# suryanshkumar/online-joint-depthfusion-and-semantic

Measured on AMD Instinct MI355X. Metric: frames/sec fused (320x240, 256^3 grid), higher is better.
Workload: dtype f16x3; 1 GPU; BASELINE configs[1]: 320x240 depth into a 256^3 fp16 TSDF grid, FusionNet_v3, geometry-only, fast integrate, f16x3 arithmetic, one scene per GPU; grid=256, n_points=9, n_tail_points=7, volume_dtype=f16, parallelism=scene-sharded x1, cpu_affinity=not pinned

## Files before the change

### online_joint_depthfusion_and_semantic_amd/csrc/ojf_net.hip

```cpp
#ifndef OJF_CHAIN_DMA_HALF
#define OJF_CHAIN_DMA_HALF 1536
#endif
#ifndef OJF_CHAIN_BLOCKS
#define OJF_CHAIN_BLOCKS 3
#endif
#ifndef OJF_CHAIN_WAVES
#define OJF_CHAIN_WAVES 4
#endif
#ifndef OJF_CHAIN_AHEAD
#define OJF_CHAIN_AHEAD 2
#endif
#include <chrono>
#include <cmath>
#include <cstdio>
#include <cstdlib>
#include <cstring>
#include <vector>

#include "ojf_common.h"

namespace ojf {

typedef float f32x4 __attribute__((ext_vector_type(4)));
typedef float f32x8 __attribute__((ext_vector_type(8)));
typedef _Float16 f16x8 __attribute__((ext_vector_type(8)));

typedef unsigned u32x4 __attribute__((ext_vector_type(4)));
__device__ __forceinline__ void split_f16(const f32x4 &a, const f32x4 &b, f16x8 &hi, f16x8 &lo)
{
    const f32x8 x = __builtin_shufflevector(a, b, 0, 1, 2, 3, 4, 5, 6, 7);
    hi = __builtin_convertvector(x, f16x8);
    const u32x4 h = __builtin_bit_cast(u32x4, hi);
    u32x4 l;
#pragma unroll
    for (int i = 0; i < 4; ++i) l[i] = split_lo_pair(h[i], x[2 * i], x[2 * i + 1]);
    lo = __builtin_bit_cast(f16x8, l);
}

typedef _Float16 f16x4 __attribute__((ext_vector_type(4)));
typedef unsigned u32x2 __attribute__((ext_vector_type(2)));
__device__ __forceinline__ f32x4 split_pack4(const f32x4 &x)
{
    const f16x4 hi = __builtin_convertvector(x, f16x4);
    const u32x2 h = __builtin_bit_cast(u32x2, hi);
    const u32x4 r{h[0], h[1], split_lo_pair(h[0], x[0], x[1]), split_lo_pair(h[1], x[2], x[3])};
    return __builtin_bit_cast(f32x4, r);
}
__device__ __forceinline__ f32x4 unsplit4(const f32x4 &s)
{
    typedef _Float16 f16x8_ __attribute__((ext_vector_type(8)));
    const f16x8_ h = __builtin_bit_cast(f16x8_, s);
    return f32x4{(float)h[0] + (float)h[4], (float)h[1] + (float)h[5], (float)h[2] + (float)h[6], (float)h[3] + (float)h[7]};
}
#ifndef OJF_UNSAFE_SWAP
#define OJF_UNSAFE_SWAP 0
#endif
__device__ __forceinline__ void unpack_split(const f32x4 &a, const f32x4 &b, f16x8 &hi, f16x8 &lo)
{
#if OJF_UNSAFE_SWAP
    u32x4 A = __builtin_bit_cast(u32x4, a), B = __builtin_bit_cast(u32x4, b);
    unsigned a2 = A[2], a3 = A[3], b0 = B[0], b1 = B[1];
    asm("v_swap_b32 %0, %1" : "+v"(a2), "+v"(b0));
    asm("v_swap_b32 %0, %1" : "+v"(a3), "+v"(b1));
    A[2] = a2; A[3] = a3; B[0] = b0; B[1] = b1;
    hi = __builtin_bit_cast(f16x8, A);
    lo = __builtin_bit_cast(f16x8, B);
#else
    hi = __builtin_bit_cast(f16x8, __builtin_shufflevector(a, b, 0, 1, 4, 5));
    lo = __builtin_bit_cast(f16x8, __builtin_shufflevector(a, b, 2, 3, 6, 7));
#endif
}

__device__ __forceinline__ f32x4 mfma_f16x3(const f32x4 &wh, const f32x4 &wl, const f16x8 &xh, const f16x8 &xl, f32x4 acc)
{
    const f16x8 h = __builtin_bit_cast(f16x8, wh), l = __builtin_bit_cast(f16x8, wl);
    acc = __builtin_amdgcn_mfma_f32_16x16x32_f16(l, xh, acc, 0, 0, 0);
    acc = __builtin_amdgcn_mfma_f32_16x16x32_f16(h, xl, acc, 0, 0, 0);
    return __builtin_amdgcn_mfma_f32_16x16x32_f16(h, xh, acc, 0, 0, 0);
}

static inline int round_up(int x, int m) { return (x + m - 1) / m * m; }

struct ConvArgs {
    const f32x4 *in;
    f32x4 *out;
    float *out_rows;
    const f32x4 *wp;
    const float *bias;
    const float *rinv;
    int in_g0, out_g0, rows_stride, rows_n;
    int h, w, npix;
    int taps, dil;
    int c4;
    int nsteps;
    int og_store;
    int act, act_n;
    float scale;
    int *ovf;
    int accum;
    const float *dscale;
    unsigned w_magic, c4_magic;
    int in_split = 0, out_split = 0;
    int row_perm = 0, perm_q = 0, perm_rem = 0;
};

__device__ __forceinline__ int perm_row(int pr, int r, int q, int rem)
{
    const int big = rem * (q + 1);
    if (pr < big) {
        const int c = pr / (q + 1);
        return c + (pr - c * (q + 1)) * r;
    }
    const int p2 = pr - big, c = p2 / q;
    return rem + c + (p2 - c * q) * r;
}

__device__ __forceinline__ int fast_div(int x, int d, unsigned magic) { return magic ? (int)__umulhi((unsigned)x, magic) : x / d; }

__device__ __forceinline__ float guard_max(float mx, const f32x4 &v)
{
    return fmaxf(fmaxf(fmaxf(mx, fabsf(v[0])), fmaxf(fabsf(v[1]), fabsf(v[2]))), fabsf(v[3]));
}
__device__ __forceinline__ bool beyond_f16(const f32x4 &v)
{
    return guard_max(0.0f, v) > 65504.0f;
}
__device__ __forceinline__ f32x4 fma4(const f32x4 &a, const f32x4 &b, const f32x4 &c)
{
    return f32x4{__builtin_fmaf(a[0], b[0], c[0]), __builtin_fmaf(a[1], b[1], c[1]), __builtin_fmaf(a[2], b[2], c[2]),
                 __builtin_fmaf(a[3], b[3], c[3])};
}

__device__ __forceinline__ float act_slope(int act)
{
    return act == OJF_ACT_RELU ? 0.0f : (act == OJF_ACT_LEAKY ? 0.01f : 1.0f);
}
__device__ __forceinline__ float leaky_max(float x, float slope)
{
    const float sx = slope * x;
    float r;
    asm("v_max_f32 %0, %1, %2" : "=v"(r) : "v"(x), "v"(sx));
    return r;
}
__device__ __forceinline__ f32x4 leaky_max4(const f32x4 &x, float slope)
{
    const f32x4 sx = x * slope;
    f32x4 r;
#pragma unroll
    for (int j = 0; j < 4; ++j) asm("v_max_f32 %0, %1, %2" : "=v"(r[j]) : "v"(x[j]), "v"(sx[j]));
    return r;
}

constexpr int kMaxSteps = 128;
constexpr int kPadSteps = 4;

template <int MT, int NT, bool GUARD = false>
__device__ __forceinline__ void conv_epilogue(const ConvArgs &a, const f32x4 (&acc)[MT][NT], int strip, int i16, int g,
                                              const f32x4 (&bvec)[NT], const f32x4 (&rvec)[NT])
{
    const float slope = act_slope(a.act);
    const bool use_tanh = a.act == OJF_ACT_TANH;
    const float oscale = a.dscale ? a.scale / *a.dscale : a.scale;
    float gmax = 0.0f;
#pragma unroll
    for (int n = 0; n < NT; ++n) {
        const int og = n * 4 + g;
        const f32x4 b = bvec[n];
        const f32x4 ri = rvec[n];
#pragma unroll
        for (int m = 0; m < MT; ++m) {
            const int p = strip + m * 16 + i16;
            const f32x4 lin4 = GUARD ? fma4(acc[m][n], ri, b) : acc[m][n] + b;
            f32x4 v = lin4;
#pragma unroll
            for (int j = 0; j < 4; ++j) {
                const float lin = v[j];
                float r = lin > 0.0f ? lin : lin * slope;
                if (use_tanh) r = tanhf(lin);
                v[j] = (og * 4 + j < a.act_n ? r : lin) * oscale;
            }
            if (p >= a.npix) continue;
            if (a.out_rows) {
#pragma unroll
                for (int j = 0; j < 4; ++j)
                    if (og * 4 + j < a.rows_n) a.out_rows[(size_t)p * a.rows_stride + og * 4 + j] = v[j];
            } else if (og < a.og_store) {
                f32x4 *dst = a.out + (size_t)(a.out_g0 + og) * a.npix + p;
                if (a.accum) v += *dst;
                *dst = a.out_split ? split_pack4(v) : v;
                if constexpr (GUARD) gmax = guard_max(gmax, lin4);
            }
        }
    }
    if constexpr (GUARD)
        if (gmax > 65504.0f && a.ovf) guard_raise(a.ovf, 1);
}

template <int MT, int NT>
__device__ __forceinline__ void conv_epilogue_lean(const ConvArgs &a, const f32x4 (&acc)[MT][NT], int strip, int i16, int g,
                                                   const f32x4 (&bvec)[NT], const f32x4 (&rvec)[NT])
{
    const float slope = act_slope(a.act);
    float gmax = 0.0f;
#pragma unroll
    for (int n = 0; n < NT; ++n) {
        const int og = n * 4 + g;
        if (og >= a.og_store) continue;
#pragma unroll
        for (int m = 0; m < MT; ++m) {
            const int p = strip + m * 16 + i16;
            const f32x4 lin4 = fma4(acc[m][n], rvec[n], bvec[n]);
            const f32x4 v = leaky_max4(lin4, slope);
            if (p < a.npix) {
                a.out[(size_t)(a.out_g0 + og) * a.npix + p] = a.out_split ? split_pack4(v) : v;
                gmax = guard_max(gmax, lin4);
            }
        }
    }
    if (gmax > 65504.0f && a.ovf) guard_raise(a.ovf, 1);
}

static inline bool conv_lean_ok(const ConvArgs &a)
{
    return !a.out_rows && a.act != OJF_ACT_TANH && (a.act == OJF_ACT_NONE || a.act_n >= 4 * a.og_store) && a.scale == 1.0f && !a.dscale && !a.accum;
}

__device__ __forceinline__ void build_tap_table(int2 *tab, const ConvArgs &a, int entries)
{
    for (int G = threadIdx.x; G < entries; G += 256) {
        const int t = G / a.c4, cg = G - t * a.c4;
        int off = -1, dy = -30000, dx = 0;
        if (t < a.taps) {
            dy = dx = 0;
            if (a.taps == 9) {
                const int ky = t / 3;
                dy = (ky - 1) * a.dil;
                dx = (t - 3 * ky - 1) * a.dil;
            }
            off = (a.in_g0 + cg) * a.npix + dy * a.w + dx;
        }
        tab[G] = int2{off, (int)(((unsigned)dy << 16) | ((unsigned)dx & 0xffffu))};
    }
}

__device__ __forceinline__ void build_tap_table16(int2 *tab, const ConvArgs &a, int entries)
{
    for (int G = threadIdx.x; G < entries; G += 256) {
        const int t = fast_div(G, a.c4, a.c4_magic), cg = G - t * a.c4;
        int off = 0, bit = 0;
        if (t < a.taps) {
            int dy = 0, dx = 0;
            if (a.taps == 9) {
                const int ky = t / 3;
                dy = (ky - 1) * a.dil;
                dx = (t - 3 * ky - 1) * a.dil;
            }
            off = ((a.in_g0 + cg) * a.npix + dy * a.w + dx) * 16;
            bit = 1 << t;
        }
        tab[G] = int2{off, bit};
    }
}

struct ConvGroup {
    ConvArgs g[4];
    int nblocks;
    int band = 0;
};


template <int MT, int NT, int ABL = 0, bool SKIP = true>
__global__ __launch_bounds__(256) void conv_mfma_kernel(const ConvGroup grp)
{
    const ConvArgs &a = grp.g[blockIdx.y];
    __shared__ int2 tab[(kMaxSteps + kPadSteps) * 4];
    build_tap_table(tab, a, (a.nsteps + kPadSteps) * 4);
    __syncthreads();

    const int lane = threadIdx.x & 63;
    const int wave = threadIdx.x >> 6;
    const int i16 = lane & 15, g = lane >> 4;
    const int strip = (blockIdx.x * 4 + wave) * (MT * 16);
    if (strip >= a.npix) return;
    constexpr int ot0 = 0;

    int py[MT], px[MT], plin[MT];
#pragma unroll
    for (int m = 0; m < MT; ++m) {
        const int p = strip + m * 16 + i16;
        plin[m] = p;
        py[m] = p < a.npix ? p / a.w : -0x40000000;
        px[m] = p - (p / a.w) * a.w;
    }
    f32x4 acc[MT][NT];
#pragma unroll
    for (int m = 0; m < MT; ++m)
#pragma unroll
        for (int n = 0; n < NT; ++n) acc[m][n] = f32x4{0.f, 0.f, 0.f, 0.f};

    const f32x4 *wb[NT];
#pragma unroll
    for (int n = 0; n < NT; ++n) wb[n] = a.wp + (size_t)(ot0 + n) * (a.nsteps + kPadSteps) * 64 + lane;
    const __amdgpu_buffer_rsrc_t rs = __builtin_amdgcn_make_buffer_rsrc(
        const_cast<f32x4 *>(a.in), 0, (a.in_g0 + a.c4) * a.npix * 16, 0x00020000);

    auto fetch = [&](f32x4(&xv)[MT], f32x4(&wv)[NT], int S, bool &live) {
        if constexpr (ABL & 8) {
            live = true;
#pragma unroll
            for (int m = 0; m < MT; ++m) {
                if constexpr (ABL & 1) xv[m] = f32x4{1.f, 2.f, 3.f, 4.f};
                else xv[m] = __builtin_bit_cast(f32x4, __builtin_amdgcn_raw_buffer_load_b128(rs, (unsigned)plin[m] * 16u, 0, 0));
            }
        } else {
            const int2 e = tab[S * 4 + g];
            const int dy = e.y >> 16, dx = (int)(short)(e.y & 0xffff);
            bool any_ok = false;
#pragma unroll
            for (int m = 0; m < MT; ++m) {
                const bool ok = (unsigned)(py[m] + dy) < (unsigned)a.h && (unsigned)(px[m] + dx) < (unsigned)a.w;
                const unsigned boff = ok ? (unsigned)(e.x + plin[m]) * 16u : 0xffffffffu;
                if constexpr (ABL & 1) {
                    xv[m] = f32x4{1.f, 2.f, 3.f, 4.f};
                    asm volatile("" ::"v"(boff));
                } else {
                    xv[m] = __builtin_bit_cast(f32x4, __builtin_amdgcn_raw_buffer_load_b128(rs, boff, 0, 0));
                }
                any_ok |= ok;
            }
            live = SKIP ? __any(any_ok) : true;
        }
#pragma unroll
        for (int n = 0; n < NT; ++n) {
            if constexpr (ABL & 2) wv[n] = f32x4{1.f, 1.f, 1.f, 1.f};
            else wv[n] = wb[n][(size_t)S * 64];
        }
    };
    auto mac = [&](const f32x4(&xv)[MT], const f32x4(&wv)[NT]) {
        if constexpr (ABL & 4) {
#pragma unroll
            for (int m = 0; m < MT; ++m) asm volatile("" ::"v"(xv[m][0]), "v"(xv[m][1]), "v"(xv[m][2]), "v"(xv[m][3]));
#pragma unroll
            for (int n = 0; n < NT; ++n) asm volatile("" ::"v"(wv[n][0]), "v"(wv[n][1]), "v"(wv[n][2]), "v"(wv[n][3]));
            return;
        }
#pragma unroll
        for (int j = 0; j < 4; ++j)
#pragma unroll
            for (int m = 0; m < MT; ++m)
#pragma unroll
                for (int n = 0; n < NT; ++n)
                    acc[m][n] = __builtin_amdgcn_mfma_f32_16x16x4f32(wv[n][j], xv[m][j], acc[m][n], 0, 0, 0);
    };

    f32x4 x0[MT], w0[NT], x1[MT], w1[NT], x2[MT], w2[NT];
    bool l0, l1, l2;
    fetch(x0, w0, 0, l0);
    fetch(x1, w1, 1, l1);
    for (int S = 0; S < a.nsteps; S += 3) {
        fetch(x2, w2, S + 2, l2);
        if (!SKIP || l0) mac(x0, w0);
        fetch(x0, w0, S + 3, l0);
        if (!SKIP || l1) mac(x1, w1);
        fetch(x1, w1, S + 4, l1);
        if (!SKIP || l2) mac(x2, w2);
    }

    f32x4 bvec[NT], rvec[NT];
#pragma unroll
    for (int n = 0; n < NT; ++n) {
        bvec[n] = *reinterpret_cast<const f32x4 *>(a.bias + (size_t)n * 16 + 4 * g);
        rvec[n] = f32x4{1.f, 1.f, 1.f, 1.f};
    }
    conv_epilogue<MT, NT>(a, acc, strip, i16, g, bvec, rvec);
}

template <int NT>
__global__ __launch_bounds__(256) void conv_mfma_lds_kernel(const ConvGroup grp)
{
    constexpr int CS = 3;
    const ConvArgs &a = grp.g[blockIdx.y];
    __shared__ int2 tab[(kMaxSteps + kPadSteps) * 4];
    __shared__ f32x4 wl[CS * NT * 64];
    build_tap_table(tab, a, (a.nsteps + kPadSteps) * 4);
    __syncthreads();
    const int lane = threadIdx.x & 63, wave = threadIdx.x >> 6;
    const int i16 = lane & 15, g = lane >> 4;
    const int strip = (blockIdx.x * 4 + wave) * 16;
    const int p = strip + i16;
    const int py = p < a.npix ? p / a.w : -0x40000000;
    const int px = p - (p / a.w) * a.w;
    f32x4 acc[1][NT];
#pragma unroll
    for (int n = 0; n < NT; ++n) acc[0][n] = f32x4{0.f, 0.f, 0.f, 0.f};
    const __amdgpu_buffer_rsrc_t rs = __builtin_amdgcn_make_buffer_rsrc(
        const_cast<f32x4 *>(a.in), 0, (a.in_g0 + a.c4) * a.npix * 16, 0x00020000);
    auto fetch = [&](f32x4 &xv, int S) {
        const int2 e = tab[S * 4 + g];
        const int dy = e.y >> 16, dx = (int)(short)(e.y & 0xffff);
        const bool ok = (unsigned)(py + dy) < (unsigned)a.h && (unsigned)(px + dx) < (unsigned)a.w;
        xv = __builtin_bit_cast(f32x4, __builtin_amdgcn_raw_buffer_load_b128(rs, ok ? (unsigned)(e.x + p) * 16u : 0xffffffffu, 0, 0));
    };
    auto mac = [&](const f32x4 &xv, int sl) {
        f32x4 wv[NT];
#pragma unroll
        for (int n = 0; n < NT; ++n) wv[n] = wl[(sl * NT + n) * 64 + lane];
#pragma unroll
        for (int j = 0; j < 4; ++j)
#pragma unroll
            for (int n = 0; n < NT; ++n) acc[0][n] = __builtin_amdgcn_mfma_f32_16x16x4f32(wv[n][j], xv[j], acc[0][n], 0, 0, 0);
    };
    f32x4 x0, x1, x2;
    fetch(x0, 0);
    fetch(x1, 1);
    const int nsp = a.nsteps + kPadSteps;
    for (int S = 0; S < a.nsteps; S += 3) {
        if (S) __syncthreads();
        for (int i = threadIdx.x; i < CS * NT * 64; i += 256) {
            const int n = i / (CS * 64), r = i - n * (CS * 64);
            wl[((r >> 6) * NT + n) * 64 + (r & 63)] = a.wp[((size_t)n * nsp + S) * 64 + r];
        }
        __syncthreads();
        fetch(x2, S + 2);
        mac(x0, 0);
        fetch(x0, S + 3);
        mac(x1, 1);
        fetch(x1, S + 4);
        mac(x2, 2);
    }
    f32x4 bvec[NT], rvec[NT];
#pragma unroll
    for (int n = 0; n < NT; ++n) {
        bvec[n] = *reinterpret_cast<const f32x4 *>(a.bias + (size_t)n * 16 + 4 * g);
        rvec[n] = f32x4{1.f, 1.f, 1.f, 1.f};
    }
    if (strip >= a.npix) return;
    conv_epilogue<1, NT>(a, acc, strip, i16, g, bvec, rvec);
}

constexpr int kPad16 = 6;
constexpr int conv16_chunk(int nt) { return nt <= 2 ? 6 : 3; }

template <int MT, int NT, bool SKIP = true, int ABL = 0, bool LEAN = false, bool INS = false>
#ifndef OJF_CONV_LB
#define OJF_CONV_LB 1
#endif
__global__ __launch_bounds__(256, (OJF_CONV_LB && MT == 2 && NT == 2 && LEAN) ? 4 : 1) void conv_f16x3_kernel(const ConvGroup grp)
{
    constexpr int CS = conv16_chunk(NT);
    const ConvArgs &a = grp.g[blockIdx.y];
    const bool persist = grp.band != 0;
    int sb = grp.nblocks ? xcd_band_block(blockIdx.x, gridDim.x) : blockIdx.x;
    int sb_end = sb + 1, sb_step = 1;
    if (persist) {
        const int x = blockIdx.x & 7, j = blockIdx.x >> 3;
        sb = x * grp.band + j;
        sb_end = (x + 1) * grp.band;
        sb_step = (int)(gridDim.x >> 3);
    }
    if (grp.nblocks && sb >= grp.nblocks) return;
    extern __shared__ int2 tab[];
    __shared__ f32x4 wl[CS * NT * 128];
    build_tap_table16(tab, a, (a.nsteps + kPad16) * 8);
    if (persist) {
#pragma unroll
        for (int i = 0; i < CS * NT * 128 / 256; ++i) wl[i * 256 + threadIdx.x] = a.wp[i * 256 + threadIdx.x];
    }

    const int lane = threadIdx.x & 63, wave = threadIdx.x >> 6;
    const int i16 = lane & 15, g = lane >> 4;
    __syncthreads();
    for (; sb < sb_end && (!grp.nblocks || sb < grp.nblocks); sb += sb_step) {
    int strip = (sb * 4 + wave) * (MT * 16);
    if (a.row_perm) {
        const int pr = fast_div(strip, a.w, a.w_magic);
        if (pr < a.h) strip = perm_row(pr, a.row_perm, a.perm_q, a.perm_rem) * a.w + (strip - pr * a.w);
    }

    int p16[MT];
    unsigned vm[MT];
#pragma unroll
    for (int m = 0; m < MT; ++m) {
        const int p = strip + m * 16 + i16;
        p16[m] = p * 16;
        const int py = fast_div(p, a.w, a.w_magic), px = p - py * a.w;
        unsigned rm = 0, cm = 0;
#pragma unroll
        for (int k = 0; k < 3; ++k) {
            rm |= ((unsigned)(py + (k - 1) * a.dil) < (unsigned)a.h ? 1u : 0u) << k;
            cm |= ((unsigned)(px + (k - 1) * a.dil) < (unsigned)a.w ? 1u : 0u) << k;
        }
        const unsigned all9 = ((rm & 1u) ? cm : 0u) | ((rm & 2u) ? cm << 3 : 0u) | ((rm & 4u) ? cm << 6 : 0u);
        vm[m] = p < a.npix ? (a.taps == 9 ? all9 : 1u) : 0u;
    }
    f32x4 acc[MT][NT];
#pragma unroll
    for (int m = 0; m < MT; ++m)
#pragma unroll
        for (int n = 0; n < NT; ++n) {
            acc[m][n] = f32x4{0.f, 0.f, 0.f, 0.f};
            if constexpr (MT == 1) asm volatile("" : "+v"(acc[m][n]));
        }
    const __amdgpu_buffer_rsrc_t rs = __builtin_amdgcn_make_buffer_rsrc(
        const_cast<f32x4 *>(a.in), 0, (a.in_g0 + a.c4) * a.npix * 16, 0x00020000);
    constexpr bool kHoist = NT <= 4;
    f32x4 bvec[NT], rvec[NT];
    if constexpr (kHoist) {
#pragma unroll
        for (int n = 0; n < NT; ++n) {
            bvec[n] = *reinterpret_cast<const f32x4 *>(a.bias + (size_t)n * 16 + 4 * g);
            rvec[n] = *reinterpret_cast<const f32x4 *>(a.rinv + (size_t)n * 16 + 4 * g);
        }
    }

    const int4 *tab4 = reinterpret_cast<const int4 *>(tab) + g;
    auto fetch = [&](f32x4(&xa)[MT], f32x4(&xb)[MT], const int4 e, bool &live) {
        unsigned any = 0;
#pragma unroll
        for (int m = 0; m < MT; ++m) {
            const unsigned o0 = (unsigned)(e.x + p16[m]) | ((vm[m] & (unsigned)e.y) ? 0u : 0xffffffffu);
            const unsigned o1 = (unsigned)(e.z + p16[m]) | ((vm[m] & (unsigned)e.w) ? 0u : 0xffffffffu);
            if constexpr (ABL & 1) {
                xa[m] = f32x4{1.f, 2.f, 3.f, 4.f};
                xb[m] = f32x4{1.f, 2.f, 3.f, 4.f};
                asm volatile("" ::"v"(o0), "v"(o1));
            } else {
                xa[m] = __builtin_bit_cast(f32x4, __builtin_amdgcn_raw_buffer_load_b128(rs, o0, 0, 0));
                xb[m] = __builtin_bit_cast(f32x4, __builtin_amdgcn_raw_buffer_load_b128(rs, o1, 0, 0));
            }
            any |= vm[m] & (unsigned)(e.y | e.w);
        }
        live = SKIP ? __any(any != 0) : true;
    };
    auto mac = [&](const f32x4(&xa)[MT], const f32x4(&xb)[MT], int sl) {
        f32x4 wh[NT], wlo[NT];
#pragma unroll
        for (int n = 0; n < NT; ++n) {
            if constexpr (ABL & 2) {
                wh[n] = wlo[n] = f32x4{1.f, 1.f, 1.f, 1.f};
                asm volatile("" ::"s"(sl));
            } else {
                wh[n] = wl[(sl * NT + n) * 128 + lane];
                wlo[n] = wl[(sl * NT + n) * 128 + 64 + lane];
            }
        }
#pragma unroll
        for (int m = 0; m < MT; ++m) {
            f16x8 xh, xl;
            if constexpr (ABL & 8) {
                xh = __builtin_bit_cast(f16x8, xa[m]);
                xl = __builtin_bit_cast(f16x8, xb[m]);
            } else if constexpr (INS) {
                unpack_split(xa[m], xb[m], xh, xl);
            } else {
                split_f16(xa[m], xb[m], xh, xl);
            }
            if constexpr (ABL & 4) {
                asm volatile("" ::"v"(xh), "v"(xl));
#pragma unroll
                for (int n = 0; n < NT; ++n) asm volatile("" ::"v"(wh[n]), "v"(wlo[n]));
            } else {
#pragma unroll
                for (int n = 0; n < NT; ++n) acc[m][n] = mfma_f16x3(wh[n], wlo[n], xh, xl, acc[m][n]);
            }
        }
    };

    f32x4 xa0[MT], xb0[MT], xa1[MT], xb1[MT], xa2[MT], xb2[MT];
    bool v0, v1, v2;
    fetch(xa0, xb0, tab4[0], v0);
    fetch(xa1, xb1, tab4[4], v1);
    int sl = persist ? 0 : CS;
    for (int S = 0; S < a.nsteps; S += 3) {
        const int4 t2 = tab4[(S + 2) * 4], t3 = tab4[(S + 3) * 4], t4 = tab4[(S + 4) * 4];
        if (sl == CS) {
            if (S) __syncthreads();
            const f32x4 *src = a.wp + (size_t)S * NT * 128;
#pragma unroll
            for (int i = 0; i < CS * NT * 128 / 256; ++i) wl[i * 256 + threadIdx.x] = src[i * 256 + threadIdx.x];
            __syncthreads();
            sl = 0;
        }
        fetch(xa2, xb2, t2, v2);
        if (!SKIP || v0) mac(xa0, xb0, sl);
        fetch(xa0, xb0, t3, v0);
        if (!SKIP || v1) mac(xa1, xb1, sl + 1);
        fetch(xa1, xb1, t4, v1);
        if (!SKIP || v2) mac(xa2, xb2, sl + 2);
        sl += 3;
    }
    if constexpr (!kHoist) {
#pragma unroll
        for (int n = 0; n < NT; ++n) {
            bvec[n] = *reinterpret_cast<const f32x4 *>(a.bias + (size_t)n * 16 + 4 * g);
            rvec[n] = *reinterpret_cast<const f32x4 *>(a.rinv + (size_t)n * 16 + 4 * g);
        }
    }
    if constexpr (LEAN) conv_epilogue_lean<MT, NT>(a, acc, strip, i16, g, bvec, rvec);
    else conv_epilogue<MT, NT, true>(a, acc, strip, i16, g, bvec, rvec);
    }
}

constexpr int kChainLdsFloat4 = 48 * 1024 / 16;
constexpr int kChainDmaHalf = OJF_CHAIN_DMA_HALF;

struct ChainArgs {
    const f32x4 *in;
    const f32x4 *w;
    const float *bias;
    float *out_rows;
    int in_g0, c4_in, npix, rows_stride, rows_n;
    float scale;
    int *ovf;
    f32x4 *out_planes;
    int out_g0, og_store, act_n;
    struct ColSums *colsum;
    int in_split = 0;
    int split_groups = 0;
};

constexpr int chain_kblocks(int arith, int ntin) { return arith == OJF_ARITH_F16X3 ? (ntin + 1) / 2 : ntin; }
constexpr int chain_unit(int arith) { return arith == OJF_ARITH_F16X3 ? 128 : 64; }
constexpr int chain_layer_size(int arith, int ntin, int ntout) { return ntout * chain_kblocks(arith, ntin) * chain_unit(arith); }
constexpr bool chain_dma(int arith) { return arith == OJF_ARITH_F16X3; }
constexpr int chain_cap(int arith) { return chain_dma(arith) ? kChainDmaHalf : kChainLdsFloat4; }
constexpr int chain_tiles_fit(int arith, int ntin)
{
    return chain_cap(arith) / (chain_kblocks(arith, ntin) * chain_unit(arith));
}
constexpr int chain_parts(int arith, int ntin, int ntout)
{
    return (ntout + chain_tiles_fit(arith, ntin) - 1) / chain_tiles_fit(arith, ntin);
}
constexpr int chain_per(int arith, int ntin, int ntout)
{
    return (ntout + chain_parts(arith, ntin, ntout) - 1) / chain_parts(arith, ntin, ntout);
}
constexpr int chain_first_size(int arith, int ntin, int ntout)
{
    return (chain_per(arith, ntin, ntout) < ntout ? chain_per(arith, ntin, ntout) : ntout) * chain_kblocks(arith, ntin) *
           chain_unit(arith);
}
constexpr int chain_bias_stride(int arith, int ntout) { return (arith == OJF_ARITH_F16X3 ? 2 : 1) * ntout * 16; }
constexpr int kChainAhead = OJF_CHAIN_AHEAD;
constexpr int kChainWaves = OJF_CHAIN_WAVES, kChainThreads = 64 * kChainWaves;
constexpr int kChainPre = kChainLdsFloat4 / kChainThreads;

__device__ __forceinline__ void dma_part(const f32x4 *src, f32x4 *dst, int size, int wave, int lane)
{
#pragma unroll
    for (int c0 = 0; c0 < kChainDmaHalf / 64; c0 += kChainWaves) {
        const int c = c0 + wave;
        if (c * 64 < size)
            __builtin_amdgcn_global_load_lds((const void __attribute__((address_space(1))) *)(src + c * 64 + lane),
                                             (void __attribute__((address_space(3))) *)(dst + c * 64), 16, 0, 0);
    }
}

enum { kChainLeaky = 0, kChainRelu = 1, kChainAccumulate = 2, kChainLastRows = 3, kChainEntry = 4 };

constexpr int kVecF4 = 64;
struct VecStage {
    f32x4 *lds;
    f32x4 reg;
    int half;
};
struct VecNext {
    const float *a = nullptr;
    int na = 0;
    const float *b = nullptr;
    int nb = 0;
};
__device__ __forceinline__ void vec_issue(VecStage &vs, const VecNext &nx)
{
    const int t = threadIdx.x;
    if (t < nx.na) vs.reg = reinterpret_cast<const f32x4 *>(nx.a)[t];
    else if (t < nx.na + nx.nb) vs.reg = reinterpret_cast<const f32x4 *>(nx.b)[t - nx.na];
}
__device__ __forceinline__ const f32x4 *vec_commit(VecStage &vs, int n)
{
    f32x4 *dst = vs.lds + vs.half * kVecF4;
    if ((int)threadIdx.x < n) dst[threadIdx.x] = vs.reg;
    vs.half ^= 1;
    return dst;
}

template <int ARITH, int MT, int NTIN, int NTOUT, int MODE, int NEXT_FIRST, int NA, int NB>
__device__ __forceinline__ void chain_layer(const f32x4 (&in)[MT][NA], f32x4 (&out)[MT][NB], f32x4 *wlds, const f32x4 *wg,
                                            const ChainArgs &a, const int (&p)[MT], int lane,
                                            f32x4 (&pre)[kChainPre], int &buf, VecStage &vs, const VecNext nx = VecNext(),
                                            const f32x4 *next_src = nullptr, int commit_extra = 0)
{
    static_assert(NTIN <= NA && NTOUT <= NB, "register arrays too small for this layer");
    const f32x4 *vec = vec_commit(vs, MODE != kChainAccumulate ? chain_bias_stride(ARITH, NTOUT) / 4 : commit_extra);
    constexpr int parts = chain_parts(ARITH, NTIN, NTOUT);
    constexpr int per = chain_per(ARITH, NTIN, NTOUT);
    constexpr int KB = chain_kblocks(ARITH, NTIN);
    constexpr int unit = chain_unit(ARITH);
    static_assert(per * KB * unit <= chain_cap(ARITH), "LDS part too large");
    f16x8 xh[MT][ARITH == OJF_ARITH_F16X3 ? KB : 1], xl[MT][ARITH == OJF_ARITH_F16X3 ? KB : 1];
    if constexpr (ARITH == OJF_ARITH_F16X3) {
#pragma unroll
        for (int m = 0; m < MT; ++m)
#pragma unroll
            for (int S = 0; S < KB; ++S) {
                const f32x4 zero = f32x4{0.f, 0.f, 0.f, 0.f};
                split_f16(in[m][2 * S], 2 * S + 1 < NTIN ? in[m][2 * S + 1 < NTIN ? 2 * S + 1 : 0] : zero, xh[m][S], xl[m][S]);
            }
    }
#pragma unroll
    for (int part = 0; part < parts; ++part) {
        const int nb = part * per;
        const int ne = nb + per < NTOUT ? nb + per : NTOUT;
        const int size = (ne - nb) * KB * unit;
        const int nnb = ne;
        const int nne = nnb + per < NTOUT ? nnb + per : NTOUT;
        const int nsize = part + 1 < parts ? (nne - nnb) * KB * unit : NEXT_FIRST;
        const f32x4 *nsrc = part + 1 < parts ? wg + (size_t)nnb * KB * unit
                                             : (next_src ? next_src : wg + (size_t)chain_layer_size(ARITH, NTIN, NTOUT));
        const f32x4 *wpart = wlds;
        if constexpr (chain_dma(ARITH)) {
            asm volatile("s_waitcnt vmcnt(0)" ::: "memory");
            __syncthreads();
            wpart = wlds + buf * chain_cap(ARITH);
            buf ^= 1;
            dma_part(nsrc, wlds + buf * chain_cap(ARITH), nsize, __builtin_amdgcn_readfirstlane(threadIdx.x >> 6), lane);
            if (part == 0) vec_issue(vs, nx);
        } else {
            __syncthreads();
#pragma unroll
            for (int k = 0; k < kChainPre; ++k)
                if ((int)threadIdx.x + kChainThreads * k < size) wlds[threadIdx.x + kChainThreads * k] = pre[k];
            __syncthreads();
#pragma unroll
            for (int k = 0; k < kChainPre; ++k)
                if ((int)threadIdx.x + kChainThreads * k < nsize) pre[k] = nsrc[threadIdx.x + kChainThreads * k];
            if (part == 0) vec_issue(vs, nx);
        }
        if constexpr (MODE != kChainAccumulate) {
#pragma unroll
            for (int n2 = 0; n2 < NTOUT; ++n2)
#pragma unroll
                for (int m = 0; m < MT; ++m)
                    if (n2 >= nb && n2 < ne) out[m][n2] = f32x4{0.f, 0.f, 0.f, 0.f};
        }
        if constexpr (ARITH == OJF_ARITH_F16X3) {
            const int cnt = ne - nb, steps = KB * cnt;
            f32x4 rh[kChainAhead], rl[kChainAhead];
            auto frag = [&](int t) { return ((t % cnt) * KB + t / cnt) * 128; };
#pragma unroll
            for (int t = 0; t < kChainAhead; ++t)
                if (t < steps) {
                    rh[t] = wpart[frag(t) + lane];
                    rl[t] = wpart[frag(t) + 64 + lane];
                }
#pragma unroll
            for (int t = 0; t < KB * NTOUT; ++t) {
                if (t >= steps) break;
                const f32x4 wh = rh[t % kChainAhead], wl = rl[t % kChainAhead];
                if (t + kChainAhead < steps) {
                    rh[t % kChainAhead] = wpart[frag(t + kChainAhead) + lane];
                    rl[t % kChainAhead] = wpart[frag(t + kChainAhead) + 64 + lane];
                }
                __builtin_amdgcn_sched_barrier(0);
                const int S = t / cnt, n2 = nb + t % cnt;
#pragma unroll
                for (int m = 0; m < MT; ++m) out[m][n2] = mfma_f16x3(wh, wl, xh[m][S], xl[m][S], out[m][n2]);
                __builtin_amdgcn_sched_barrier(0);
            }
        } else {
#pragma unroll
        for (int S = 0; S < KB; ++S)
#pragma unroll
            for (int n2 = 0; n2 < NTOUT; ++n2) {
                if (n2 < nb || n2 >= ne) continue;
                {
                    const f32x4 wv = wpart[((n2 - nb) * KB + S) * 64 + lane];
#pragma unroll
                    for (int j = 0; j < 4; ++j)
#pragma unroll
                        for (int m = 0; m < MT; ++m)
                            out[m][n2] = __builtin_amdgcn_mfma_f32_16x16x4f32(wv[j], in[m][S][j], out[m][n2], 0, 0, 0);
                }
            }
        }
    }
    if constexpr (MODE != kChainAccumulate) {
        const int g = lane >> 4;
        float gmax = 0.0f;
#pragma unroll
        for (int n2 = 0; n2 < NTOUT; ++n2) {
            const f32x4 b = vec[n2 * 4 + g];
            f32x4 ri{1.f, 1.f, 1.f, 1.f};
            if constexpr (ARITH == OJF_ARITH_F16X3) ri = vec[(NTOUT + n2) * 4 + g];
#pragma unroll
            for (int m = 0; m < MT; ++m) {
                const f32x4 lin4 = ARITH == OJF_ARITH_F16X3 ? fma4(out[m][n2], ri, b) : out[m][n2] + b;
                f32x4 v = lin4;
                if constexpr (MODE == kChainLastRows) {
#pragma unroll
                    for (int j = 0; j < 4; ++j) {
                        const int oc = n2 * 16 + 4 * g + j;
                        if (oc < a.rows_n && p[m] < a.npix)
                            a.out_rows[(size_t)p[m] * a.rows_stride + oc] = tanhf(v[j]) * a.scale;
                    }
                } else if constexpr (MODE == kChainEntry) {
                    const int og = n2 * 4 + g;
#pragma unroll
                    for (int j = 0; j < 4; ++j) v[j] = (og * 4 + j < a.act_n && !(v[j] > 0.0f)) ? (v[j] != v[j] ? v[j] : 0.0f) : v[j];
                    if (p[m] < a.npix && og < a.og_store) {
                        a.out_planes[(size_t)(a.out_g0 + og) * a.npix + p[m]] = og < a.split_groups ? split_pack4(v) : v;
                        if constexpr (ARITH == OJF_ARITH_F16X3) gmax = guard_max(gmax, lin4);
                    }
                } else {
                    constexpr float slope = MODE == kChainRelu ? 0.0f : 0.01f;
                    v = leaky_max4(v, slope);
                    if constexpr (ARITH == OJF_ARITH_F16X3) gmax = guard_max(gmax, lin4);
                    out[m][n2] = v;
                }
            }
        }
        if constexpr (ARITH == OJF_ARITH_F16X3)
            if (gmax > 65504.0f && a.ovf) guard_raise(a.ovf, 1);
    }
}

template <int ARITH, int MT, int NTIN, int NTOUT>
__device__ __forceinline__ void chain_run(f32x4 (&x)[MT][8], f32x4 (&y)[MT][8], f32x4 *wlds, const f32x4 *wg,
                                          const float *bias, const ChainArgs &a, const int (&p)[MT], int lane,
                                          f32x4 (&pre)[kChainPre], int &buf, VecStage &vs)
{
    chain_layer<ARITH, MT, NTIN, NTOUT, kChainLastRows, 0>(x, y, wlds, wg, a, p, lane, pre, buf, vs);
}

template <int ARITH, int MT, int NTIN, int NTOUT, int NTNEXT, int... REST>
__device__ __forceinline__ void chain_run(f32x4 (&x)[MT][8], f32x4 (&y)[MT][8], f32x4 *wlds, const f32x4 *wg,
                                          const float *bias, const ChainArgs &a, const int (&p)[MT], int lane,
                                          f32x4 (&pre)[kChainPre], int &buf, VecStage &vs)
{
    VecNext nx;
    nx.a = bias + chain_bias_stride(ARITH, NTOUT);
    nx.na = chain_bias_stride(ARITH, NTNEXT) / 4;
    chain_layer<ARITH, MT, NTIN, NTOUT, kChainLeaky, chain_first_size(ARITH, NTOUT, NTNEXT)>(x, y, wlds, wg, a, p, lane, pre,
                                                                                             buf, vs, nx);
    chain_run<ARITH, MT, NTOUT, NTNEXT, REST...>(y, x, wlds, wg + (size_t)chain_layer_size(ARITH, NTIN, NTOUT),
                                                 bias + chain_bias_stride(ARITH, NTOUT), a, p, lane, pre, buf, vs);
}

template <int ARITH, int MT, int NT0, int... NTS>
__global__ __launch_bounds__(kChainThreads, OJF_CHAIN_BLOCKS) void chain1x1_kernel(const ChainArgs a)
{
    __shared__ f32x4 wlds[chain_dma(ARITH) ? 2 * kChainDmaHalf : kChainLdsFloat4];
    __shared__ f32x4 vec_lds[2 * kVecF4];
    const int lane = threadIdx.x & 63, wave = threadIdx.x >> 6;
    const int i16 = lane & 15, g = lane >> 4;
    const int strip = (banded_block_x() * kChainWaves + wave) * (MT * 16);
    int p[MT];
    f32x4 x[MT][8], y[MT][8];
    VecStage vs;
    vs.lds = vec_lds; vs.half = 0;
    {
        constexpr int first[] = {NTS...};
        VecNext nx;
        nx.a = a.bias; nx.na = chain_bias_stride(ARITH, first[0]) / 4;
        vec_issue(vs, nx);
    }
#pragma unroll
    for (int m = 0; m < MT; ++m) {
        p[m] = strip + m * 16 + i16;
#pragma unroll
        for (int S = 0; S < NT0; ++S) {
            const int G = 4 * S + g;
            const bool ok = p[m] < a.npix && G < a.c4_in;
            x[m][S] = a.in[ok ? (a.in_g0 + G) * a.npix + p[m] : -1];
        }
    }
    f32x4 pre[kChainPre];
    int buf = 0;
    {
        constexpr int first[] = {NTS...};
        constexpr int size0 = chain_first_size(ARITH, NT0, first[0]);
        if constexpr (chain_dma(ARITH)) {
            dma_part(a.w, wlds, size0, __builtin_amdgcn_readfirstlane(threadIdx.x >> 6), lane);
        } else {
#pragma unroll
            for (int k = 0; k < kChainPre; ++k)
                if ((int)threadIdx.x + kChainThreads * k < size0) pre[k] = a.w[threadIdx.x + kChainThreads * k];
        }
    }
    chain_run<ARITH, MT, NT0, NTS...>(x, y, wlds, a.w, a.bias, a, p, lane, pre, buf, vs);
}

constexpr int kColShards = 16;
constexpr float kColScale = 1048576.0f;

constexpr int kColMax = 256;
struct ColSums {
    long long fix[kColShards][kColMax];
    unsigned bad[kColMax];
};
constexpr int colsum_row(int nt) { return nt > 8 ? 256 : 128; }

template <int MT, int NT, int NA>
__device__ __forceinline__ void block_colsum(const f32x4 (&x)[MT][NA], const int (&p)[MT], int npix, float *red ,
                                             ColSums *out, int lane, int wave, int off = 0)
{
    constexpr int RS = colsum_row(NT);
    const int g = lane >> 4;
#pragma unroll
    for (int S = 0; S < NT; ++S) {
        f32x4 s{0.f, 0.f, 0.f, 0.f};
#pragma unroll
        for (int m = 0; m < MT; ++m)
            if (p[m] < npix) s += x[m][S];
#pragma unroll
        for (int j = 0; j < 4; ++j) {
            float v = s[j];
            v += __shfl_xor(v, 8, 64);
            v += __shfl_xor(v, 4, 64);
            v += __shfl_xor(v, 2, 64);
            v += __shfl_xor(v, 1, 64);
            s[j] = v;
        }
        if ((lane & 15) == 0) *reinterpret_cast<f32x4 *>(red + wave * RS + S * 16 + 4 * g) = s;
    }
    __syncthreads();
    static_assert(NT * 16 <= kChainThreads && NT * 16 <= kColMax, "one thread per channel");
    if ((int)threadIdx.x < NT * 16) {
        const int t = threadIdx.x;
        float v = (red[t] + red[RS + t]) + (red[2 * RS + t] + red[3 * RS + t]);
#pragma unroll
        for (int w4 = 4; w4 < kChainWaves; w4 += 4)
            v += (red[w4 * RS + t] + red[(w4 + 1) * RS + t]) + (red[(w4 + 2) * RS + t] + red[(w4 + 3) * RS + t]);
        if (v - v == 0.0f) {
            const long long q = (long long)__builtin_rintf(v * kColScale);
            if (q) atomicAdd(reinterpret_cast<unsigned long long *>(&out->fix[blockIdx.x % kColShards][t + off]), (unsigned long long)q);
        } else {
            atomicOr(&out->bad[t + off], 1u);
        }
    }
}

template <int ARITH, int MT, int NTIN, int NTOUT>
__global__ __launch_bounds__(kChainThreads, OJF_CHAIN_BLOCKS) void entry1x1_kernel(const ChainArgs a)
{
    __shared__ f32x4 wlds[chain_dma(ARITH) ? 2 * kChainDmaHalf : kChainLdsFloat4];
    __shared__ f32x4 vec_lds[2 * kVecF4];
    __shared__ float red[kChainWaves * colsum_row(NTIN)];
    const int lane = threadIdx.x & 63, wave = threadIdx.x >> 6;
    const int i16 = lane & 15, g = lane >> 4;
    const int strip = (banded_block_x() * kChainWaves + wave) * (MT * 16);
    f32x4 pre[kChainPre];
    int buf = 0;
    VecStage vs;
    vs.lds = vec_lds; vs.half = 0;
    {
        VecNext nx;
        nx.a = a.bias; nx.na = chain_bias_stride(ARITH, NTOUT) / 4;
        vec_issue(vs, nx);
    }
    {
        constexpr int size0 = chain_first_size(ARITH, NTIN, NTOUT);
        if constexpr (chain_dma(ARITH)) {
            dma_part(a.w, wlds, size0, __builtin_amdgcn_readfirstlane(threadIdx.x >> 6), lane);
        } else {
#pragma unroll
            for (int k = 0; k < kChainPre; ++k)
                if ((int)threadIdx.x + kChainThreads * k < size0) pre[k] = a.w[threadIdx.x + kChainThreads * k];
        }
    }
    int p[MT];
    f32x4 x[MT][NTIN], y[MT][NTOUT];
#pragma unroll
    for (int m = 0; m < MT; ++m) {
        p[m] = strip + m * 16 + i16;
#pragma unroll
        for (int S = 0; S < NTIN; ++S) {
            const int G = 4 * S + g;
            const bool ok = p[m] < a.npix && G < a.c4_in;
            x[m][S] = a.in[ok ? (a.in_g0 + G) * a.npix + p[m] : -1];
            if (a.in_split) x[m][S] = unsplit4(x[m][S]);
        }
    }
    if (a.colsum) block_colsum<MT, NTIN>(x, p, a.npix, red, a.colsum, lane, wave);
    chain_layer<ARITH, MT, NTIN, NTOUT, kChainEntry, 0>(x, y, wlds, a.w, a, p, lane, pre, buf, vs);
}

struct TailArgs {
    const f32x4 *v[4];
    const f32x4 *w;
    const float *b1;
    const float *bias_final;
    const float *rinv_final;
    f32x4 *out;
    int c4, out_g0, og_store, npix;
    int *ovf;
    const f32x4 *chain_w;
    const float *chain_b;
    float *out_rows;
    int rows_stride, rows_n;
    float scale;
    const f32x4 *entry_w;
    const float *entry_b;
    f32x4 *entry_out;
    int entry_og, entry_act_n;
    struct ColSums *colsum;
    int entry_split;
    int colsum_off = 0;
};

constexpr int kTailEntry = 1;

template <int ARITH, int MT, int KIND>
__device__ __forceinline__ void head_run(f32x4 (&x)[MT][8], f32x4 (&y)[MT][8], f32x4 *wlds, const f32x4 *wg, const float *bias,
                                         const ChainArgs &a, const int (&p)[MT], int lane, f32x4 (&pre)[kChainPre], int &buf,
                                         VecStage &vs)
{
    if constexpr (KIND == 19) chain_run<ARITH, MT, 8, 6, 6, 5, 5, 4, 4, 3, 3, 2, 2, 1>(x, y, wlds, wg, bias, a, p, lane, pre, buf, vs);
    else chain_run<ARITH, MT, 8, 7, 7, 5, 5, 4, 4, 3, 3, 2, 2, 1>(x, y, wlds, wg, bias, a, p, lane, pre, buf, vs);
}
constexpr int head_first_ntout(int kind) { return kind == 19 ? 6 : 7; }
constexpr int head_first_size(int arith, int kind) { return chain_first_size(arith, 8, kind == 19 ? 6 : 7); }

template <int ARITH, int MT, int NV, int NO, int CHAIN = 0>
__global__ __launch_bounds__(kChainThreads, OJF_CHAIN_BLOCKS) void vortex_tail_kernel(const TailArgs a)
{
    static_assert(CHAIN == 0 || NO == 8, "the fused prediction head / entry layer expects 8 input tiles");
    __shared__ f32x4 wlds[chain_dma(ARITH) ? 2 * kChainDmaHalf : kChainLdsFloat4];
    __shared__ f32x4 vec_lds[2 * kVecF4];
    __shared__ float red[CHAIN == kTailEntry ? kChainWaves * 128 : 1];
    const int lane = threadIdx.x & 63, wave = threadIdx.x >> 6;
    const int i16 = lane & 15, g = lane >> 4;
    const int strip = (banded_block_x() * kChainWaves + wave) * (MT * 16);
    int p[MT];
#pragma unroll
    for (int m = 0; m < MT; ++m) p[m] = strip + m * 16 + i16;
    constexpr int kVec1 = chain_bias_stride(ARITH, NO) / 4, kVecFin = NO * 4 * (ARITH == OJF_ARITH_F16X3 ? 2 : 1);
    VecStage vs;
    vs.lds = vec_lds; vs.half = 0;
    {
        VecNext nx;
        nx.a = a.b1; nx.na = kVec1;
        vec_issue(vs, nx);
    }
    ChainArgs ca;
    ca.npix = a.npix; ca.out_rows = nullptr; ca.rows_n = 0; ca.rows_stride = 0; ca.scale = 1.0f; ca.ovf = a.ovf;
    f32x4 y[MT][NO];
#pragma unroll
    for (int m = 0; m < MT; ++m)
#pragma unroll
        for (int n = 0; n < NO; ++n) y[m][n] = f32x4{0.f, 0.f, 0.f, 0.f};
    f32x4 pre[kChainPre];
    int buf = 0;
    {
        constexpr int size0 = chain_first_size(ARITH, NV, NO);
        if constexpr (chain_dma(ARITH)) {
            dma_part(a.w, wlds, size0, __builtin_amdgcn_readfirstlane(threadIdx.x >> 6), lane);
        } else {
#pragma unroll
            for (int k = 0; k < kChainPre; ++k)
                if ((int)threadIdx.x + kChainThreads * k < size0) pre[k] = a.w[threadIdx.x + kChainThreads * k];
        }
    }
    constexpr size_t per_branch = (size_t)chain_layer_size(ARITH, NV, NO) + chain_layer_size(ARITH, NO, NO);
    f32x4 t[MT][NO];
    const f32x4 *vfin = vec_lds;
#pragma unroll
    for (int b = 0; b < 4; ++b) {
        f32x4 vin[MT][NV];
#pragma unroll
        for (int m = 0; m < MT; ++m)
#pragma unroll
            for (int S = 0; S < NV; ++S) {
                const int G = 4 * S + g;
                const bool ok = p[m] < a.npix && G < a.c4;
                vin[m][S] = a.v[b][ok ? G * a.npix + p[m] : -1];
            }
        const f32x4 *w1 = a.w + b * per_branch, *wf = w1 + (size_t)chain_layer_size(ARITH, NV, NO);
        VecNext nx;
        if (b < 3) {
            nx.a = a.b1 + (b + 1) * chain_bias_stride(ARITH, NO); nx.na = kVec1;
        } else {
            nx.a = a.bias_final; nx.na = NO * 4;
            if constexpr (ARITH == OJF_ARITH_F16X3) { nx.b = a.rinv_final; nx.nb = NO * 4; }
        }
        chain_layer<ARITH, MT, NV, NO, kChainRelu, chain_first_size(ARITH, NO, NO)>(vin, t, wlds, w1, ca, p, lane, pre, buf, vs, nx);
        if (b < 3) {
            chain_layer<ARITH, MT, NO, NO, kChainAccumulate, chain_first_size(ARITH, NV, NO)>(t, y, wlds, wf, ca, p, lane, pre, buf, vs);
        } else {
            vfin = vs.lds + vs.half * kVecF4;
            VecNext nf;
            if constexpr (CHAIN == kTailEntry) { nf.a = a.entry_b; nf.na = chain_bias_stride(ARITH, 5) / 4; }
            else if constexpr (CHAIN != 0) { nf.a = a.chain_b; nf.na = chain_bias_stride(ARITH, head_first_ntout(CHAIN)) / 4; }
            chain_layer<ARITH, MT, NO, NO, kChainAccumulate,
                        CHAIN == kTailEntry ? chain_first_size(ARITH, 8, 5) : (CHAIN ? head_first_size(ARITH, CHAIN) : 0)>(
                t, y, wlds, wf, ca, p, lane, pre, buf, vs, nf, CHAIN == kTailEntry ? a.entry_w : a.chain_w, kVecFin);
        }
    }
    float gmax = 0.0f;
#pragma unroll
    for (int n = 0; n < NO; ++n) {
        const int og = n * 4 + g;
        const f32x4 bf = vfin[n * 4 + g];
#pragma unroll
        for (int m = 0; m < MT; ++m) {
            f32x4 v = y[m][n] + bf;
            if constexpr (ARITH == OJF_ARITH_F16X3) v = fma4(y[m][n], vfin[NO * 4 + n * 4 + g], bf);
            if constexpr (ARITH == OJF_ARITH_F16X3) gmax = guard_max(gmax, v);
            if constexpr (CHAIN) y[m][n] = v;
            else if (p[m] < a.npix && og < a.og_store) a.out[(size_t)(a.out_g0 + og) * a.npix + p[m]] = v;
        }
    }
    if constexpr (ARITH == OJF_ARITH_F16X3)
        if (gmax > 65504.0f && a.ovf) guard_raise(a.ovf, 1);
    if constexpr (CHAIN == kTailEntry) {
        block_colsum<MT, NO>(y, p, a.npix, red, a.colsum, lane, wave, a.colsum_off);
        ca.out_planes = a.entry_out; ca.out_g0 = 0; ca.og_store = a.entry_og; ca.act_n = a.entry_act_n; ca.split_groups = a.entry_split;
        chain_layer<ARITH, MT, 8, 5, kChainEntry, 0>(y, t, wlds, a.entry_w, ca, p, lane, pre, buf, vs);
    } else if constexpr (CHAIN) {
        ca.out_rows = a.out_rows; ca.rows_stride = a.rows_stride; ca.rows_n = a.rows_n; ca.scale = a.scale;
        head_run<ARITH, MT, CHAIN>(y, t, wlds, a.chain_w, a.chain_b, ca, p, lane, pre, buf, vs);
    }
}

struct GaveArgs {
    const float *partial;
    struct ColSums *fixed;
    int nparts, pstride, cphys, npix;
    const float *WgT, *bg, *WfgT, *bf;
    int c_out;
    float *bias_out;
    int bias_len;
};

struct PyramidArgs {
    const f32x4 *z;
    f32x4 *q[3];
    const float *bias[3];
    int h, w, c4;
    int tiles;
    int fold_gave;
    const f32x4 *z2 = nullptr;
    f32x4 *q0 = nullptr;
    const float *bias0 = nullptr;
    int split_out;
    GaveArgs gave;
};

constexpr int kPoolTW = 32, kPoolTH = 8, kPoolStride = kPoolTW + 6;

template <int LV>
__device__ __forceinline__ void pool_pyramid_body(const PyramidArgs &a, f32x4 (&buf)[2][kPoolStride * (kPoolTH + 6)], int cg)
{
    const int tiles_x = (a.w + kPoolTW - 1) / kPoolTW;
    const int tile = banded_block_x();
    const int ty = tile / tiles_x, tx = tile - ty * tiles_x;
    const int x0 = tx * kPoolTW, y0 = ty * kPoolTH, npix = a.h * a.w;
    const f32x4 *plane = a.z + (size_t)(LV * a.c4 + cg) * npix;
    const f32x4 *plane2 = a.z2 ? a.z2 + (size_t)(LV * a.c4 + cg) * npix : nullptr;
    const f32x4 zero{0.f, 0.f, 0.f, 0.f};
    {
        constexpr int W0 = kPoolTW + 2 * LV, H0 = kPoolTH + 2 * LV;
#pragma unroll
        for (int i0 = 0; i0 < W0 * H0; i0 += 256) {
            const int i = i0 + threadIdx.x;
            if (i >= W0 * H0) break;
            const int ly = i / W0, lx = i - ly * W0;
            const int gy = y0 - LV + ly, gx = x0 - LV + lx;
            const bool in = (unsigned)gy < (unsigned)a.h && (unsigned)gx < (unsigned)a.w;
            f32x4 v = in ? plane[gy * a.w + gx] : zero;
            if (plane2 && in) v += plane2[gy * a.w + gx];
            buf[0][ly * kPoolStride + lx] = v;
        }
    }
    __syncthreads();
#pragma unroll
    for (int l = 1; l <= LV; ++l) {
        const int halo = LV - l;
        const int Wl = kPoolTW + 2 * halo, Hl = kPoolTH + 2 * halo;
        const f32x4 *src = buf[(l - 1) & 1];
#pragma unroll
        for (int i0 = 0; i0 < Wl * Hl; i0 += 256) {
            const int i = i0 + threadIdx.x;
            if (i >= Wl * Hl) break;
            const int ly = i / Wl, lx = i - ly * Wl;
            const int gy = y0 - halo + ly, gx = x0 - halo + lx;
            const bool in = (unsigned)gy < (unsigned)a.h && (unsigned)gx < (unsigned)a.w;
            f32x4 s = zero;
#pragma unroll
            for (int dy = 0; dy < 3; ++dy)
#pragma unroll
                for (int dx = 0; dx < 3; ++dx) s += src[(ly + dy) * kPoolStride + lx + dx];
            s = s / 9.0f;
            if (l < LV) {
                buf[l & 1][ly * kPoolStride + lx] = in ? s : zero;
            } else if (in) {
                s += *reinterpret_cast<const f32x4 *>(a.bias[LV - 1] + 4 * cg);
#pragma unroll
                for (int j = 0; j < 4; ++j) s[j] = s[j] < 0.0f ? 0.0f : s[j];
                a.q[LV - 1][(size_t)cg * npix + gy * a.w + gx] = a.split_out ? split_pack4(s) : s;
            }
        }
        if (l < LV) __syncthreads();
    }
}

__device__ __forceinline__ void gave_bias_block(const GaveArgs &a, float *mean, float *gv);

__global__ __launch_bounds__(256) void pool_pyramid_kernel(const PyramidArgs a)
{
    __shared__ f32x4 buf[2][kPoolStride * (kPoolTH + 6)];
    if (banded_block_x() >= a.tiles) {
        if (blockIdx.y == 0 && banded_block_x() == a.tiles && a.fold_gave)
            gave_bias_block(a.gave, reinterpret_cast<float *>(buf), reinterpret_cast<float *>(buf) + 256);
        return;
    }
    const int yg = blockIdx.y / a.c4, cg = blockIdx.y - yg * a.c4;
    const int lv = yg < 3 ? 3 - yg : 4;
    if (lv == 4) {
        const int tiles_x = (a.w + kPoolTW - 1) / kPoolTW;
        const int tile = banded_block_x();
        const int ty = tile / tiles_x, tx = tile - ty * tiles_x;
        const int gy = ty * kPoolTH + (int)threadIdx.x / kPoolTW, gx = tx * kPoolTW + (int)threadIdx.x % kPoolTW;
        if (gy < a.h && gx < a.w) {
            const size_t at = (size_t)cg * a.h * a.w + gy * a.w + gx;
            f32x4 v = a.z[at] + a.z2[at] + *reinterpret_cast<const f32x4 *>(a.bias0 + 4 * cg);
#pragma unroll
            for (int j = 0; j < 4; ++j) v[j] = v[j] < 0.0f ? 0.0f : v[j];
            a.q0[at] = a.split_out ? split_pack4(v) : v;
        }
        return;
    }
    if (lv == 1) pool_pyramid_body<1>(a, buf, cg);
    else if (lv == 2) pool_pyramid_body<2>(a, buf, cg);
    else pool_pyramid_body<3>(a, buf, cg);
}

constexpr int kSumBlocks = 32;

__global__ __launch_bounds__(256) void colsum_kernel(const f32x4 *in, int g0, int npix, float *partial)
{
    __shared__ f32x4 red[4];
    const int cg = blockIdx.y;
    const int per = (npix + gridDim.x - 1) / gridDim.x;
    const int p0 = blockIdx.x * per, p1 = min(npix, p0 + per);
    const f32x4 *plane = in + (size_t)(g0 + cg) * npix;
    f32x4 s{0.f, 0.f, 0.f, 0.f};
    for (int p = p0 + threadIdx.x; p < p1; p += 256) s += plane[p];
#pragma unroll
    for (int j = 0; j < 4; ++j)
        for (int off = 32; off > 0; off >>= 1) s[j] += __shfl_down(s[j], off, 64);
    if ((threadIdx.x & 63) == 0) red[threadIdx.x >> 6] = s;
    __syncthreads();
    if (threadIdx.x == 0) {
        s = (red[0] + red[1]) + (red[2] + red[3]);
        *reinterpret_cast<f32x4 *>(partial + (size_t)blockIdx.x * 256 + 4 * cg) = s;
    }
}


__device__ __forceinline__ void gave_bias_block(const GaveArgs &a, float *mean , float *gv )
{
    const int t = threadIdx.x;
    if (a.fixed) {
        if (t < kColMax) {
            long long q = 0;
#pragma unroll
            for (int sh = 0; sh < kColShards; ++sh) {
                q += a.fixed->fix[sh][t];
                a.fixed->fix[sh][t] = 0;
            }
            const bool bad = a.fixed->bad[t] != 0;
            a.fixed->bad[t] = 0;
            const float sum = (float)((double)q * (1.0 / (double)kColScale));
            mean[t] = t < a.cphys ? (bad ? __builtin_nanf("") : sum / (float)a.npix) : 0.0f;
        }
    } else if (a.cphys <= 128) {
        const int ch = t & 127, half = t >> 7;
        float s = 0.0f;
        if (ch < a.cphys) {
            const int r0 = half ? (a.nparts + 1) / 2 : 0, r1 = half ? a.nparts : (a.nparts + 1) / 2;
#pragma unroll 8
            for (int b = r0; b < r1; ++b) s += a.partial[(size_t)b * a.pstride + ch];
        }
        gv[t] = s;
        __syncthreads();
        mean[t] = t < a.cphys ? (gv[t] + gv[128 + t]) / (float)a.npix : 0.0f;
    } else {
        float s = 0.0f;
        if (t < a.cphys) {
#pragma unroll 8
            for (int b = 0; b < a.nparts; ++b) s += a.partial[(size_t)b * a.pstride + t];
        }
        mean[t] = s / (float)a.npix;
    }
    __syncthreads();
    float s1 = 0.0f;
    if (t < a.c_out) {
        s1 = a.bg[t];
#pragma unroll 8
        for (int c = 0; c < a.cphys; ++c) s1 = __builtin_fmaf(a.WgT[(size_t)c * a.c_out + t], mean[c], s1);
    }
    __syncthreads();
    gv[t] = s1;
    __syncthreads();
    if (t < a.bias_len) {
        float s = 0.0f;
        if (t < a.c_out) {
            s = a.bf[t];
#pragma unroll 8
            for (int j = 0; j < a.c_out; ++j) s = __builtin_fmaf(a.WfgT[(size_t)j * a.c_out + t], gv[j], s);
        }
        a.bias_out[t] = s;
    }
}

__global__ __launch_bounds__(256) void gave_bias_kernel(const GaveArgs a)
{
    __shared__ float mean[256];
    __shared__ float gv[256];
    gave_bias_block(a, mean, gv);
}

struct PrepArgs {
    const float *values;
    const float *weights;
    const float *depth;
    const uint8_t *sem;
    f32x4 *x0;
    f32x4 *x1;
    int rows_stride, in_layout, npix, P, cs4, n_classes, v2_sem;
    int *ovf;
    int split;
};

__global__ __launch_bounds__(256) void prepare_input_kernel(const PrepArgs a)
{
    const int p = blockIdx.x * blockDim.x + threadIdx.x;
    if (p >= a.npix) return;
    const size_t pix = a.in_layout ? (size_t)p : (size_t)p * a.rows_stride;
    const size_t chn = a.in_layout ? (size_t)a.rows_stride : 1;
    const float *v = a.values + pix;
    const float *wt = a.weights + pix;
    const float d = a.depth[p];
    const float sf = a.sem ? (1.0f + (float)a.sem[p]) / (float)a.n_classes : 0.0f;
    bool bad = false;
    for (int cg = 0; cg < a.cs4; ++cg) {
        f32x4 r0, r1;
#pragma unroll
        for (int j = 0; j < 4; ++j) {
            const int c = 4 * cg + j;
            float base = 0.0f;
            if (c < a.P) base = v[c * chn];
            else if (c < 2 * a.P) base = wt[(c - a.P) * chn];
            r0[j] = base;
            r1[j] = base;
            if (c == 2 * a.P) { r0[j] = d; r1[j] = sf; }
            if (c == 2 * a.P + 1 && a.v2_sem) r0[j] = sf;
        }
        a.x0[(size_t)cg * a.npix + p] = a.split ? split_pack4(r0) : r0;
        if (a.x1) a.x1[(size_t)cg * a.npix + p] = a.split ? split_pack4(r1) : r1;
        bad = bad || beyond_f16(r0) || beyond_f16(r1);
    }
    if (bad && a.ovf) guard_raise(a.ovf, 1);
}

__global__ __launch_bounds__(256) void rows_to_planes_kernel(const float *rows, int stride, int off, int c, f32x4 *planes,
                                                              int c4, int npix)
{
    const int item = blockIdx.x * blockDim.x + threadIdx.x;
    if (item >= npix * c4) return;
    const int cg = item / npix, p = item - cg * npix;
    f32x4 v;
#pragma unroll
    for (int j = 0; j < 4; ++j) v[j] = (4 * cg + j < c) ? rows[(size_t)p * stride + off + 4 * cg + j] : 0.0f;
    planes[(size_t)cg * npix + p] = v;
}

__global__ __launch_bounds__(256) void planes_to_rows_kernel(const f32x4 *planes, int c4, int npix, float *rows, int stride,
                                                              int off)
{
    const int item = blockIdx.x * blockDim.x + threadIdx.x;
    if (item >= npix * c4) return;
    const int cg = item / npix, p = item - cg * npix;
    const f32x4 v = planes[(size_t)cg * npix + p];
#pragma unroll
    for (int j = 0; j < 4; ++j) rows[(size_t)p * stride + off + 4 * cg + j] = v[j];
}

}
#include "ojf_net_pair.h"
#include "ojf_net_chain.h"
namespace ojf {

struct PackedConv {
    float *wp = nullptr;
    float *bias = nullptr;
    float *rinv = nullptr;
    int c_in_phys = 0, c_out_phys = 0, taps = 1, dil = 1, n_ot = 0;
    int arith = OJF_ARITH_F32, nsteps = 0;
};

static int g_default_arith = OJF_ARITH_F16X3;

static volatile int *g_ovf_host = nullptr;
static int *g_ovf_dev = nullptr;

static int *overflow_flag()
{
    if (!g_ovf_dev) {
        void *h = nullptr, *hd = nullptr, *d = nullptr;
        if (hipHostMalloc(&h, sizeof(int), hipHostMallocMapped) != hipSuccess) return nullptr;
        *static_cast<int *>(h) = 0;
        if (hipHostGetDevicePointer(&hd, h, 0) != hipSuccess) return nullptr;
        if (hipMalloc(&d, 16) != hipSuccess) return nullptr;
        struct { int flag, skipped; void *mirror; } init{0, 0, hd};
        static_assert(sizeof(init) == 16, "guard block layout");
        if (hipMemcpy(d, &init, sizeof(init), hipMemcpyHostToDevice) != hipSuccess) return nullptr;
        g_ovf_host = static_cast<volatile int *>(h);
        g_ovf_dev = static_cast<int *>(d);
    }
    return g_ovf_dev;
}

int *range_flag_device() { return overflow_flag(); }
const int *range_guard_if_any() { return g_ovf_dev; }

static int guard_take(int *skipped, bool clear)
{
    if (!g_ovf_host || !*g_ovf_host) {
        if (skipped) *skipped = 0;
        return 0;
    }
    const int what = *g_ovf_host;
    int blk[2] = {what, 0};
    (void)hipMemcpy(blk, g_ovf_dev, sizeof(blk), hipMemcpyDeviceToHost);
    if (skipped) *skipped = blk[1];
    if (clear) {
        (void)hipMemset(g_ovf_dev, 0, 2 * sizeof(int));
        (void)hipStreamSynchronize(nullptr);
        *g_ovf_host = 0;
    }
    return what;
}

struct LaunchMark { const char *name; hipStream_t st; hipEvent_t ev; };
static thread_local int g_launches = 0;
static thread_local bool g_profile = false;
static thread_local std::vector<LaunchMark> g_marks;

static inline void mark_launch(const char *name, hipStream_t st)
{
    ++g_launches;
    if (!g_profile) return;
    hipEvent_t e = nullptr;
    if (hipEventCreateWithFlags(&e, hipEventDisableSystemFence) != hipSuccess) return;
    (void)hipEventRecord(e, st);
    g_marks.push_back(LaunchMark{name, st, e});
}

static unsigned event_flags()
{
    static const bool fence = getenv("OJF_EVENT_FENCE") && atoi(getenv("OJF_EVENT_FENCE"));
    return fence ? hipEventDisableTiming : (hipEventDisableTiming | hipEventDisableSystemFence);
}

static const char *kChainStuckMsg =
    "fusion net: dense_chain_kernel gave up waiting for a neighbouring tile (internal error: the results of this forward pass are invalid)";
static const char *kOverflowMsg =
    "split-fp16 arithmetic: an activation or input left the fp16 range (|x| > 65504 or NaN); results since the last "
    "ojf_net_check are invalid - use ojf_net_set_arithmetic(OJF_ARITH_F32) for this network";

static inline float row_scale(float row_max)
{
    if (!(row_max > 0.0f) || !std::isfinite(row_max)) return 1.0f;
    int e = 0;
    (void)std::frexp(row_max, &e);
    int k = 14 - e;
    k = k > 100 ? 100 : (k < -100 ? -100 : k);
    return std::ldexp(1.0f, k);
}

static inline void split_weight(float v, _Float16 &hi, _Float16 &lo)
{
    hi = (_Float16)v;
    lo = (_Float16)(v - (float)hi);
}

constexpr int kNT = 2;

struct ConvBuilder {
    int c_in_phys, c_out_phys, taps, dil;
    std::vector<float> W;
    std::vector<float> B;
    ConvBuilder(int cin_phys, int cout_phys, int ksize, int dilation)
        : c_in_phys(cin_phys), c_out_phys(cout_phys), taps(ksize * ksize), dil(dilation),
          W((size_t)cout_phys * ksize * ksize * cin_phys, 0.0f), B(cout_phys, 0.0f) {}
    void add(const ojf_conv_layer &L, int ci0, int ci1, const std::vector<int> &in_map, int oc_off, bool with_bias)
    {
        const int kk = L.ksize * L.ksize;
        for (int o = 0; o < L.c_out; ++o) {
            for (int ci = ci0; ci < ci1; ++ci)
                for (int t = 0; t < kk; ++t)
                    W[((size_t)(oc_off + o) * taps + t) * c_in_phys + in_map[ci - ci0]] =
                        L.weight_host[((size_t)o * L.c_in + ci) * kk + t];
            if (with_bias) B[oc_off + o] = L.bias_host[o];
        }
    }
};

static int upload(const std::vector<float> &h, float **d)
{
    OJF_HIP(hipMalloc(reinterpret_cast<void **>(d), h.size() * sizeof(float)));
    OJF_HIP(hipMemcpy(*d, h.data(), h.size() * sizeof(float), hipMemcpyHostToDevice));
    return 0;
}

static int finish(const ConvBuilder &b, PackedConv &pc, int arith = OJF_ARITH_F32)
{
    if (b.c_in_phys % 4) return fail("conv packing: c_in_phys must be a multiple of 4");
    pc.c_in_phys = b.c_in_phys;
    pc.c_out_phys = b.c_out_phys;
    pc.taps = b.taps;
    pc.dil = b.dil;
    pc.arith = arith;
    pc.n_ot = round_up(round_up(b.c_out_phys, 16) / 16, kNT);
    const int c4 = b.c_in_phys / 4, groups = b.taps * c4;
    const int per = arith == OJF_ARITH_F16X3 ? 8 : 4;
    const int nsteps = (groups + per - 1) / per;
    if (nsteps > kMaxSteps) return fail("conv packing: K too large for the tap table");
    pc.nsteps = nsteps;
    std::vector<float> wp, bias((size_t)pc.n_ot * 16, 0.0f);
    if (arith == OJF_ARITH_F16X3) {
        std::vector<float> rs((size_t)pc.n_ot * 16, 1.0f), rinv((size_t)pc.n_ot * 16, 1.0f);
        for (int oc = 0; oc < b.c_out_phys; ++oc) {
            float mx = 0.0f;
            const float *row = b.W.data() + (size_t)oc * b.taps * b.c_in_phys;
            for (int i = 0; i < b.taps * b.c_in_phys; ++i) mx = std::fmax(mx, std::fabs(row[i]));
            rs[oc] = row_scale(mx);
            rinv[oc] = 1.0f / rs[oc];
        }
        if (upload(rinv, &pc.rinv)) return -2;
        const int nsp = nsteps + kPad16;
        wp.assign((size_t)nsp * pc.n_ot * 128 * 4, 0.0f);
        _Float16 *hp = reinterpret_cast<_Float16 *>(wp.data());
        for (int S = 0; S < nsteps; ++S)
            for (int ot = 0; ot < pc.n_ot; ++ot)
                for (int lane = 0; lane < 64; ++lane)
                    for (int j = 0; j < 8; ++j) {
                        const int oc = ot * 16 + (lane & 15), G = 8 * S + 2 * (lane >> 4) + (j >> 2);
                        if (oc >= b.c_out_phys || G >= groups) continue;
                        const int t = G / c4, cg = G % c4;
                        const float v = rs[oc] * b.W[((size_t)oc * b.taps + t) * b.c_in_phys + 4 * cg + (j & 3)];
                        const size_t base = ((size_t)S * pc.n_ot + ot) * 2 * 64 * 8;
                        split_weight(v, hp[base + (size_t)lane * 8 + j], hp[base + 64 * 8 + (size_t)lane * 8 + j]);
                    }
    } else {
        const int nsp = nsteps + kPadSteps;
        wp.assign((size_t)pc.n_ot * nsp * 256, 0.0f);
        for (int ot = 0; ot < pc.n_ot; ++ot)
            for (int S = 0; S < nsteps; ++S)
                for (int lane = 0; lane < 64; ++lane) {
                    const int oc = ot * 16 + (lane & 15), G = 4 * S + (lane >> 4);
                    if (oc >= b.c_out_phys || G >= groups) continue;
                    const int t = G / c4, cg = G % c4;
                    const float *row = b.W.data() + ((size_t)oc * b.taps + t) * b.c_in_phys + 4 * cg;
                    float *dst = wp.data() + (((size_t)ot * nsp + S) * 64 + lane) * 4;
                    for (int j = 0; j < 4; ++j) dst[j] = row[j];
                }
    }
    for (int o = 0; o < b.c_out_phys; ++o) bias[o] = b.B[o];
    if (upload(wp, &pc.wp)) return -2;
    if (upload(bias, &pc.bias)) return -2;
    return 0;
}

static void release(PackedConv &pc)
{
    if (pc.wp) (void)hipFree(pc.wp);
    if (pc.bias) (void)hipFree(pc.bias);
    if (pc.rinv) (void)hipFree(pc.rinv);
    pc.wp = pc.bias = pc.rinv = nullptr;
}

static inline f32x4 *planes(float *p) { return reinterpret_cast<f32x4 *>(p); }
static inline const f32x4 *planes(const float *p) { return reinterpret_cast<const f32x4 *>(p); }

#ifdef OJF_PAIR_TIMING
static long long *g_pair_dbg = nullptr;
#endif
struct PackedPair {
    float *wa = nullptr, *wb = nullptr, *vec = nullptr;
    int c4_in = 0, n_chunks = 0, np_last = 0, np_b = 0, og_store = 0;
    int cfg = 0;
};

enum PairCfg { PAIR_20x16_W16 = 0, PAIR_12x8_W16 = 1, PAIR_20x8_W8 = 2, PAIR_16x8_W8 = 3, PAIR_20x8_W8_CP4 = 4,
               PAIR_20x16_W16_P5 = 5, PAIR_12x8_W16_P5 = 6, PAIR_CFG_COUNT = 7 };
static inline int pair_cfg_chunk_pairs(int cfg) { return cfg == PAIR_20x8_W8 || cfg == PAIR_16x8_W8 ? 3 : 4; }
static inline bool pair_cfg_pack(int cfg) { return cfg == PAIR_20x16_W16_P5 || cfg == PAIR_12x8_W16_P5; }
static int pair_cfg_for(int h, int w, int c_out_phys)
{
    static const int forced = getenv("OJF_PAIR_CFG") ? atoi(getenv("OJF_PAIR_CFG")) : -1;
    const bool big = ((w + 19) / 20) * ((h + 15) / 16) >= 200;
    int cfg = big ? PAIR_20x16_W16 : PAIR_12x8_W16;
    if (forced >= 0 && forced < PAIR_CFG_COUNT && (!pair_cfg_pack(forced) || c_out_phys == 20)) cfg = forced;
    return cfg;
}

static void release(PackedPair &pp)
{
    float *ptrs[] = {pp.wa, pp.wb, pp.vec};
    for (float *p : ptrs)
        if (p) (void)hipFree(p);
    pp.wa = pp.wb = pp.vec = nullptr;
}

static void pack_pair_conv5(const ConvBuilder &b, const std::vector<float> &rs, std::vector<float> &dst, int cp)
{
    const int npairs = (b.c_in_phys + 7) / 8, n_chunks = (npairs + cp - 1) / cp, ocp = b.c_out_phys;
    for (int c = 0; c < n_chunks; ++c) {
        const int np = c == n_chunks - 1 ? npairs - cp * c : cp, nkb = (9 * np + 3) / 4;
        const size_t base = dst.size();
        dst.resize(base + (size_t)nkb * 192 * 4, 0.0f);
        _Float16 *hp = reinterpret_cast<_Float16 *>(dst.data() + base);
        for (int S = 0; S < nkb; ++S)
            for (int t = 0; t < 3; ++t)
                for (int lane = 0; lane < 64; ++lane)
                    for (int j = 0; j < 8; ++j) {
                        const int R = t * 16 + (lane & 15), u = 4 * S + (lane >> 4);
                        if (R >= 2 * ocp || u >= 9 * np) continue;
                        const int oc = R < ocp ? R : R - ocp;
                        const int tap = u / np, ch = 8 * (cp * c + u % np) + j;
                        if (ch >= b.c_in_phys) continue;
                        const float v = rs[oc] * b.W[((size_t)oc * b.taps + tap) * b.c_in_phys + ch];
                        _Float16 hi, lo;
                        split_weight(v, hi, lo);
                        hp[(((size_t)S * 3 + t) * 64 + lane) * 8 + j] = R < ocp ? hi : lo;
                    }
    }
}

static void pack_pair_conv(const ConvBuilder &b, const std::vector<float> &rs, std::vector<float> &dst, int cp)
{
    const int npairs = (b.c_in_phys + 7) / 8, n_chunks = (npairs + cp - 1) / cp;
    for (int c = 0; c < n_chunks; ++c) {
        const int np = c == n_chunks - 1 ? npairs - cp * c : cp, nkb = (9 * np + 3) / 4;
        const size_t base = dst.size();
        dst.resize(base + (size_t)nkb * 256 * 4, 0.0f);
        _Float16 *hp = reinterpret_cast<_Float16 *>(dst.data() + base);
        for (int S = 0; S < nkb; ++S)
            for (int nt = 0; nt < 2; ++nt)
                for (int lane = 0; lane < 64; ++lane)
                    for (int j = 0; j < 8; ++j) {
                        const int oc = nt * 16 + (lane & 15), u = 4 * S + (lane >> 4);
                        if (oc >= b.c_out_phys || u >= 9 * np) continue;
                        const int tap = u / np, ch = 8 * (cp * c + u % np) + j;
                        if (ch >= b.c_in_phys) continue;
                        const float v = rs[oc] * b.W[((size_t)oc * b.taps + tap) * b.c_in_phys + ch];
                        const size_t ub = ((size_t)S * 2 + nt) * 2 * 64 * 8;
                        split_weight(v, hp[ub + (size_t)lane * 8 + j], hp[ub + 64 * 8 + (size_t)lane * 8 + j]);
                    }
    }
}

static int finish_pair(const ConvBuilder &ba, const ConvBuilder &bb, PackedPair &pp, int cfg = PAIR_20x16_W16)
{
    const int cp = pair_cfg_chunk_pairs(cfg);
    pp.cfg = cfg;
    if (ba.taps != 9 || bb.taps != 9 || ba.dil != 1 || bb.dil != 1 || ba.c_out_phys > 24 || bb.c_in_phys != ba.c_out_phys ||
        bb.c_out_phys > 32 || ba.c_in_phys % 4)
        return fail("pair packing: unsupported layer shapes");
    std::vector<float> vec(128, 0.0f), wa, wb;
    auto scales = [&](const ConvBuilder &b, int off) {
        std::vector<float> rs(32, 1.0f);
        for (int oc = 0; oc < b.c_out_phys; ++oc) {
            float mx = 0.0f;
            const float *row = b.W.data() + (size_t)oc * b.taps * b.c_in_phys;
            for (int i = 0; i < b.taps * b.c_in_phys; ++i) mx = std::fmax(mx, std::fabs(row[i]));
            rs[oc] = row_scale(mx);
            vec[off + oc] = b.B[oc];
        }
        for (int oc = 0; oc < 32; ++oc) vec[off + 32 + oc] = 1.0f / rs[oc];
        return rs;
    };
    const std::vector<float> ra = scales(ba, 0), rb = scales(bb, 64);
    if (pair_cfg_pack(cfg)) {
        if (ba.c_out_phys != 20 || bb.c_out_phys != 20) return fail("pair packing: the packed-row shapes need 20 physical output channels");
        pack_pair_conv5(ba, ra, wa, cp);
        pack_pair_conv5(bb, rb, wb, 4);
    } else {
        pack_pair_conv(ba, ra, wa, cp);
        pack_pair_conv(bb, rb, wb, 4);
    }
    pp.np_b = (bb.c_in_phys + 7) / 8;
    const int npairs = (ba.c_in_phys + 7) / 8;
    pp.c4_in = ba.c_in_phys / 4;
    pp.n_chunks = (npairs + cp - 1) / cp;
    pp.np_last = npairs - cp * (pp.n_chunks - 1);
    pp.og_store = round_up(bb.c_out_phys, 4) / 4;
    if (upload(wa, &pp.wa) || upload(wb, &pp.wb) || upload(vec, &pp.vec)) return -2;
    return 0;
}

template <int TW, int TH, int WAVES = 16, int CP = 4, bool ALIAS = false, bool PACK = false>
static int launch_pair_t(PairArgs &a, hipStream_t st)
{
    using G = PairGeom<TW, TH, WAVES, CP, ALIAS, PACK>;
    static bool configured = false;
    if (!configured) {
        OJF_HIP(hipFuncSetAttribute(reinterpret_cast<const void *>(&dense_pair_kernel<TW, TH, WAVES, CP, ALIAS, PACK>),
                                    hipFuncAttributeMaxDynamicSharedMemorySize, (int)G::LDS_BYTES));
        configured = true;
    }
    a.tiles_x = (a.w + TW - 1) / TW;
    const int tiles = a.tiles_x * ((a.h + TH - 1) / TH);
    hipLaunchKernelGGL((dense_pair_kernel<TW, TH, WAVES, CP, ALIAS, PACK>), dim3(tiles), dim3(G::THREADS), G::LDS_BYTES, st, a);
    mark_launch("dense_pair_kernel", st);
    return check_hip(hipGetLastError(), "dense_pair_kernel launch");
}

static int launch_pair(const PackedPair &pp, const float *in, int in_g0, float *out, int out_g0, int h, int w, hipStream_t st)
{
    PairArgs a;
    a.in = planes(in); a.out = planes(out);
    a.wa = planes(pp.wa); a.wb = planes(pp.wb);
    a.bias_a = pp.vec; a.rinv_a = pp.vec + 32; a.bias_b = pp.vec + 64; a.rinv_b = pp.vec + 96;
    a.in_g0 = in_g0; a.c4_in = pp.c4_in; a.out_g0 = out_g0; a.og_store = pp.og_store;
    a.h = h; a.w = w; a.npix = h * w; a.tiles_x = 0;
    a.n_chunks = pp.n_chunks; a.np_last = pp.np_last; a.np_b = pp.np_b;
    static const bool no_band = getenv("OJF_NO_XCD_BAND") != nullptr;
    a.xcd_bands = no_band ? 0 : 1;
    a.ovf = overflow_flag();
#ifdef OJF_PAIR_TIMING
    a.dbg = g_pair_dbg;
#endif
    switch (pp.cfg) {
    case PAIR_20x16_W16: return launch_pair_t<20, 16>(a, st);
    case PAIR_12x8_W16: return launch_pair_t<12, 8>(a, st);
    case PAIR_20x8_W8: return launch_pair_t<20, 8, 8, 3, true>(a, st);
    case PAIR_16x8_W8: return launch_pair_t<16, 8, 8, 3, true>(a, st);
    case PAIR_20x8_W8_CP4: return launch_pair_t<20, 8, 8, 4, true>(a, st);
    case PAIR_20x16_W16_P5: return launch_pair_t<20, 16, 16, 4, false, true>(a, st);
    case PAIR_12x8_W16_P5: return launch_pair_t<12, 8, 16, 4, false, true>(a, st);
    }
    return fail("dense pair: unknown launch shape");
}

#ifdef OJF_CHAIN_TIMING
static long long *g_chain_dbg = nullptr;
#endif
struct PackedChain {
    float *w = nullptr, *vec = nullptr;
    int *sync = nullptr;
    int layers = 0;
};
constexpr int kChainSyncInts = kChainFlags0 + 8192;

static void release(PackedChain &pc)
{
    if (pc.w) (void)hipFree(pc.w);
    if (pc.vec) (void)hipFree(pc.vec);
    if (pc.sync) (void)hipFree(pc.sync);
    pc.w = pc.vec = nullptr; pc.sync = nullptr; pc.layers = 0;
}

static void pack_chain_step(const ConvBuilder &b, const std::vector<float> &rs, int ch0, std::vector<float> &dst)
{
    const size_t base = dst.size();
    dst.resize(base + (size_t)kChainStepF4 * 4, 0.0f);
    _Float16 *hp = reinterpret_cast<_Float16 *>(dst.data() + base);
    for (int S = 0; S < kChainKB; ++S)
        for (int t = 0; t < 3; ++t)
            for (int lane = 0; lane < 64; ++lane)
                for (int j = 0; j < 8; ++j) {
                    const int r16 = lane & 15, g = lane >> 4, R = 2 * S + (j >> 2);
                    const int oc = t < 2 ? r16 : (r16 < 8 ? 16 + (r16 & 3) : -1);
                    const bool want_lo = t == 1 || (t == 2 && r16 >= 4);
                    const int tap = chain_hu_tap(R, g), ch = ch0 + 4 * chain_hu_q(R, g) + (j & 3);
                    if (oc < 0 || oc >= b.c_out_phys || tap < 0 || ch >= b.c_in_phys) continue;
                    const float v = rs[oc] * b.W[((size_t)oc * b.taps + tap) * b.c_in_phys + ch];
                    _Float16 hi, lo;
                    split_weight(v, hi, lo);
                    hp[(((size_t)S * 3 + t) * 64 + lane) * 8 + j] = want_lo ? lo : hi;
                }
}

static int finish_chain(const std::vector<ConvBuilder> &ba, const std::vector<ConvBuilder> &bb, PackedChain &pc)
{
    const int L = (int)ba.size();
    if (L < 1 || L > kChainMaxLayers || (int)bb.size() != L) return fail("chain packing: unsupported Block count");
    std::vector<float> vec((size_t)L * 128, 0.0f), w;
    for (int l = 0; l < L; ++l) {
        const ConvBuilder &a = ba[l], &b = bb[l];
        if (a.taps != 9 || b.taps != 9 || a.dil != 1 || b.dil != 1 || a.c_out_phys != 4 * kChainNG || b.c_in_phys != 4 * kChainNG ||
            b.c_out_phys != 4 * kChainNG || a.c_in_phys != 4 * kChainNG * (l + 1))
            return fail("chain packing: unsupported layer shapes");
        auto scales = [&](const ConvBuilder &cb, int off) {
            std::vector<float> rs(32, 1.0f);
            for (int oc = 0; oc < cb.c_out_phys; ++oc) {
                float mx = 0.0f;
                const float *row = cb.W.data() + (size_t)oc * cb.taps * cb.c_in_phys;
                for (int i = 0; i < cb.taps * cb.c_in_phys; ++i) mx = std::fmax(mx, std::fabs(row[i]));
                rs[oc] = row_scale(mx);
                vec[(size_t)l * 128 + off + oc] = cb.B[oc];
            }
            for (int oc = 0; oc < 32; ++oc) vec[(size_t)l * 128 + off + 32 + oc] = 1.0f / rs[oc];
            return rs;
        };
        const std::vector<float> ra = scales(a, 0), rb = scales(b, 64);
        for (int c = 0; c <= l; ++c) pack_chain_step(a, ra, 4 * kChainNG * c, w);
        pack_chain_step(b, rb, 0, w);
    }
    pc.layers = L;
    if (upload(w, &pc.w) || upload(vec, &pc.vec)) return -2;
    OJF_HIP(hipMalloc(reinterpret_cast<void **>(&pc.sync), kChainSyncInts * sizeof(int)));
    OJF_HIP(hipMemset(pc.sync, 0, kChainSyncInts * sizeof(int)));
    OJF_HIP(hipStreamSynchronize(nullptr));
    const int epoch0 = kChainEpoch;
    OJF_HIP(hipMemcpy(pc.sync, &epoch0, sizeof(int), hipMemcpyHostToDevice));
    return 0;
}

static int device_cu_count()
{
    static int cus = 0;
    if (!cus) {
        int dev = 0;
        if (hipGetDevice(&dev) != hipSuccess || hipDeviceGetAttribute(&cus, hipDeviceAttributeMultiprocessorCount, dev) != hipSuccess) cus = 0;
    }
    return cus;
}

template <int TW, int TH, int WAVES>
static int launch_chain_t(ChainDenseArgs &a, hipStream_t st)
{
    using G = ChainGeom<TW, TH, WAVES>;
    static bool configured = false;
    if (!configured) {
        OJF_HIP(hipFuncSetAttribute(reinterpret_cast<const void *>(&dense_chain_kernel<TW, TH, WAVES>),
                                    hipFuncAttributeMaxDynamicSharedMemorySize, (int)G::LDS_BYTES));
        configured = true;
    }
    a.tiles_x = (a.w_img + TW - 1) / TW;
    a.tiles_y = (a.h + TH - 1) / TH;
    const int tiles = a.tiles_x * a.tiles_y, cus = device_cu_count();
    if (tiles > kChainSyncInts - kChainFlags0) return fail("dense chain: too many tiles for the flag array");
    const int grid = cus > 0 && cus < tiles ? cus : tiles;
    hipLaunchKernelGGL((dense_chain_kernel<TW, TH, WAVES>), dim3(grid), dim3(G::THREADS), G::LDS_BYTES, st, a);
    mark_launch("dense_chain_kernel", st);
    return check_hip(hipGetLastError(), "dense_chain_kernel launch");
}

static int launch_chain(const PackedChain &pc, float *x, int h, int w, hipStream_t st)
{
    ChainDenseArgs a;
    a.x = planes(x); a.xo = planes(x);
    a.w = planes(pc.w); a.vec = pc.vec;
    a.sync = pc.sync; a.layers = pc.layers;
    a.h = h; a.w_img = w; a.npix = h * w; a.tiles_x = a.tiles_y = 0;
    static const bool no_band = getenv("OJF_NO_XCD_BAND") != nullptr;
    a.xcd_bands = no_band ? 0 : 1;
    a.ovf = overflow_flag();
#ifdef OJF_CHAIN_TIMING
    a.dbg = g_chain_dbg;
#endif
    static const int waves = getenv("OJF_CHAIN_WAVES") ? atoi(getenv("OJF_CHAIN_WAVES")) : 16;
    if (((w + 19) / 20) * ((h + 15) / 16) >= 200)
        return waves == 16 ? launch_chain_t<20, 16, 16>(a, st) : (waves == 12 ? launch_chain_t<20, 16, 12>(a, st) : launch_chain_t<20, 16, 8>(a, st));
    return launch_chain_t<12, 8, 8>(a, st);
}

}
#include "ojf_net_branch.h"
namespace ojf {

struct PackedBranches {
    float *w = nullptr, *vec = nullptr;
    int4 *items = nullptr;
    int n_items = 0;
    int4 *sub_items = nullptr;
    int n_sub = 0;
    int dil[4] = {0, 0, 0, 0};
};

static void release(PackedBranches &pb)
{
    if (pb.w) (void)hipFree(pb.w);
    if (pb.vec) (void)hipFree(pb.vec);
    if (pb.items) (void)hipFree(pb.items);
    if (pb.sub_items) (void)hipFree(pb.sub_items);
    pb = PackedBranches();
}

static std::vector<int4> branch_items(const int (&dil)[4], int h, int w)
{
    struct Plan { int br, kind, ntx, nty, cost; };
    std::vector<Plan> plans;
    for (int br = 0; br < 4; ++br) {
        const int d = dil[br], smw = (w + d - 1) / d, smh = (h + d - 1) / d;
        Plan p{br, 0, 0, 0, 0};
        if (smw <= BranchK2::TW && smh <= BranchK2::TH) {
            p.kind = 2; p.ntx = p.nty = 1;
        } else {
            const int ntx = (smw + 19) / 20, n0 = (smh + BranchK0::TH - 1) / BranchK0::TH, n1 = (smh + BranchK1::TH - 1) / BranchK1::TH;
            const int c0 = n0 * (BranchK0::TILES_A + BranchK0::TILES_B), c1 = n1 * (BranchK1::TILES_A + BranchK1::TILES_B);
            p.kind = c1 < c0 ? 1 : 0; p.ntx = ntx; p.nty = c1 < c0 ? n1 : n0;
        }
        plans.push_back(p);
    }
    std::vector<int4> items;
    for (int kind = 0; kind < 3; ++kind)
        for (const Plan &p : plans) {
            if (p.kind != kind) continue;
            const int d = dil[p.br];
            std::vector<int> phases;
            for (int py = 0; py < d && py < h; ++py)
                for (int px = 0; px < d && px < w; ++px) phases.push_back(px | (py << 16));
            const int head = p.br | (kind << 4);
            if (kind == 2) {
                for (size_t i = 0; i < phases.size(); i += 2)
                    items.push_back(int4{head, phases[i], i + 1 < phases.size() ? phases[i + 1] : -1, 0});
                continue;
            }
            const int tw = 20, th = kind == 1 ? BranchK1::TH : BranchK0::TH, nt = p.ntx * p.nty;
            for (int t0 = 0; t0 < nt; t0 += 8) {
                const int n = nt - t0 < 8 ? nt - t0 : 8;
                for (int ph : phases)
                    for (int c = 0; c < n; ++c) {
                        const int t = n == 8 ? t0 + (int)(items.size() & 7u) : t0 + c;
                        items.push_back(int4{head, ph, -1, ((t % p.ntx) * tw) | (((t / p.ntx) * th) << 16)});
                    }
            }
        }
    return items;
}

static std::vector<int4> subconv_items(const int (&dil)[4], int h, int w)
{
    struct Kind { int tw, th, tiles; };
    const Kind kinds[4] = {{SubK0::TW, SubK0::TH, SubK0::TILES}, {SubK1::TW, SubK1::TH, SubK1::TILES}, {SubK2::TW, SubK2::TH, SubK2::TILES},
                           {SubK3::TW, SubK3::TH, SubK3::TILES}};
    std::vector<int4> items;
    for (int br = 0; br < 4; ++br) {
        const int d = dil[br], smw = (w + d - 1) / d, smh = (h + d - 1) / d;
        int best = 0;
        long best_cost = -1;
        for (int k = 0; k < 4; ++k) {
            const long cost = (long)((smw + kinds[k].tw - 1) / kinds[k].tw) * ((smh + kinds[k].th - 1) / kinds[k].th) * kinds[k].tiles;
            if (best_cost < 0 || cost < best_cost) { best_cost = cost; best = k; }
        }
        const Kind &K = kinds[best];
        const int ntx = (smw + K.tw - 1) / K.tw, nty = (smh + K.th - 1) / K.th, nt = ntx * nty, head = br | (best << 4);
        std::vector<int> phases;
        for (int py = 0; py < d && py < h; ++py)
            for (int px = 0; px < d && px < w; ++px) phases.push_back(px | (py << 16));
        for (int t0 = 0; t0 < nt; t0 += 8) {
            const int n = nt - t0 < 8 ? nt - t0 : 8;
            for (int ph : phases)
                for (int c = 0; c < n; ++c) {
                    const int t = n == 8 ? t0 + (int)(items.size() & 7u) : t0 + c;
                    items.push_back(int4{head, ph, -1, ((t % ntx) * K.tw) | (((t / ntx) * K.th) << 16)});
                }
        }
    }
    return items;
}

static int finish_branches(const std::vector<ConvBuilder> &ba, const std::vector<ConvBuilder> &bb, int h, int w, PackedBranches &pb)
{
    if (ba.size() != 4 || bb.size() != 4) return fail("branch packing: four branches expected");
    std::vector<float> vec(4 * 128, 0.0f), wts;
    for (int br = 0; br < 4; ++br) {
        const ConvBuilder &a = ba[br], &b = bb[br];
        if (a.taps != 9 || b.taps != 9 || a.dil != b.dil || a.dil < 1 || a.c_in_phys != 4 * kChainNG || a.c_out_phys != 4 * kChainNG ||
            b.c_in_phys != 4 * kChainNG || b.c_out_phys != 4 * kChainNG)
            return fail("branch packing: unsupported layer shapes");
        pb.dil[br] = a.dil;
        auto scales = [&](const ConvBuilder &cb, int off) {
            std::vector<float> rs(32, 1.0f);
            for (int oc = 0; oc < cb.c_out_phys; ++oc) {
                float mx = 0.0f;
                const float *row = cb.W.data() + (size_t)oc * cb.taps * cb.c_in_phys;
                for (int i = 0; i < cb.taps * cb.c_in_phys; ++i) mx = std::fmax(mx, std::fabs(row[i]));
                rs[oc] = row_scale(mx);
                vec[(size_t)br * 128 + off + oc] = cb.B[oc];
            }
            for (int oc = 0; oc < 32; ++oc) vec[(size_t)br * 128 + off + 32 + oc] = 1.0f / rs[oc];
            return rs;
        };
        const std::vector<float> ra = scales(a, 0), rb = scales(b, 64);
        pack_chain_step(a, ra, 0, wts);
        pack_chain_step(b, rb, 0, wts);
    }
    const std::vector<int4> items = branch_items(pb.dil, h, w);
    if (items.empty() || items.size() > (1u << 20)) return fail("branch packing: bad item count");
    pb.n_items = (int)items.size();
    if (upload(wts, &pb.w) || upload(vec, &pb.vec)) return -2;
    OJF_HIP(hipMalloc(reinterpret_cast<void **>(&pb.items), items.size() * sizeof(int4)));
    OJF_HIP(hipMemcpy(pb.items, items.data(), items.size() * sizeof(int4), hipMemcpyHostToDevice));
    const std::vector<int4> sub = subconv_items(pb.dil, h, w);
    if (sub.empty() || sub.size() > (1u << 22)) return fail("branch packing: bad subconv item count");
    pb.n_sub = (int)sub.size();
    OJF_HIP(hipMalloc(reinterpret_cast<void **>(&pb.sub_items), sub.size() * sizeof(int4)));
    OJF_HIP(hipMemcpy(pb.sub_items, sub.data(), sub.size() * sizeof(int4), hipMemcpyHostToDevice));
    return 0;
}

static int launch_subconv(const PackedBranches &pb, const float *const *in, float *const *out, int second, bool out_split, int h, int w,
                          hipStream_t st)
{
    static bool configured = false;
    if (!configured) {
        OJF_HIP(hipFuncSetAttribute(reinterpret_cast<const void *>(&subconv_kernel), hipFuncAttributeMaxDynamicSharedMemorySize, (int)kSubLdsBytes));
        configured = true;
    }
    SubArgs a;
    for (int br = 0; br < 4; ++br) { a.in[br] = planes(in[br]); a.out[br] = planes(out[br]); a.dil[br] = pb.dil[br]; }
    a.w = planes(pb.w); a.vec = pb.vec; a.items = pb.sub_items;
    a.second = second; a.out_split = out_split ? 1 : 0;
    a.h = h; a.w_img = w; a.npix = h * w;
    a.ovf = overflow_flag();
    hipLaunchKernelGGL(subconv_kernel, dim3(pb.n_sub), dim3(256), kSubLdsBytes, st, a);
    mark_launch("subconv_kernel", st);
    return check_hip(hipGetLastError(), "subconv_kernel launch");
}

static int launch_branches(const PackedBranches &pb, const float *const *in, float *out, int h, int w, hipStream_t st)
{
    static bool configured = false;
    if (!configured) {
        OJF_HIP(hipFuncSetAttribute(reinterpret_cast<const void *>(&vortex_branch_kernel), hipFuncAttributeMaxDynamicSharedMemorySize,
                                    (int)kBranchLdsBytes));
        configured = true;
    }
    BranchArgs a;
    for (int br = 0; br < 4; ++br) { a.in[br] = planes(in[br]); a.dil[br] = pb.dil[br]; }
    a.out = planes(out);
    a.w = planes(pb.w); a.vec = pb.vec; a.items = pb.items; a.n_items = pb.n_items;
    a.h = h; a.w_img = w; a.npix = h * w;
    a.ovf = overflow_flag();
    const int cus = device_cu_count();
    const int grid = cus > 0 && cus < pb.n_items ? cus : pb.n_items;
    hipLaunchKernelGGL(vortex_branch_kernel, dim3(grid), dim3(64 * kBranchWaves), kBranchLdsBytes, st, a);
    mark_launch("vortex_branch_kernel", st);
    return check_hip(hipGetLastError(), "vortex_branch_kernel launch");
}

static int launch_conv_args(const ConvArgs *args, int n, int nt, hipStream_t st, int arith)
{
    ConvGroup grp;
    for (int i = 0; i < n; ++i) grp.g[i] = args[i];
    for (int i = n; i < 4; ++i) grp.g[i] = args[0];
    grp.nblocks = 0;
    static const int mt_env = getenv("OJF_CONV_MT") ? atoi(getenv("OJF_CONV_MT")) : 0;
    const int mt = arith == OJF_ARITH_F16X3 ? (mt_env ? mt_env : (nt >= 6 ? 1 : 2)) : 1;
    const int strips = (args[0].npix + mt * 16 - 1) / (mt * 16);
    const dim3 grid((strips + 3) / 4, n), block(256);
#define OJF_LAUNCH32(NT_) hipLaunchKernelGGL((conv_mfma_kernel<1, NT_>), grid, block, 0, st, grp)
    int max_steps = 0;
    for (int i = 0; i < n; ++i) max_steps = args[i].nsteps > max_steps ? args[i].nsteps : max_steps;
    const size_t tab_bytes = (size_t)(max_steps + kPad16) * 8 * sizeof(int2);
    static const bool no_band = getenv("OJF_NO_XCD_BAND") != nullptr;
    dim3 grid16 = grid;
    if (arith == OJF_ARITH_F16X3 && !no_band && grid.x >= 64) {
        grp.nblocks = (int)grid.x;
        grid16.x = round_up((int)grid.x, 8);
    }
    static const bool no_perm = getenv("OJF_CONV_ROW_PERM") && atoi(getenv("OJF_CONV_ROW_PERM")) == 0;
    if (grp.nblocks && !no_perm)
        for (int i = 0; i < n; ++i) {
            ConvArgs &g = grp.g[i];
            if (g.taps == 9 && g.dil > 1 && g.dil < g.h && g.w % (mt * 16) == 0) {
                g.row_perm = g.dil; g.perm_q = g.h / g.dil; g.perm_rem = g.h % g.dil;
            }
        }
    static const int persist_bpc = getenv("OJF_CONV_PERSIST") ? atoi(getenv("OJF_CONV_PERSIST")) : 3;
    if (grp.nblocks && persist_bpc > 0 && arith == OJF_ARITH_F16X3) {
        bool single = true;
        for (int i = 0; i < n; ++i) single = single && args[i].nsteps <= conv16_chunk(nt);
        const int cus = device_cu_count();
        const int n8 = round_up(grp.nblocks, 8);
        int G = cus > 0 ? (cus * persist_bpc / n) / 8 * 8 : 0;
        if (single && G >= 8 && G < n8) {
            grp.band = n8 / 8;
            grid16.x = (unsigned)G;
        }
    }
    static const bool no_lean = getenv("OJF_CONV_LEAN") && atoi(getenv("OJF_CONV_LEAN")) == 0;
    bool lean = arith == OJF_ARITH_F16X3 && !no_lean;
    for (int i = 0; i < n && lean; ++i) lean = conv_lean_ok(args[i]);
    int n_ins = 0, n_outs = 0;
    for (int i = 0; i < n; ++i) { n_ins += args[i].in_split ? 1 : 0; n_outs += args[i].out_split ? 1 : 0; }
    if ((n_ins || n_outs) && (arith != OJF_ARITH_F16X3 || (n_ins && (n_ins != n || mt != 2 || nt != 2))))
        return fail("conv: split planes are a format of the split-fp16 grouped 3x3 launches only");
#define OJF_LAUNCH16(MT_, NT_)                                                                                      \
    do {                                                                                                             \
        if (lean) hipLaunchKernelGGL((conv_f16x3_kernel<MT_, NT_, true, 0, true>), grid16, block, tab_bytes, st, grp); \
        else hipLaunchKernelGGL((conv_f16x3_kernel<MT_, NT_>), grid16, block, tab_bytes, st, grp);                   \
    } while (0)
    if (arith == OJF_ARITH_F16X3 && mt == 2) {
        switch (nt) {
            case 2:
                if (n_ins && lean) hipLaunchKernelGGL((conv_f16x3_kernel<2, 2, true, 0, true, true>), grid16, block, tab_bytes, st, grp);
                else if (n_ins) hipLaunchKernelGGL((conv_f16x3_kernel<2, 2, true, 0, false, true>), grid16, block, tab_bytes, st, grp);
                else OJF_LAUNCH16(2, 2);
                break;
            case 4: OJF_LAUNCH16(2, 4); break;
            case 6: OJF_LAUNCH16(2, 6); break;
            case 8: OJF_LAUNCH16(2, 8); break;
            default: return fail("conv: unsupported number of output tiles");
        }
    } else if (arith == OJF_ARITH_F16X3) {
        switch (nt) {
            case 2: OJF_LAUNCH16(1, 2); break;
            case 4: OJF_LAUNCH16(1, 4); break;
            case 6: OJF_LAUNCH16(1, 6); break;
            case 8: OJF_LAUNCH16(1, 8); break;
            default: return fail("conv: unsupported number of output tiles");
        }
    } else {
        static const bool no_lds32 = getenv("OJF_CONV32_LDS") && atoi(getenv("OJF_CONV32_LDS")) == 0;
        switch (nt) {
            case 2: OJF_LAUNCH32(2); break;
            case 4: OJF_LAUNCH32(4); break;
            case 6:
                if (no_lds32) OJF_LAUNCH32(6);
                else hipLaunchKernelGGL((conv_mfma_lds_kernel<6>), grid, block, 0, st, grp);
                break;
            case 8:
                if (no_lds32) OJF_LAUNCH32(8);
                else hipLaunchKernelGGL((conv_mfma_lds_kernel<8>), grid, block, 0, st, grp);
                break;
            default: return fail("conv: unsupported number of output tiles");
        }
    }
#undef OJF_LAUNCH32
#undef OJF_LAUNCH16
    mark_launch(arith == OJF_ARITH_F16X3 ? (n > 1 ? "conv_f16x3_kernel (grouped)" : "conv_f16x3_kernel") : "conv_mfma_kernel", st);
    return check_hip(hipGetLastError(), "conv kernel launch");
}

static unsigned div_magic(int d, uint64_t limit)
{
    if (d <= 1 || limit * (uint64_t)d >= (1ull << 32)) return 0;
    return (unsigned)(((1ull << 32) + (uint64_t)d - 1) / (uint64_t)d);
}

static void fill_conv_args(ConvArgs &a, const PackedConv &pc, const float *in, int in_g0, float *out, int out_g0,
                           const float *bias, int act, int act_n, float scale, int h, int w)
{
    a.ovf = pc.arith == OJF_ARITH_F16X3 ? overflow_flag() : nullptr;
    a.accum = 0; a.dscale = nullptr;
    a.in = planes(in); a.out = planes(out); a.out_rows = nullptr;
    a.wp = planes(pc.wp); a.bias = bias ? bias : pc.bias; a.rinv = pc.rinv;
    a.in_g0 = in_g0; a.out_g0 = out_g0; a.rows_stride = 0; a.rows_n = 0;
    a.h = h; a.w = w; a.npix = h * w;
    a.taps = pc.taps; a.dil = pc.dil;
    a.c4 = pc.c_in_phys / 4; a.nsteps = pc.nsteps;
    a.w_magic = div_magic(w, (uint64_t)h * w);
    a.c4_magic = div_magic(a.c4, (uint64_t)(pc.nsteps + kPad16) * 8);
    a.og_store = round_up(pc.c_out_phys, 4) / 4;
    a.act = act; a.act_n = act_n; a.scale = scale;
}

static int launch_conv(const PackedConv &pc, const float *in, int in_g0, float *out, int out_g0, const float *bias,
                       int act, int act_n, float scale, int h, int w, hipStream_t st, float *rows = nullptr,
                       int rows_stride = 0, int rows_n = 0)
{
    ConvArgs a;
    fill_conv_args(a, pc, in, in_g0, out, out_g0, bias, act, act_n, scale, h, w);
    a.out_rows = rows; a.rows_stride = rows_stride; a.rows_n = rows_n;
    return launch_conv_args(&a, 1, pc.n_ot, st, pc.arith);
}

static std::vector<int> slot_map(int n_logical, int group, int slot)
{
    std::vector<int> m(n_logical);
    for (int j = 0; j < n_logical; ++j) m[j] = (j / group) * slot + (j % group);
    return m;
}

template <class F>
static std::vector<float> chain_row_scales(int arith, int nt_out, int n_k, F weight)
{
    std::vector<float> r((size_t)nt_out * 16, 1.0f);
    if (arith != OJF_ARITH_F16X3) return r;
    for (int oc = 0; oc < nt_out * 16; ++oc) {
        float mx = 0.0f;
        for (int k = 0; k < n_k; ++k) mx = std::fmax(mx, std::fabs(weight(oc, k)));
        r[oc] = row_scale(mx);
    }
    return r;
}

template <class F>
static void pack_chain_layer(std::vector<float> &dst, int arith, int nt_out, int nt_in, const std::vector<float> &rs, F weight)
{
    const size_t base = dst.size();
    dst.resize(base + (size_t)chain_layer_size(arith, nt_in, nt_out) * 4, 0.0f);
    if (arith == OJF_ARITH_F16X3) {
        const int KB = chain_kblocks(arith, nt_in);
        _Float16 *hp = reinterpret_cast<_Float16 *>(dst.data() + base);
        for (int n2 = 0; n2 < nt_out; ++n2)
            for (int S = 0; S < KB; ++S)
                for (int lane = 0; lane < 64; ++lane)
                    for (int j = 0; j < 8; ++j) {
                        const int oc = n2 * 16 + (lane & 15), g = lane >> 4;
                        const int k = 32 * S + (j < 4 ? 4 * g + j : 16 + 4 * g + (j - 4));
                        const size_t ub = ((size_t)n2 * KB + S) * 2 * 64 * 8;
                        split_weight(rs[oc] * weight(oc, k), hp[ub + (size_t)lane * 8 + j], hp[ub + 64 * 8 + (size_t)lane * 8 + j]);
                    }
    } else {
        for (int n2 = 0; n2 < nt_out; ++n2)
            for (int S = 0; S < nt_in; ++S)
                for (int lane = 0; lane < 64; ++lane)
                    for (int j = 0; j < 4; ++j)
                        dst[base + (((size_t)n2 * nt_in + S) * 64 + lane) * 4 + j] =
                            weight(n2 * 16 + (lane & 15), 16 * S + 4 * (lane >> 4) + j);
    }
}

static void append_chain_bias(std::vector<float> &dst, int arith, int nt_out, int c_out, const float *bias_host,
                              const std::vector<float> &rs)
{
    const size_t bb = dst.size();
    dst.resize(bb + (size_t)chain_bias_stride(arith, nt_out), 0.0f);
    for (int o = 0; o < c_out; ++o) dst[bb + o] = bias_host[o];
    if (arith == OJF_ARITH_F16X3)
        for (int o = 0; o < nt_out * 16; ++o) dst[bb + (size_t)nt_out * 16 + o] = 1.0f / rs[o];
}

struct Vortex {
    int c_in = 0, c_in_phys = 0;
    PackedConv stacked, b3a[4], b3b[4], b1[4], fin;
    float *pool_bias[4] = {nullptr, nullptr, nullptr, nullptr};
    float *Wg = nullptr, *bg = nullptr, *Wfg = nullptr, *bf = nullptr, *bias_final = nullptr;
    float *tail_w = nullptr, *tail_b1 = nullptr, *tail_rinv = nullptr;
    float *entry_w = nullptr, *entry_b = nullptr;
    int entry_ntin = 8;
    float *entry_wh[2] = {nullptr, nullptr}, *entry_bh[2] = {nullptr, nullptr}, *bias0 = nullptr;
    PackedBranches branches;
};

}

struct ojf_net {
    int version, P, c, cs, gf, sem, heads, h, w, npix;
    int arith;
    int pool_in, os;
    float scale;
    int64_t macs_per_pixel;
    int last_launches = 0;
    std::vector<ojf::PackedConv> dense[2];
    std::vector<ojf::PackedPair> pairs[2];
    ojf::PackedChain chains[2];
    bool chain_dense = false;
    ojf::Vortex vortex[3];
    std::vector<ojf::PackedConv> pred;
    float *chain_w = nullptr, *chain_b = nullptr;
    int chain_kind = 0;
    float *X[2] = {nullptr, nullptr};
    struct Scratch {
        float *T = nullptr, *Z = nullptr, *Q1 = nullptr, *Q2 = nullptr, *Q3 = nullptr, *U = nullptr, *V = nullptr;
        float *Q0 = nullptr;
        float *partial = nullptr;
        ojf::ColSums *colsum = nullptr;
        float *CAT = nullptr;
        hipStream_t side = nullptr;
        hipEvent_t ev_fork = nullptr, ev_join = nullptr, ev_entry = nullptr;
    } sc[2];
    hipStream_t head1 = nullptr;
    hipStream_t head_paired_with = nullptr;
    bool head_paired = false;
    hipEvent_t ev_head_fork = nullptr, ev_head_join = nullptr;
    ojf::ColSums *colsum3 = nullptr;
    float *YY = nullptr;
    float *Y3 = nullptr;
    float *PA = nullptr, *PB = nullptr;
    hipStream_t cap = nullptr;
    hipGraph_t graph = nullptr;
    hipGraphExec_t gexec = nullptr;
    float *g_est = nullptr;
    int g_stride = 0;
    bool use_graph = false;
};

namespace ojf {

constexpr size_t kPrefix = 64;

static int alloc_planes(float **p, size_t npix, int ch)
{
    float *raw = nullptr;
    OJF_HIP(hipMalloc(reinterpret_cast<void **>(&raw), (npix * ch + kPrefix) * sizeof(float)));
    OJF_HIP(hipMemset(raw, 0, (npix * ch + kPrefix) * sizeof(float)));
    OJF_HIP(hipStreamSynchronize(nullptr));
    *p = raw + kPrefix;
    return 0;
}

static void free_planes(float *p)
{
    if (p) (void)hipFree(p - kPrefix);
}

static int ensure_planes(float **p, size_t npix, int ch)
{
    return *p ? 0 : alloc_planes(p, npix, ch);
}

static int build_vortex(ojf_net *net, Vortex &v, const ojf_conv_layer *L, int c_in, const std::vector<int> &in_map,
                        int c_in_phys)
{
    const int c = net->c, cs = net->cs, out = net->pool_in, os = net->os;
    v.c_in = c_in;
    v.c_in_phys = c_in_phys;
    for (int i = 0; i < 18; ++i) {
        const bool k3 = (i >= 1 && i <= 16) && ((i - 1) % 4 == 1 || (i - 1) % 4 == 2);
        if (L[i].ksize != (k3 ? 3 : 1)) return fail("ojf_net_create: unexpected kernel size in a VortexPooling layer");
    }
    if (L[0].c_in != c_in || L[0].c_out != out || L[17].c_in != 5 * out || L[17].c_out != out)
        return fail("ojf_net_create: VortexPooling layer shapes do not match the topology");
    {
        ConvBuilder b(c_in_phys, 4 * cs, 1, 1);
        for (int br = 0; br < 4; ++br) {
            const ojf_conv_layer &l = L[1 + 4 * br];
            if (l.c_in != c_in || l.c_out != c) return fail("ojf_net_create: branch entry conv shape mismatch");
            b.add(l, 0, c_in, in_map, br * cs, br == 0);
            if (br > 0) {
                std::vector<float> pb(cs, 0.0f);
                for (int o = 0; o < c; ++o) pb[o] = l.bias_host[o];
                if (upload(pb, &v.pool_bias[br])) return -2;
            }
        }
        if (finish(b, v.stacked, net->arith)) return -2;
        static const bool no_wide_entry = getenv("OJF_NO_WIDE_ENTRY") != nullptr;
        if ((c_in_phys <= 128 || (c_in_phys <= 256 && !no_wide_entry)) && 4 * cs <= 80) {
            v.entry_ntin = c_in_phys <= 128 ? 8 : 16;
            auto we = [&](int oc, int k) { return oc < 4 * cs && k < c_in_phys ? b.W[(size_t)oc * c_in_phys + k] : 0.0f; };
            const std::vector<float> re = chain_row_scales(net->arith, 5, c_in_phys, we);
            std::vector<float> ew, eb;
            pack_chain_layer(ew, net->arith, 5, v.entry_ntin, re, we);
            append_chain_bias(eb, net->arith, 5, 4 * cs, b.B.data(), re);
            if (upload(ew, &v.entry_w) || upload(eb, &v.entry_b)) return -2;
            static const bool no_half = getenv("OJF_NO_HALF_ENTRY") != nullptr;
            if (v.entry_ntin == 16 && c_in_phys == 2 * net->os && !no_half) {
                const std::vector<float> zero_bias(4 * cs, 0.0f);
                for (int hd = 0; hd < 2; ++hd) {
                    auto wh = [&](int oc, int k) { return oc < 4 * cs && k < net->os ? b.W[(size_t)oc * c_in_phys + hd * net->os + k] : 0.0f; };
                    const std::vector<float> rh = chain_row_scales(net->arith, 5, net->os, wh);
                    std::vector<float> hw, hb;
                    pack_chain_layer(hw, net->arith, 5, 8, rh, wh);
                    append_chain_bias(hb, net->arith, 5, 4 * cs, zero_bias.data(), rh);
                    if (upload(hw, &v.entry_wh[hd]) || upload(hb, &v.entry_bh[hd])) return -2;
                }
                std::vector<float> b0(cs, 0.0f);
                for (int o = 0; o < cs; ++o) b0[o] = b.B[o];
                if (upload(b0, &v.bias0)) return -2;
            }
        }
    }
    const std::vector<int> id_c = slot_map(c, c, cs);
    std::vector<ConvBuilder> bas, bbs;
    for (int br = 0; br < 4; ++br) {
        const ojf_conv_layer &la = L[2 + 4 * br], &lb = L[3 + 4 * br], &l1 = L[4 + 4 * br];
        if (la.c_in != c || la.c_out != c || lb.c_in != c || lb.c_out != c || l1.c_in != c || l1.c_out != out)
            return fail("ojf_net_create: branch conv shape mismatch");
        ConvBuilder ba(cs, cs, 3, la.dilation), bb(cs, cs, 3, lb.dilation), b1(cs, os, 1, 1);
        ba.add(la, 0, c, id_c, 0, true);
        bb.add(lb, 0, c, id_c, 0, true);
        b1.add(l1, 0, c, id_c, 0, true);
        if (finish(ba, v.b3a[br], net->arith) || finish(bb, v.b3b[br], net->arith) || finish(b1, v.b1[br], net->arith)) return -2;
        bas.push_back(ba);
        bbs.push_back(bb);
    }
    if (net->arith == OJF_ARITH_F16X3 && cs == 4 * kChainNG && v.entry_w && bas[0].dil == bbs[0].dil && bas[1].dil == bbs[1].dil &&
        bas[2].dil == bbs[2].dil && bas[3].dil == bbs[3].dil && finish_branches(bas, bbs, net->h, net->w, v.branches))
        return -2;
    {
        const ojf_conv_layer &lf = L[17];
        ConvBuilder b(4 * os, os, 1, 1);
        b.add(lf, out, 5 * out, slot_map(4 * out, out, os), 0, false);
        if (finish(b, v.fin, net->arith)) return -2;
        std::vector<float> Wg((size_t)out * c_in_phys, 0.0f), bg(out), Wfg((size_t)out * out), bf(out);
        for (int o = 0; o < out; ++o) {
            for (int ci = 0; ci < c_in; ++ci) Wg[(size_t)in_map[ci] * out + o] = L[0].weight_host[(size_t)o * c_in + ci];
            bg[o] = L[0].bias_host[o];
            for (int j = 0; j < out; ++j) Wfg[(size_t)j * out + o] = lf.weight_host[(size_t)o * 5 * out + j];
            bf[o] = lf.bias_host[o];
        }
        if (upload(Wg, &v.Wg) || upload(bg, &v.bg) || upload(Wfg, &v.Wfg) || upload(bf, &v.bf)) return -2;
        std::vector<float> zero((size_t)v.fin.n_ot * 16, 0.0f);
        if (upload(zero, &v.bias_final)) return -2;
    }
    if ((cs + 15) / 16 == 2 && (os + 15) / 16 == 8) {
        const int NV = 2, NO = 8;
        std::vector<float> tw, tb;
        const ojf_conv_layer &lf = L[17];
        const std::vector<float> rf = chain_row_scales(net->arith, NO, 4 * out, [&](int oc, int k) {
            return oc < out ? lf.weight_host[(size_t)oc * 5 * out + out + k] : 0.0f;
        });
        for (int br = 0; br < 4; ++br) {
            const ojf_conv_layer &l1 = L[4 + 4 * br];
            auto w1 = [&](int oc, int k) { return oc < out && k < c ? l1.weight_host[(size_t)oc * c + k] : 0.0f; };
            const std::vector<float> r1 = chain_row_scales(net->arith, NO, c, w1);
            pack_chain_layer(tw, net->arith, NO, NV, r1, w1);
            pack_chain_layer(tw, net->arith, NO, NO, rf, [&](int oc, int k) {
                return oc < out && k < out ? lf.weight_host[(size_t)oc * 5 * out + out * (br + 1) + k] : 0.0f;
            });
            append_chain_bias(tb, net->arith, NO, out, l1.bias_host, r1);
        }
        std::vector<float> rfi(rf.size());
        for (size_t i = 0; i < rf.size(); ++i) rfi[i] = 1.0f / rf[i];
        if (upload(rfi, &v.tail_rinv)) return -2;
        if (upload(tw, &v.tail_w) || upload(tb, &v.tail_b1)) return -2;
    }
    return 0;
}

static void free_vortex(Vortex &v)
{
    release(v.stacked);
    release(v.fin);
    for (int b = 0; b < 4; ++b) {
        release(v.b3a[b]);
        release(v.b3b[b]);
        release(v.b1[b]);
        if (v.pool_bias[b]) (void)hipFree(v.pool_bias[b]);
    }
    release(v.branches);
    float *ptrs[] = {v.Wg, v.bg, v.Wfg, v.bf, v.bias_final, v.tail_w, v.tail_b1, v.tail_rinv, v.entry_w, v.entry_b,
                     v.entry_wh[0], v.entry_wh[1], v.entry_bh[0], v.entry_bh[1], v.bias0};
    for (float *p : ptrs)
        if (p) (void)hipFree(p);
}

static GaveArgs gave_args(const ojf_net *net, const Vortex &v, const float *partial, int nparts, int pstride, ColSums *fixed = nullptr)
{
    GaveArgs ga;
    ga.partial = partial; ga.fixed = fixed; ga.nparts = nparts; ga.pstride = pstride; ga.cphys = v.c_in_phys; ga.npix = net->npix;
    ga.WgT = v.Wg; ga.bg = v.bg; ga.WfgT = v.Wfg; ga.bf = v.bf; ga.c_out = net->pool_in;
    ga.bias_out = v.bias_final; ga.bias_len = v.fin.n_ot * 16;
    return ga;
}

static int chain_blocks(const ojf_net *net) { return ((net->npix + 15) / 16 + ojf::kChainWaves - 1) / ojf::kChainWaves; }

static int run_vortex(ojf_net *net, Vortex &v, const float *in, int in_g0, float *out, int out_g0, hipStream_t st,
                      ojf_net::Scratch &sc, const ChainArgs *head = nullptr, bool *head_done = nullptr,
                      bool entry_done = false, const Vortex *next = nullptr, bool *next_done = nullptr, bool in_split = false,
                      int half = -1, ColSums *next_colsum = nullptr, const float *z2 = nullptr)
{
    const int h = net->h, w = net->w, c4 = net->cs / 4, o4 = net->os / 4;
    const bool h16 = net->arith == OJF_ARITH_F16X3;
    static const bool legacy_env = getenv("OJF_LEGACY_VORTEX") != nullptr;
    const bool chain_flow = v.entry_w && v.tail_w && !legacy_env;
    static const bool no_split = getenv("OJF_CONV_SPLIT") && atoi(getenv("OJF_CONV_SPLIT")) == 0;
    const bool split = h16 && chain_flow && !no_split;
    if (in_split && (!chain_flow || entry_done)) return fail("run_vortex: internal error (split-plane input without the entry kernel)");
    if (!chain_flow) {
        if (entry_done) return fail("run_vortex: internal error (entry planes without the chain flow)");
        OJF_HIP(hipEventRecord(sc.ev_fork, st));
        OJF_HIP(hipStreamWaitEvent(sc.side, sc.ev_fork, 0));
        hipLaunchKernelGGL(colsum_kernel, dim3(kSumBlocks, v.c_in_phys / 4), dim3(256), 0, sc.side, planes(in), in_g0,
                           net->npix, sc.partial);
        mark_launch("colsum_kernel", sc.side);
        OJF_HIP(hipGetLastError());
        hipLaunchKernelGGL(gave_bias_kernel, dim3(1), dim3(256), 0, sc.side, gave_args(net, v, sc.partial, kSumBlocks, 256));
        mark_launch("gave_bias_kernel", sc.side);
        OJF_HIP(hipGetLastError());
        if (launch_conv(v.stacked, in, in_g0, sc.Z, 0, nullptr, OJF_ACT_RELU, net->cs, 1.0f, h, w, st)) return -2;
        OJF_HIP(hipEventRecord(sc.ev_entry, st));
    } else if (!entry_done) {
        ChainArgs ea;
        ea.in = planes(in); ea.w = planes(v.entry_w); ea.bias = v.entry_b; ea.out_rows = nullptr;
        ea.in_g0 = in_g0; ea.c4_in = v.c_in_phys / 4; ea.npix = net->npix; ea.rows_stride = 0; ea.rows_n = 0; ea.scale = 1.0f;
        ea.ovf = h16 ? overflow_flag() : nullptr;
        ea.out_planes = planes(sc.Z); ea.out_g0 = 0; ea.og_store = 4 * c4; ea.act_n = net->cs; ea.colsum = sc.colsum;
        ea.split_groups = split ? c4 : 0;
        ea.in_split = in_split ? 1 : 0;
        const dim3 grid(chain_blocks(net)), block(ojf::kChainThreads);
        if (v.entry_ntin == 16 && h16) hipLaunchKernelGGL((entry1x1_kernel<OJF_ARITH_F16X3, 1, 16, 5>), grid, block, 0, st, ea);
        else if (v.entry_ntin == 16) hipLaunchKernelGGL((entry1x1_kernel<OJF_ARITH_F32, 1, 16, 5>), grid, block, 0, st, ea);
        else if (h16) hipLaunchKernelGGL((entry1x1_kernel<OJF_ARITH_F16X3, 1, 8, 5>), grid, block, 0, st, ea);
        else hipLaunchKernelGGL((entry1x1_kernel<OJF_ARITH_F32, 1, 8, 5>), grid, block, 0, st, ea);
        mark_launch("entry1x1_kernel", st);
        OJF_HIP(hipGetLastError());
    }
    {
        PyramidArgs pa;
        pa.z = planes(sc.Z);
        pa.q[0] = planes(sc.Q1); pa.q[1] = planes(sc.Q2); pa.q[2] = planes(sc.Q3);
        for (int b = 0; b < 3; ++b) pa.bias[b] = v.pool_bias[b + 1];
        pa.h = h; pa.w = w; pa.c4 = c4;
        pa.tiles = ((w + kPoolTW - 1) / kPoolTW) * ((h + kPoolTH - 1) / kPoolTH);
        pa.gave = gave_args(net, v, nullptr, 0, 0, (z2 && net->colsum3) ? net->colsum3 : sc.colsum);
        pa.fold_gave = chain_flow ? 1 : 0;
        pa.split_out = split ? 1 : 0;
        if (z2) {
            if (!entry_done || !chain_flow || !sc.Q0 || !v.bias0) return fail("run_vortex: internal error (partial entry sums without the chain flow)");
            pa.z2 = planes(z2); pa.q0 = planes(sc.Q0); pa.bias0 = v.bias0;
        }
        hipLaunchKernelGGL(pool_pyramid_kernel, dim3(round_up(pa.tiles + (chain_flow ? 1 : 0), 8), (z2 ? 4 : 3) * c4), dim3(256), 0, st, pa);
        mark_launch("pool_pyramid_kernel", st);
        OJF_HIP(hipGetLastError());
    }
    const float *bin[4] = {z2 ? sc.Q0 : sc.Z, sc.Q1, sc.Q2, sc.Q3};
    static const bool unfused = getenv("OJF_NO_TAIL") != nullptr;
    const bool fused = v.tail_w && !unfused;
    static const bool branch_kernel = getenv("OJF_BRANCH_KERNEL") != nullptr && atoi(getenv("OJF_BRANCH_KERNEL")) != 0;
    static const bool subconv = getenv("OJF_SUBCONV") != nullptr && atoi(getenv("OJF_SUBCONV")) != 0;
    if (split && v.branches.n_items && branch_kernel) {
        if (launch_branches(v.branches, bin, sc.V, h, w, st)) return -2;
    } else if (split && v.branches.n_sub && subconv) {
        float *u[4], *vv[4];
        const float *uc[4];
        for (int br = 0; br < 4; ++br) {
            u[br] = sc.U + (size_t)br * c4 * 4 * net->npix;
            uc[br] = u[br];
            vv[br] = sc.V + (size_t)br * c4 * 4 * net->npix;
        }
        if (launch_subconv(v.branches, bin, u, 0, true, h, w, st)) return -2;
        if (launch_subconv(v.branches, uc, vv, 1, false, h, w, st)) return -2;
    } else {
        ConvArgs ga[4], gb[4];
        for (int br = 0; br < 4; ++br) {
            fill_conv_args(ga[br], v.b3a[br], bin[br], 0, sc.U, br * c4, nullptr, OJF_ACT_RELU, net->cs, 1.0f, h, w);
            fill_conv_args(gb[br], v.b3b[br], sc.U, br * c4, sc.V, br * c4, nullptr, OJF_ACT_RELU, net->cs, 1.0f, h, w);
            ga[br].in_split = ga[br].out_split = gb[br].in_split = split ? 1 : 0;
        }
        static const bool b0_main = getenv("OJF_BRANCH0_MAIN") != nullptr;
        if (chain_flow || b0_main || net->npix < 32768) {
            if (launch_conv_args(ga, 4, v.b3a[0].n_ot, st, net->arith)) return -2;
            if (launch_conv_args(gb, 4, v.b3b[0].n_ot, st, net->arith)) return -2;
        } else {
            OJF_HIP(hipStreamWaitEvent(sc.side, sc.ev_entry, 0));
            if (launch_conv_args(ga, 1, v.b3a[0].n_ot, sc.side, net->arith)) return -2;
            if (launch_conv_args(gb, 1, v.b3b[0].n_ot, sc.side, net->arith)) return -2;
            if (launch_conv_args(ga + 1, 3, v.b3a[1].n_ot, st, net->arith)) return -2;
            if (launch_conv_args(gb + 1, 3, v.b3b[1].n_ot, st, net->arith)) return -2;
        }
    }
    if (!chain_flow) {
        OJF_HIP(hipEventRecord(sc.ev_join, sc.side));
        OJF_HIP(hipStreamWaitEvent(st, sc.ev_join, 0));
    }
    if (!fused) {
        if (ensure_planes(&sc.CAT, (size_t)net->npix, 4 * net->os)) return -2;
        for (int br = 0; br < 4; ++br)
            if (launch_conv(v.b1[br], sc.V, br * c4, sc.CAT, br * o4, nullptr, OJF_ACT_RELU, net->os, 1.0f, h, w, st))
                return -2;
    }
    if (!fused) return launch_conv(v.fin, sc.CAT, 0, out, out_g0, v.bias_final, OJF_ACT_NONE, 0, 1.0f, h, w, st);
    TailArgs ta;
    for (int br = 0; br < 4; ++br) ta.v[br] = planes(sc.V) + (size_t)br * c4 * net->npix;
    ta.w = planes(v.tail_w); ta.b1 = v.tail_b1; ta.bias_final = v.bias_final; ta.rinv_final = v.tail_rinv;
    ta.out = planes(out); ta.c4 = c4; ta.out_g0 = out_g0; ta.og_store = o4; ta.npix = net->npix;
    ta.ovf = h16 ? overflow_flag() : nullptr;
    ta.chain_w = nullptr; ta.chain_b = nullptr; ta.out_rows = nullptr; ta.rows_stride = 0; ta.rows_n = 0; ta.scale = 1.0f;
    ta.entry_w = nullptr; ta.entry_b = nullptr; ta.entry_out = nullptr; ta.entry_og = 0; ta.entry_act_n = 0; ta.colsum = nullptr; ta.entry_split = 0;
    const dim3 grid(chain_blocks(net)), block(ojf::kChainThreads);
    static const bool no_head_fusion = getenv("OJF_NO_HEAD_FUSION") != nullptr;
    static const bool no_entry_fusion = getenv("OJF_NO_ENTRY_FUSION") != nullptr;
    if (head && net->chain_kind && !no_head_fusion) {
        ta.chain_w = head->w; ta.chain_b = head->bias; ta.out_rows = head->out_rows;
        ta.rows_stride = head->rows_stride; ta.rows_n = head->rows_n; ta.scale = head->scale;
        if (net->chain_kind == 19 && h16) hipLaunchKernelGGL((vortex_tail_kernel<OJF_ARITH_F16X3, 1, 2, 8, 19>), grid, block, 0, st, ta);
        else if (net->chain_kind == 19) hipLaunchKernelGGL((vortex_tail_kernel<OJF_ARITH_F32, 1, 2, 8, 19>), grid, block, 0, st, ta);
        else if (h16) hipLaunchKernelGGL((vortex_tail_kernel<OJF_ARITH_F16X3, 1, 2, 8, 20>), grid, block, 0, st, ta);
        else hipLaunchKernelGGL((vortex_tail_kernel<OJF_ARITH_F32, 1, 2, 8, 20>), grid, block, 0, st, ta);
        mark_launch("vortex_tail_kernel (+ prediction head)", st);
        if (head_done) *head_done = true;
    } else if (chain_flow && next && half >= 0 && half < 2 && next->entry_wh[half] && next->tail_w && next_colsum && !legacy_env && !no_entry_fusion) {
        ta.entry_w = planes(next->entry_wh[half]); ta.entry_b = next->entry_bh[half]; ta.entry_out = planes(sc.Z);
        ta.entry_og = 4 * c4; ta.entry_act_n = 0; ta.colsum = next_colsum; ta.colsum_off = half * net->os;
        ta.entry_split = 0;
        if (h16) hipLaunchKernelGGL((vortex_tail_kernel<OJF_ARITH_F16X3, 1, 2, 8, kTailEntry>), grid, block, 0, st, ta);
        else hipLaunchKernelGGL((vortex_tail_kernel<OJF_ARITH_F32, 1, 2, 8, kTailEntry>), grid, block, 0, st, ta);
        mark_launch("vortex_tail_kernel (+ half of the next entry GEMM)", st);
        if (next_done) *next_done = true;
    } else if (chain_flow && next && next->entry_w && next->tail_w && next->c_in_phys == net->os && !legacy_env && !no_entry_fusion) {
        ta.entry_w = planes(next->entry_w); ta.entry_b = next->entry_b; ta.entry_out = planes(sc.Z);
        ta.entry_og = 4 * c4; ta.entry_act_n = net->cs; ta.colsum = sc.colsum;
        ta.entry_split = (h16 && !no_split) ? c4 : 0;
        if (h16) hipLaunchKernelGGL((vortex_tail_kernel<OJF_ARITH_F16X3, 1, 2, 8, kTailEntry>), grid, block, 0, st, ta);
        else hipLaunchKernelGGL((vortex_tail_kernel<OJF_ARITH_F32, 1, 2, 8, kTailEntry>), grid, block, 0, st, ta);
        mark_launch("vortex_tail_kernel (+ next entry GEMM)", st);
        if (next_done) *next_done = true;
    } else if (h16) {
        hipLaunchKernelGGL((vortex_tail_kernel<OJF_ARITH_F16X3, 1, 2, 8>), grid, block, 0, st, ta);
        mark_launch("vortex_tail_kernel", st);
    } else {
        hipLaunchKernelGGL((vortex_tail_kernel<OJF_ARITH_F32, 1, 2, 8>), grid, block, 0, st, ta);
        mark_launch("vortex_tail_kernel", st);
    }
    return check_hip(hipGetLastError(), "vortex_tail_kernel launch");
}

static int run_dense(ojf_net *net, int head, hipStream_t st)
{
    const int c4 = net->cs / 4;
    float *T = net->sc[head].T;
    static const bool no_pair = getenv("OJF_NO_PAIR") != nullptr;
    if (net->chain_dense) return launch_chain(net->chains[head], net->X[head], net->h, net->w, st);
    if (!no_pair && (int)net->pairs[head].size() == net->gf) {
        for (int i = 0; i < net->gf; ++i)
            if (launch_pair(net->pairs[head][i], net->X[head], 0, net->X[head], (i + 1) * c4, net->h, net->w, st)) return -2;
        return 0;
    }
    for (int i = 0; i < net->gf; ++i) {
        if (launch_conv(net->dense[head][2 * i], net->X[head], 0, T, 0, nullptr, OJF_ACT_LEAKY, net->cs, 1.0f,
                        net->h, net->w, st)) return -2;
        if (launch_conv(net->dense[head][2 * i + 1], T, 0, net->X[head], (i + 1) * c4, nullptr, OJF_ACT_LEAKY,
                        net->cs, 1.0f, net->h, net->w, st)) return -2;
    }
    return 0;
}

static int layer_count(int version, int gf, int sem)
{
    const int pred = 2 * (gf - 1) + 3;
    if (version == 3) return (sem ? 2 : 1) * (2 * gf + 18) + 18 + pred;
    if (version == 2) return 2 * gf + 18 + 18 + pred;
    return -1;
}

}

OJF_API int ojf_net_layer_count(int version, int n_points, int growth, int use_semantics)
{
    if (n_points < 1 || growth < 1) return -1;
    return ojf::layer_count(version, growth, use_semantics ? 1 : 0);
}

namespace ojf { static void drop_graph(ojf_net *net); }

OJF_API void ojf_net_destroy(ojf_net *net)
{
    using namespace ojf;
    if (!net) return;
    for (int hd = 0; hd < 2; ++hd) {
        for (auto &pc : net->dense[hd]) release(pc);
        for (auto &pp : net->pairs[hd]) release(pp);
        release(net->chains[hd]);
    }
    for (auto &pc : net->pred) release(pc);
    for (auto &v : net->vortex) free_vortex(v);
    float *bufs[] = {net->X[0], net->X[1], net->YY, net->Y3, net->PA, net->PB};
    for (float *p : bufs) free_planes(p);
    for (auto &sc : net->sc) {
        float *sb[] = {sc.T, sc.Z, sc.Q0, sc.Q1, sc.Q2, sc.Q3, sc.U, sc.V, sc.partial, sc.CAT};
        if (sc.colsum) (void)hipFree(sc.colsum);
        for (float *p : sb) free_planes(p);
        if (sc.ev_fork) (void)hipEventDestroy(sc.ev_fork);
        if (sc.ev_join) (void)hipEventDestroy(sc.ev_join);
        if (sc.ev_entry) (void)hipEventDestroy(sc.ev_entry);
        if (sc.side) (void)hipStreamDestroy(sc.side);
    }
    if (net->colsum3) (void)hipFree(net->colsum3);
    if (net->ev_head_fork) (void)hipEventDestroy(net->ev_head_fork);
    if (net->ev_head_join) (void)hipEventDestroy(net->ev_head_join);
    if (net->head1) (void)hipStreamDestroy(net->head1);
    drop_graph(net);
    if (net->cap) (void)hipStreamDestroy(net->cap);
    if (net->chain_w) (void)hipFree(net->chain_w);
    if (net->chain_b) (void)hipFree(net->chain_b);
    delete net;
}

OJF_API int ojf_net_create(ojf_net **out, int version, int n_points, int growth, int use_semantics, float output_scale,
                           const ojf_conv_layer *L, int n_layers, int h, int w)
{
    using namespace ojf;
    if (!out || !L) return fail("ojf_net_create: null pointer argument");
    *out = nullptr;
    if (version != 2 && version != 3) return fail("ojf_net_create: version must be 2 or 3");
    if (n_points < 1 || growth < 1 || h <= 0 || w <= 0) return fail("ojf_net_create: bad sizes");
    const int sem = use_semantics ? 1 : 0;
    if (n_layers != layer_count(version, growth, sem)) return fail("ojf_net_create: wrong number of folded layers");
    for (int i = 0; i < n_layers; ++i)
        if (!L[i].weight_host || !L[i].bias_host || (L[i].ksize != 1 && L[i].ksize != 3) || L[i].dilation < 1)
            return fail("ojf_net_create: malformed layer descriptor");
    for (int i = 0; i < n_layers; ++i) {
        const size_t nw = (size_t)L[i].c_out * L[i].c_in * L[i].ksize * L[i].ksize;
        for (size_t k = 0; k < nw; ++k)
            if (!std::isfinite(L[i].weight_host[k])) return fail("ojf_net_create: non-finite weight");
        for (int k = 0; k < L[i].c_out; ++k)
            if (!std::isfinite(L[i].bias_host[k])) return fail("ojf_net_create: non-finite bias");
    }

    ojf_net *net = new ojf_net();
    net->version = version; net->P = n_points; net->gf = growth; net->sem = sem;
    net->arith = g_default_arith;
    net->c = 2 * n_points + 1 + (version == 2 ? sem : 0);
    net->cs = round_up(net->c, 4);
    net->heads = (version == 3 && sem) ? 2 : 1;
    net->h = h; net->w = w; net->npix = h * w;
    net->pool_in = net->c * (growth + 1);
    net->os = round_up(net->pool_in, 4);
    net->scale = output_scale;
    const int c = net->c, cs = net->cs, gf = growth, os = net->os;
    if (net->heads * os > 256 || (gf + 1) * cs > 256) { delete net; return fail("ojf_net_create: topology too wide"); }
    net->macs_per_pixel = 0;
    for (int i = 0; i < n_layers; ++i) net->macs_per_pixel += (int64_t)L[i].c_in * L[i].c_out * L[i].ksize * L[i].ksize;

    int rc = 0;
    int li = 0;
    auto build_dense = [&](int head) -> int {
        std::vector<ConvBuilder> bas, bbs;
        for (int i = 0; i < gf; ++i) {
            const ojf_conv_layer &la = L[li++], &lb = L[li++];
            if (la.ksize != 3 || lb.ksize != 3 || la.c_in != (i + 1) * c || la.c_out != c || lb.c_in != c || lb.c_out != c)
                return fail("ojf_net_create: dense block layer shape mismatch");
            ConvBuilder ba((i + 1) * cs, cs, 3, la.dilation), bb(cs, cs, 3, lb.dilation);
            ba.add(la, 0, (i + 1) * c, slot_map((i + 1) * c, c, cs), 0, true);
            bb.add(lb, 0, c, slot_map(c, c, cs), 0, true);
            PackedConv pa, pb;
            if (finish(ba, pa, net->arith) || finish(bb, pb, net->arith)) return -2;
            net->dense[head].push_back(pa);
            net->dense[head].push_back(pb);
            if (net->arith == OJF_ARITH_F16X3 && cs <= 24) {
                PackedPair pp;
                if (finish_pair(ba, bb, pp, pair_cfg_for(net->h, net->w, cs))) return -2;
                net->pairs[head].push_back(pp);
                bas.push_back(ba);
                bbs.push_back(bb);
            }
        }
        if ((int)bas.size() == gf && cs == 4 * kChainNG && gf <= kChainMaxLayers && finish_chain(bas, bbs, net->chains[head])) return -2;
        return 0;
    };
    const std::vector<int> dense_map = slot_map(net->pool_in, c, cs);
    const std::vector<int> flat_map = slot_map(net->pool_in, net->pool_in, os);
    if (version == 3) {
        rc = build_dense(0);
        if (!rc) { rc = build_vortex(net, net->vortex[0], L + li, net->pool_in, dense_map, (gf + 1) * cs); li += 18; }
        if (!rc && sem) {
            rc = build_dense(1);
            if (!rc) { rc = build_vortex(net, net->vortex[1], L + li, net->pool_in, dense_map, (gf + 1) * cs); li += 18; }
        }
        if (!rc) {
            rc = build_vortex(net, net->vortex[2], L + li, net->heads * net->pool_in,
                              slot_map(net->heads * net->pool_in, net->pool_in, os), net->heads * os);
            li += 18;
        }
    } else {
        rc = build_dense(0);
        if (!rc) { rc = build_vortex(net, net->vortex[0], L + li, net->pool_in, dense_map, (gf + 1) * cs); li += 18; }
        if (!rc) { rc = build_vortex(net, net->vortex[2], L + li, net->pool_in, flat_map, os); li += 18; }
    }
    if (!rc) {
        int prev_phys = os;
        for (; li < n_layers; ++li) {
            const ojf_conv_layer &l = L[li];
            if (l.ksize != 1) { rc = fail("ojf_net_create: prediction head must be 1x1 convolutions"); break; }
            if (round_up(l.c_in, 4) != prev_phys) { rc = fail("ojf_net_create: prediction head shapes do not chain"); break; }
            ConvBuilder b(prev_phys, round_up(l.c_out, 4), 1, 1);
            b.add(l, 0, l.c_in, slot_map(l.c_in, l.c_in, prev_phys), 0, true);
            PackedConv pc;
            if (finish(b, pc, net->arith)) { rc = -2; break; }
            net->pred.push_back(pc);
            prev_phys = round_up(l.c_out, 4);
        }
    }
    if (!rc && n_points == 9 && growth == 5 && (c == 19 || c == 20)) {
        const int first = n_layers - (2 * (gf - 1) + 3);
        std::vector<float> cw, cb;
        int prev_phys = os;
        for (int l = first; l < n_layers; ++l) {
            const ojf_conv_layer &ly = L[l];
            const int nt_in = (prev_phys + 15) / 16, out_phys = round_up(ly.c_out, 4), nt_out = (out_phys + 15) / 16;
            auto wl = [&](int oc, int k) { return oc < ly.c_out && k < ly.c_in ? ly.weight_host[(size_t)oc * ly.c_in + k] : 0.0f; };
            const std::vector<float> rs = chain_row_scales(net->arith, nt_out, ly.c_in, wl);
            pack_chain_layer(cw, net->arith, nt_out, nt_in, rs, wl);
            append_chain_bias(cb, net->arith, nt_out, ly.c_out, ly.bias_host, rs);
            prev_phys = out_phys;
        }
        if (upload(cw, &net->chain_w) || upload(cb, &net->chain_b)) rc = -2;
        else net->chain_kind = c;
    }
    if (!rc) {
        int idx = 0;
        auto skip_dense = [&]() { idx += 2 * gf; };
        auto sub_gave = [&]() { net->macs_per_pixel -= (int64_t)L[idx].c_in * L[idx].c_out; idx += 18; };
        skip_dense(); sub_gave();
        if (version == 3 && sem) { skip_dense(); sub_gave(); }
        sub_gave();
    }
    if (!rc) {
        static const bool no_chain = getenv("OJF_NO_DENSE_CHAIN") != nullptr || getenv("OJF_LEGACY_VORTEX") != nullptr ||
                                     getenv("OJF_NO_PAIR") != nullptr;
        bool ok = net->arith == OJF_ARITH_F16X3 && !no_chain;
        {
            const int big = ((w + 19) / 20) * ((h + 15) / 16);
            const int tiles = big >= 200 ? big : ((w + 11) / 12) * ((h + 7) / 8);
            if (tiles > kChainSyncInts - kChainFlags0 || (w % 8) != 0) ok = false;
        }
        for (int hd = 0; hd < net->heads && ok; ++hd)
            ok = net->chains[hd].layers == gf && net->vortex[hd].entry_w && net->vortex[hd].tail_w;
        net->chain_dense = ok;
    }
    const size_t np = (size_t)net->npix;
    if (!rc) rc = alloc_planes(&net->X[0], np, (gf + 1) * cs);
    if (!rc && net->heads == 2) rc = alloc_planes(&net->X[1], np, (gf + 1) * cs);
    for (int hd = 0; hd < net->heads && !rc; ++hd) {
        ojf_net::Scratch &sc = net->sc[hd];
        rc = alloc_planes(&sc.T, np, cs);
        if (!rc) rc = alloc_planes(&sc.Z, np, 4 * cs);
        if (!rc && hd == 0 && net->heads == 2) rc = alloc_planes(&sc.Q0, np, cs);
        if (!rc) rc = alloc_planes(&sc.Q1, np, cs);
        if (!rc) rc = alloc_planes(&sc.Q2, np, cs);
        if (!rc) rc = alloc_planes(&sc.Q3, np, cs);
        if (!rc) rc = alloc_planes(&sc.U, np, 4 * cs);
        if (!rc) rc = alloc_planes(&sc.V, np, 4 * cs);
        if (!rc) rc = alloc_planes(&sc.partial, kSumBlocks, 256);
        if (!rc) rc = check_hip(hipMalloc(reinterpret_cast<void **>(&sc.colsum), sizeof(ColSums)), "hipMalloc");
        if (!rc) rc = check_hip(hipMemset(sc.colsum, 0, sizeof(ColSums)), "hipMemset");
        if (!rc && hd == 0 && net->heads == 2) {
            rc = check_hip(hipMalloc(reinterpret_cast<void **>(&net->colsum3), sizeof(ColSums)), "hipMalloc");
            if (!rc) rc = check_hip(hipMemset(net->colsum3, 0, sizeof(ColSums)), "hipMemset");
            if (!rc) rc = check_hip(hipStreamSynchronize(nullptr), "hipStreamSynchronize");
        }
        if (!rc) rc = check_hip(hipStreamSynchronize(nullptr), "hipStreamSynchronize");
        if (!rc) rc = check_hip(hipStreamCreateWithFlags(&sc.side, hipStreamNonBlocking), "hipStreamCreate");
        if (!rc) rc = check_hip(hipEventCreateWithFlags(&sc.ev_fork, event_flags()), "hipEventCreate");
        if (!rc) rc = check_hip(hipEventCreateWithFlags(&sc.ev_join, event_flags()), "hipEventCreate");
        if (!rc) rc = check_hip(hipEventCreateWithFlags(&sc.ev_entry, event_flags()), "hipEventCreate");
    }
    if (!rc && net->heads == 2) {
        rc = check_hip(hipStreamCreateWithFlags(&net->head1, hipStreamNonBlocking), "hipStreamCreate");
        if (!rc) rc = check_hip(hipEventCreateWithFlags(&net->ev_head_fork, event_flags()), "hipEventCreate");
        if (!rc) rc = check_hip(hipEventCreateWithFlags(&net->ev_head_join, event_flags()), "hipEventCreate");
    }
    if (!rc) rc = alloc_planes(&net->YY, np, net->heads * os);
    if (!rc) rc = alloc_planes(&net->Y3, np, os);
    if (!rc) rc = check_hip(hipStreamCreateWithFlags(&net->cap, hipStreamNonBlocking), "hipStreamCreate");
    {
        const char *g = getenv("OJF_NET_GRAPH");
        net->use_graph = g && g[0] == '1';
    }
    if (rc) {
        const std::string keep = ojf_last_error();
        ojf_net_destroy(net);
        set_error(keep);
        return rc;
    }
    *out = net;
    return 0;
}

namespace ojf {
int net_input_slot(::ojf_net *net, NetInputSlot *slot)
{
    if (!net || !slot || net->sem || net->heads != 1) return 1;
    slot->x0 = net->X[0]; slot->cs4 = net->cs / 4; slot->P = net->P; slot->h = net->h; slot->w = net->w;
    slot->ovf = net->arith == OJF_ARITH_F16X3 ? overflow_flag() : nullptr;
    slot->split = net->chain_dense ? 1 : 0;
    return 0;
}
}

OJF_API int ojf_net_prepare_input(ojf_net *net, const float *values, const float *weights, int rows_stride,
                                  int in_layout, const float *depth, const uint8_t *sem_ids, int n_classes, ojf_stream_t stream)
{
    using namespace ojf;
    if (!net || !values || !weights || !depth) return fail("ojf_net_prepare_input: null pointer argument");
    if (in_layout != 0 && in_layout != 1) return fail("ojf_net_prepare_input: in_layout must be 0 or 1");
    if (in_layout == 0 && rows_stride < net->P) return fail("ojf_net_prepare_input: rows_stride < n_points");
    if (in_layout == 1 && rows_stride < net->npix) return fail("ojf_net_prepare_input: plane stride < h*w");
    if (net->sem && (!sem_ids || n_classes <= 0))
        return fail("ojf_net_prepare_input: this net uses semantics: sem_ids and n_classes are required");
    PrepArgs a;
    a.values = values; a.weights = weights; a.depth = depth;
    a.sem = net->sem ? sem_ids : nullptr;
    a.x0 = planes(net->X[0]);
    a.x1 = net->heads == 2 ? planes(net->X[1]) : nullptr;
    a.rows_stride = rows_stride; a.in_layout = in_layout; a.npix = net->npix; a.P = net->P; a.cs4 = net->cs / 4;
    a.n_classes = n_classes;
    a.v2_sem = (net->version == 2 && net->sem) ? 1 : 0;
    a.ovf = net->arith == OJF_ARITH_F16X3 ? overflow_flag() : nullptr;
    a.split = net->chain_dense ? 1 : 0;
    hipLaunchKernelGGL(prepare_input_kernel, dim3((a.npix + 255) / 256), dim3(256), 0, as_stream(stream), a);
    return check_hip(hipGetLastError(), "prepare_input_kernel launch");
}

namespace ojf {

__global__ void spin_kernel(long long cycles)
{
    const long long t0 = (long long)__builtin_amdgcn_s_memtime();
    while ((long long)__builtin_amdgcn_s_memtime() - t0 < cycles) __builtin_amdgcn_s_sleep(32);
}

static double spin_pair_us(hipStream_t a, hipStream_t b, long long cycles)
{
    (void)hipStreamSynchronize(a);
    (void)hipStreamSynchronize(b);
    const auto t0 = std::chrono::steady_clock::now();
    hipLaunchKernelGGL(spin_kernel, dim3(1), dim3(64), 0, a, cycles);
    hipLaunchKernelGGL(spin_kernel, dim3(1), dim3(64), 0, a, 1LL);
    hipLaunchKernelGGL(spin_kernel, dim3(1), dim3(64), 0, b, cycles);
    (void)hipStreamSynchronize(a);
    (void)hipStreamSynchronize(b);
    return std::chrono::duration<double, std::micro>(std::chrono::steady_clock::now() - t0).count();
}

static void pair_stream(hipStream_t &s, const hipStream_t *others, int n, double alone, long long cycles, const char *what)
{
    static const bool dbg = getenv("OJF_DEBUG_STREAMS") != nullptr;
    std::vector<hipStream_t> rejected;
    for (int attempt = 0; attempt < 8; ++attempt) {
        double worst = 0.0;
        for (int k = 0; k < n; ++k) {
            const double both = spin_pair_us(others[k], s, cycles);
            worst = both > worst ? both : worst;
        }
        if (dbg) fprintf(stderr, "ojf: %s stream, attempt %d: one spin %.0f us, one per stream %.0f us\n", what, attempt, alone, worst);
        if (worst < 1.5 * alone) break;
        hipStream_t fresh = nullptr;
        if (hipStreamCreateWithFlags(&fresh, hipStreamNonBlocking) != hipSuccess) break;
        rejected.push_back(s);
        s = fresh;
    }
    for (hipStream_t r : rejected) (void)hipStreamDestroy(r);
}

}

OJF_API int ojf_streams_overlap(ojf_stream_t a, ojf_stream_t b)
{
    using namespace ojf;
    hipStream_t sa = as_stream(a), sb = as_stream(b);
    hipStreamCaptureStatus cs = hipStreamCaptureStatusNone;
    if (hipStreamIsCapturing(sa, &cs) != hipSuccess || cs != hipStreamCaptureStatusNone) return fail("ojf_streams_overlap: stream a is capturing");
    if (hipStreamIsCapturing(sb, &cs) != hipSuccess || cs != hipStreamCaptureStatusNone) return fail("ojf_streams_overlap: stream b is capturing");
    const long long cycles = 300000;
    (void)spin_pair_us(sa, sb, 1000);
    double alone = 1e30, both = 1e30;
    for (int rep = 0; rep < 2; ++rep) {
        const double t1 = spin_pair_us(sa, sa, cycles) * 0.5;
        const double t2 = spin_pair_us(sa, sb, cycles);
        alone = t1 < alone ? t1 : alone;
        both = t2 < both ? t2 : both;
    }
    if (hipGetLastError() != hipSuccess) return fail("ojf_streams_overlap: spin kernel launch failed");
    return both < 1.5 * alone ? 1 : 0;
}

namespace ojf {

static void pair_head_stream(ojf_net *net, hipStream_t st)
{
    if (net->heads != 2 || (net->head_paired && net->head_paired_with == st) || !net->head1) return;
    hipStreamCaptureStatus cs = hipStreamCaptureStatusNone;
    if (hipStreamIsCapturing(st, &cs) != hipSuccess || cs != hipStreamCaptureStatusNone) return;
    net->head_paired_with = st;
    net->head_paired = true;
    const long long cycles = 300000;
    (void)spin_pair_us(st, st, 1000);
    const double alone = spin_pair_us(st, st, cycles) * 0.5;
    pair_stream(net->head1, &st, 1, alone, cycles, "second head");
    if (net->sc[1].side) pair_stream(net->sc[1].side, &net->head1, 1, alone, cycles, "head 1 side");
    if (net->sc[0].side) pair_stream(net->sc[0].side, &st, 1, alone, cycles, "head 0 side");
}

static int forward_launches(ojf_net *net, float *est, int est_stride, hipStream_t st)
{
    const int o4 = net->os / 4;
    static const bool unfused = getenv("OJF_NO_CHAIN") != nullptr;
    ChainArgs ca;
    ca.in = planes(net->Y3); ca.w = planes(net->chain_w); ca.bias = net->chain_b;
    ca.out_rows = est; ca.in_g0 = 0; ca.c4_in = o4; ca.npix = net->npix;
    ca.rows_stride = est_stride; ca.rows_n = net->P; ca.scale = net->scale;
    ca.ovf = net->arith == OJF_ARITH_F16X3 ? overflow_flag() : nullptr;
    const ChainArgs *head = (net->chain_kind && !unfused) ? &ca : nullptr;
    bool head_done = false;
    static const bool serial_heads = getenv("OJF_SERIAL_HEADS") != nullptr;
    if (net->version == 3) {
        const bool two = net->heads == 2;
        if (two && !serial_heads) pair_head_stream(net, st);
        hipStream_t s1 = (two && !serial_heads) ? net->head1 : st;
        if (two && s1 != st) {
            OJF_HIP(hipEventRecord(net->ev_head_fork, st));
            OJF_HIP(hipStreamWaitEvent(s1, net->ev_head_fork, 0));
        }
        const bool halves = two && net->vortex[2].entry_wh[0] && net->vortex[2].entry_wh[1] && net->sc[0].Q0 && net->colsum3;
        bool done1 = false;
        if (two) {
            if (run_dense(net, 1, s1)) return -2;
            if (run_vortex(net, net->vortex[1], net->X[1], 0, net->YY, o4, s1, net->sc[1], nullptr, nullptr, false,
                           halves ? &net->vortex[2] : nullptr, &done1, net->chain_dense, halves ? 1 : -1, net->colsum3)) return -2;
        }
        if (run_dense(net, 0, st)) return -2;
        bool entry_done = false;
        if (run_vortex(net, net->vortex[0], net->X[0], 0, net->YY, 0, st, net->sc[0], nullptr, nullptr, false,
                       (two && !halves) ? nullptr : &net->vortex[2], &entry_done, net->chain_dense, halves ? 0 : -1, halves ? net->colsum3 : net->sc[0].colsum)) return -2;
        if (two && s1 != st) {
            OJF_HIP(hipEventRecord(net->ev_head_join, s1));
            OJF_HIP(hipStreamWaitEvent(st, net->ev_head_join, 0));
        }
        if (halves && entry_done != done1) return fail("ojf_net_forward: internal error (one head ran its half of the entry GEMM, the other did not)");
        if (run_vortex(net, net->vortex[2], net->YY, 0, net->Y3, 0, st, net->sc[0], head, &head_done, entry_done, nullptr, nullptr, false, -1,
                       nullptr, (halves && entry_done) ? net->sc[1].Z : nullptr)) return -2;
    } else {
        if (run_dense(net, 0, st)) return -2;
        bool entry_done = false;
        if (run_vortex(net, net->vortex[0], net->X[0], 0, net->YY, 0, st, net->sc[0], nullptr, nullptr, false, &net->vortex[2],
                       &entry_done, net->chain_dense)) return -2;
        if (run_vortex(net, net->vortex[2], net->YY, 0, net->Y3, 0, st, net->sc[0], head, &head_done, entry_done)) return -2;
    }
    if (head_done) return 0;
    if (net->chain_kind && !unfused) {
        const bool h16 = net->arith == OJF_ARITH_F16X3;
        const dim3 grid(chain_blocks(net)), block(ojf::kChainThreads);
        if (net->chain_kind == 19 && h16)
            hipLaunchKernelGGL((chain1x1_kernel<OJF_ARITH_F16X3, 1, 8, 6, 6, 5, 5, 4, 4, 3, 3, 2, 2, 1>), grid, block, 0, st, ca);
        else if (net->chain_kind == 19)
            hipLaunchKernelGGL((chain1x1_kernel<OJF_ARITH_F32, 1, 8, 6, 6, 5, 5, 4, 4, 3, 3, 2, 2, 1>), grid, block, 0, st, ca);
        else if (h16)
            hipLaunchKernelGGL((chain1x1_kernel<OJF_ARITH_F16X3, 1, 8, 7, 7, 5, 5, 4, 4, 3, 3, 2, 2, 1>), grid, block, 0, st, ca);
        else
            hipLaunchKernelGGL((chain1x1_kernel<OJF_ARITH_F32, 1, 8, 7, 7, 5, 5, 4, 4, 3, 3, 2, 2, 1>), grid, block, 0, st, ca);
        mark_launch("chain1x1_kernel", st);
        return check_hip(hipGetLastError(), "chain1x1_kernel launch");
    }
    const float *pin = net->Y3;
    const int np = (int)net->pred.size();
    if (ensure_planes(&net->PA, (size_t)net->npix, net->os) || ensure_planes(&net->PB, (size_t)net->npix, net->os)) return -2;
    float *pp[2] = {net->PA, net->PB};
    for (int i = 0; i < np; ++i) {
        const PackedConv &pc = net->pred[i];
        const bool last = (i == np - 1);
        if (last) {
            if (launch_conv(pc, pin, 0, nullptr, 0, nullptr, OJF_ACT_TANH, pc.n_ot * 16, net->scale, net->h, net->w, st,
                            est, est_stride, net->P)) return -2;
        } else {
            if (launch_conv(pc, pin, 0, pp[i & 1], 0, nullptr, OJF_ACT_LEAKY, pc.n_ot * 16, 1.0f, net->h, net->w, st))
                return -2;
            pin = pp[i & 1];
        }
    }
    return 0;
}

static void drop_graph(ojf_net *net)
{
    if (net->gexec) (void)hipGraphExecDestroy(net->gexec);
    if (net->graph) (void)hipGraphDestroy(net->graph);
    net->gexec = nullptr;
    net->graph = nullptr;
}

static void capture_graph(ojf_net *net, float *est, int est_stride)
{
    drop_graph(net);
    net->g_est = est;
    net->g_stride = est_stride;
    if (ensure_planes(&net->sc[0].CAT, (size_t)net->npix, 4 * net->os) ||
        (net->heads == 2 && ensure_planes(&net->sc[1].CAT, (size_t)net->npix, 4 * net->os)) ||
        ensure_planes(&net->PA, (size_t)net->npix, net->os) ||
        ensure_planes(&net->PB, (size_t)net->npix, net->os)) { net->use_graph = false; return; }
    if (hipStreamBeginCapture(net->cap, hipStreamCaptureModeThreadLocal) != hipSuccess) { net->use_graph = false; return; }
    const int rc = forward_launches(net, est, est_stride, net->cap);
    hipGraph_t g = nullptr;
    const hipError_t e = hipStreamEndCapture(net->cap, &g);
    if (rc || e != hipSuccess || !g || hipGraphInstantiate(&net->gexec, g, nullptr, nullptr, 0) != hipSuccess) {
        if (g) (void)hipGraphDestroy(g);
        net->gexec = nullptr;
        net->use_graph = false;
        (void)hipGetLastError();
        return;
    }
    net->graph = g;
}

}

OJF_API int ojf_net_forward(ojf_net *net, float *est, int est_stride, ojf_stream_t stream)
{
    using namespace ojf;
    if (!net || !est) return fail("ojf_net_forward: null pointer argument");
    if (est_stride < net->P) return fail("ojf_net_forward: est_stride < n_points");
    hipStream_t st = as_stream(stream);
    if (net->arith == OJF_ARITH_F16X3 && g_ovf_host && *g_ovf_host) return fail(*g_ovf_host == 2 ? kChainStuckMsg : kOverflowMsg);
    if (net->use_graph) {
        if (!net->gexec || net->g_est != est || net->g_stride != est_stride) capture_graph(net, est, est_stride);
        if (net->gexec) return check_hip(hipGraphLaunch(net->gexec, st), "hipGraphLaunch (net forward)");
    }
    const int before = g_launches;
    const int rc = forward_launches(net, est, est_stride, st);
    net->last_launches = g_launches - before;
    return rc;
}

OJF_API int64_t ojf_net_macs_per_pixel(const ojf_net *net) { return net ? net->macs_per_pixel : -1; }

OJF_API int ojf_net_launch_count(const ojf_net *net) { return net ? net->last_launches : -1; }

OJF_API int ojf_net_side_streams(ojf_net *net, ojf_stream_t stream, ojf_stream_t out[3])
{
    using namespace ojf;
    if (!net || !out) return fail("ojf_net_side_streams: null pointer argument");
    pair_head_stream(net, as_stream(stream));
    out[0] = net->heads == 2 ? reinterpret_cast<ojf_stream_t>(net->head1) : nullptr;
    out[1] = reinterpret_cast<ojf_stream_t>(net->sc[0].side);
    out[2] = net->heads == 2 ? reinterpret_cast<ojf_stream_t>(net->sc[1].side) : nullptr;
    return (out[0] != nullptr) + (out[1] != nullptr) + (out[2] != nullptr);
}

OJF_API int ojf_net_profile(ojf_net *net, float *est, int est_stride, ojf_stream_t stream, char *names, int names_cap,
                            float *micros, int max_entries)
{
    using namespace ojf;
    if (!net || !est || !names || !micros || names_cap < 1 || max_entries < 1) return fail("ojf_net_profile: bad argument");
    hipStream_t st = as_stream(stream);
    hipEvent_t e0 = nullptr;
    OJF_HIP(hipEventCreateWithFlags(&e0, hipEventDisableSystemFence));
    g_marks.clear();
    g_profile = true;
    (void)hipEventRecord(e0, st);
    const int rc = forward_launches(net, est, est_stride, st);
    g_profile = false;
    int n = 0;
    size_t used = 0;
    names[0] = 0;
    if (!rc && hipStreamSynchronize(st) == hipSuccess) {
        for (size_t i = 0; i < g_marks.size() && n < max_entries; ++i) {
            hipEvent_t prev = nullptr;
            for (size_t j = i; j-- > 0;)
                if (g_marks[j].st == g_marks[i].st) { prev = g_marks[j].ev; break; }
            if (!prev && g_marks[i].st == st) prev = e0;
            float ms = 0.0f;
            (void)hipEventSynchronize(g_marks[i].ev);
            if (!prev || hipEventElapsedTime(&ms, prev, g_marks[i].ev) != hipSuccess) ms = -1e-3f;
            const size_t len = strlen(g_marks[i].name);
            if (used + len + 2 > (size_t)names_cap) break;
            memcpy(names + used, g_marks[i].name, len);
            names[used + len] = '\n';
            used += len + 1;
            names[used] = 0;
            micros[n++] = ms * 1e3f;
        }
    }
    for (auto &m : g_marks) (void)hipEventDestroy(m.ev);
    g_marks.clear();
    (void)hipEventDestroy(e0);
    return rc ? rc : n;
}

OJF_API int ojf_net_set_arithmetic(int arithmetic)
{
    if (arithmetic != OJF_ARITH_F32 && arithmetic != OJF_ARITH_F16X3)
        return ojf::fail("ojf_net_set_arithmetic: unknown arithmetic (OJF_ARITH_F32 or OJF_ARITH_F16X3)");
    ojf::g_default_arith = arithmetic;
    return 0;
}

OJF_API int ojf_net_get_arithmetic(const ojf_net *net) { return net ? net->arith : ojf::g_default_arith; }

OJF_API int ojf_net_check(ojf_stream_t stream)
{
    using namespace ojf;
    OJF_HIP(hipStreamSynchronize(as_stream(stream)));
    if (const int what = guard_take(nullptr, true)) return fail(what == 2 ? kChainStuckMsg : kOverflowMsg);
    return 0;
}

OJF_API int ojf_guard_poll(void) { return ojf::g_ovf_host ? *ojf::g_ovf_host : 0; }

OJF_API int ojf_guard_status(ojf_stream_t stream, int *flag, int *skipped)
{
    using namespace ojf;
    OJF_HIP(hipStreamSynchronize(as_stream(stream)));
    const int what = guard_take(skipped, false);
    if (flag) *flag = what;
    return 0;
}

OJF_API int ojf_conv2d(const float *in, int in_stride, int in_off, float *out, int out_stride, int out_off,
                       const ojf_conv_layer *layer, int act, int h, int w, ojf_stream_t stream)
{
    using namespace ojf;
    if (!in || !out || !layer || !layer->weight_host || !layer->bias_host) return fail("ojf_conv2d: null pointer argument");
    if ((layer->ksize != 1 && layer->ksize != 3) || layer->dilation < 1) return fail("ojf_conv2d: 1x1 or 3x3 kernels only");
    const int cin_phys = round_up(layer->c_in, 4), cout_phys = round_up(layer->c_out, 4);
    if (in_off + layer->c_in > in_stride || out_off + cout_phys > out_stride)
        return fail("ojf_conv2d: channel window exceeds the row stride");
    hipStream_t st = as_stream(stream);
    const int npix = h * w;
    ConvBuilder b(cin_phys, cout_phys, layer->ksize, layer->dilation);
    b.add(*layer, 0, layer->c_in, slot_map(layer->c_in, layer->c_in, cin_phys), 0, true);
    PackedConv pc;
    if (finish(b, pc, g_default_arith)) return -2;
    float *pin = nullptr, *pout = nullptr;
    int rc = alloc_planes(&pin, npix, cin_phys);
    if (!rc) rc = alloc_planes(&pout, npix, cout_phys);
    if (!rc) {
        hipLaunchKernelGGL(rows_to_planes_kernel, dim3((npix * (cin_phys / 4) + 255) / 256), dim3(256), 0, st, in, in_stride,
                           in_off, layer->c_in, planes(pin), cin_phys / 4, npix);
        rc = launch_conv(pc, pin, 0, pout, 0, nullptr, act, cout_phys, 1.0f, h, w, st);
    }
    if (!rc) {
        hipLaunchKernelGGL(planes_to_rows_kernel, dim3((npix * (cout_phys / 4) + 255) / 256), dim3(256), 0, st,
                           planes(pout), cout_phys / 4, npix, out, out_stride, out_off);
        rc = check_hip(hipStreamSynchronize(st), "ojf_conv2d sync");
        if (!rc && guard_take(nullptr, true)) rc = fail(kOverflowMsg);
    }
    free_planes(pin);
    free_planes(pout);
    release(pc);
    return rc;
}

#include "ojf_net_train.h"
#include "ojf_train_net.h"
```

Baseline: 2610 frames/sec.

## Fold tail final 1x1 conv into the next consumer's first layer

Precomputes on the host the product of the vortex tail's final 1x1 projection weights and the following consumer's first layer (the prediction head's first layer or the next block's entry GEMM). The tail then accumulates directly into the narrower consumer width (5–7 tiles instead of 8), which removes one chained GEMM per pixel and the intermediate 8-tile activation. Column sums for the global-average bias are now taken on per-branch intermediates, and the bias is reconstructed through a transposed weight product in gave_bias_block. This adds host-side weight folding, widens ColSums to 512 columns, and changes the rounding path in f16x3. It also adds a waves_per_eu hint to the pool pyramid kernel.

```diff
diff --git a/online_joint_depthfusion_and_semantic_amd/csrc/ojf_net.hip b/online_joint_depthfusion_and_semantic_amd/csrc/ojf_net.hip
--- a/online_joint_depthfusion_and_semantic_amd/csrc/ojf_net.hip
+++ b/online_joint_depthfusion_and_semantic_amd/csrc/ojf_net.hip
@@ -894,7 +894,7 @@
 constexpr int kColShards = 16;
 constexpr float kColScale = 1048576.0f;
 
-constexpr int kColMax = 256;
+constexpr int kColMax = 512;
 struct ColSums {
     long long fix[kColShards][kColMax];
     unsigned bad[kColMax];
@@ -1007,6 +1007,7 @@
     struct ColSums *colsum;
     int entry_split;
     int colsum_off = 0;
+    const float *fold_b = nullptr;
 };
 
 constexpr int kTailEntry = 1;
@@ -1021,11 +1022,22 @@
 }
 constexpr int head_first_ntout(int kind) { return kind == 19 ? 6 : 7; }
 constexpr int head_first_size(int arith, int kind) { return chain_first_size(arith, 8, kind == 19 ? 6 : 7); }
-
-template <int ARITH, int MT, int NV, int NO, int CHAIN = 0>
+template <int ARITH, int MT, int KIND>
+__device__ __forceinline__ void head_run_from2(f32x4 (&x)[MT][8], f32x4 (&y)[MT][8], f32x4 *wlds, const f32x4 *wg, const float *bias,
+                                               const ChainArgs &a, const int (&p)[MT], int lane, f32x4 (&pre)[kChainPre], int &buf,
+                                               VecStage &vs)
+{
+    if constexpr (KIND == 19) chain_run<ARITH, MT, 6, 6, 5, 5, 4, 4, 3, 3, 2, 2, 1>(x, y, wlds, wg, bias, a, p, lane, pre, buf, vs);
+    else chain_run<ARITH, MT, 7, 7, 5, 5, 4, 4, 3, 3, 2, 2, 1>(x, y, wlds, wg, bias, a, p, lane, pre, buf, vs);
+}
+
+template <int ARITH, int MT, int NV, int NO, int CHAIN = 0, int NACC = NO>
 __global__ __launch_bounds__(kChainThreads, OJF_CHAIN_BLOCKS) void vortex_tail_kernel(const TailArgs a)
 {
     static_assert(CHAIN == 0 || NO == 8, "the fused prediction head / entry layer expects 8 input tiles");
+    constexpr bool FOLD = NACC != NO;
+    static_assert(!FOLD || NACC == (CHAIN == kTailEntry ? 5 : head_first_ntout(CHAIN)), "folded width of an unknown consumer");
+    constexpr int NW = FOLD ? NACC : NO;
     __shared__ f32x4 wlds[chain_dma(ARITH) ? 2 * kChainDmaHalf : kChainLdsFloat4];
     __shared__ f32x4 vec_lds[2 * kVecF4];
     __shared__ float red[CHAIN == kTailEntry ? kChainWaves * 128 : 1];
@@ -1035,7 +1047,7 @@
     int p[MT];
 #pragma unroll
     for (int m = 0; m < MT; ++m) p[m] = strip + m * 16 + i16;
-    constexpr int kVec1 = chain_bias_stride(ARITH, NO) / 4, kVecFin = NO * 4 * (ARITH == OJF_ARITH_F16X3 ? 2 : 1);
+    constexpr int kVec1 = chain_bias_stride(ARITH, NO) / 4, kVecFin = chain_bias_stride(ARITH, NW) / 4;
     VecStage vs;
     vs.lds = vec_lds; vs.half = 0;
     {
@@ -1062,7 +1074,10 @@
                 if ((int)threadIdx.x + kChainThreads * k < size0) pre[k] = a.w[threadIdx.x + kChainThreads * k];
         }
     }
-    constexpr size_t per_branch = (size_t)chain_layer_size(ARITH, NV, NO) + chain_layer_size(ARITH, NO, NO);
+    constexpr size_t per_branch = (size_t)chain_layer_size(ARITH, NV, NO) + chain_layer_size(ARITH, NO, NW);
+    constexpr int kHead2 = CHAIN != 0 && CHAIN != kTailEntry ? head_first_ntout(CHAIN) : 1;
+    constexpr int kNextFirst = FOLD ? (CHAIN == kTailEntry ? 0 : chain_first_size(ARITH, NACC, kHead2))
+                                    : (CHAIN == kTailEntry ? chain_first_size(ARITH, 8, 5) : (CHAIN ? head_first_size(ARITH, CHAIN) : 0));
     f32x4 t[MT][NO];
     const f32x4 *vfin = vec_lds;
 #pragma unroll
@@ -1080,46 +1095,90 @@
         VecNext nx;
         if (b < 3) {
             nx.a = a.b1 + (b + 1) * chain_bias_stride(ARITH, NO); nx.na = kVec1;
+        } else if constexpr (FOLD) {
+            nx.a = a.fold_b; nx.na = kVecFin;
         } else {
             nx.a = a.bias_final; nx.na = NO * 4;
             if constexpr (ARITH == OJF_ARITH_F16X3) { nx.b = a.rinv_final; nx.nb = NO * 4; }
         }
-        chain_layer<ARITH, MT, NV, NO, kChainRelu, chain_first_size(ARITH, NO, NO)>(vin, t, wlds, w1, ca, p, lane, pre, buf, vs, nx);
+        chain_layer<ARITH, MT, NV, NO, kChainRelu, chain_first_size(ARITH, NO, NW)>(vin, t, wlds, w1, ca, p, lane, pre, buf, vs, nx);
+        if constexpr (FOLD && CHAIN == kTailEntry) block_colsum<MT, NO>(t, p, a.npix, red, a.colsum, lane, wave, a.colsum_off + b * 128);
         if (b < 3) {
-            chain_layer<ARITH, MT, NO, NO, kChainAccumulate, chain_first_size(ARITH, NV, NO)>(t, y, wlds, wf, ca, p, lane, pre, buf, vs);
+            chain_layer<ARITH, MT, NO, NW, kChainAccumulate, chain_first_size(ARITH, NV, NO)>(t, y, wlds, wf, ca, p, lane, pre, buf, vs);
         } else {
             vfin = vs.lds + vs.half * kVecF4;
             VecNext nf;
-            if constexpr (CHAIN == kTailEntry) { nf.a = a.entry_b; nf.na = chain_bias_stride(ARITH, 5) / 4; }
-            else if constexpr (CHAIN != 0) { nf.a = a.chain_b; nf.na = chain_bias_stride(ARITH, head_first_ntout(CHAIN)) / 4; }
-            chain_layer<ARITH, MT, NO, NO, kChainAccumulate,
-                        CHAIN == kTailEntry ? chain_first_size(ARITH, 8, 5) : (CHAIN ? head_first_size(ARITH, CHAIN) : 0)>(
-                t, y, wlds, wf, ca, p, lane, pre, buf, vs, nf, CHAIN == kTailEntry ? a.entry_w : a.chain_w, kVecFin);
-        }
-    }
-    float gmax = 0.0f;
-#pragma unroll
-    for (int n = 0; n < NO; ++n) {
-        const int og = n * 4 + g;
-        const f32x4 bf = vfin[n * 4 + g];
-#pragma unroll
-        for (int m = 0; m < MT; ++m) {
-            f32x4 v = y[m][n] + bf;
-            if constexpr (ARITH == OJF_ARITH_F16X3) v = fma4(y[m][n], vfin[NO * 4 + n * 4 + g], bf);
-            if constexpr (ARITH == OJF_ARITH_F16X3) gmax = guard_max(gmax, v);
-            if constexpr (CHAIN) y[m][n] = v;
-            else if (p[m] < a.npix && og < a.og_store) a.out[(size_t)(a.out_g0 + og) * a.npix + p[m]] = v;
-        }
-    }
-    if constexpr (ARITH == OJF_ARITH_F16X3)
-        if (gmax > 65504.0f && a.ovf) guard_raise(a.ovf, 1);
-    if constexpr (CHAIN == kTailEntry) {
-        block_colsum<MT, NO>(y, p, a.npix, red, a.colsum, lane, wave, a.colsum_off);
-        ca.out_planes = a.entry_out; ca.out_g0 = 0; ca.og_store = a.entry_og; ca.act_n = a.entry_act_n; ca.split_groups = a.entry_split;
-        chain_layer<ARITH, MT, 8, 5, kChainEntry, 0>(y, t, wlds, a.entry_w, ca, p, lane, pre, buf, vs);
-    } else if constexpr (CHAIN) {
-        ca.out_rows = a.out_rows; ca.rows_stride = a.rows_stride; ca.rows_n = a.rows_n; ca.scale = a.scale;
-        head_run<ARITH, MT, CHAIN>(y, t, wlds, a.chain_w, a.chain_b, ca, p, lane, pre, buf, vs);
+            const f32x4 *next_w = CHAIN == kTailEntry ? a.entry_w : a.chain_w;
+            if constexpr (FOLD && CHAIN != kTailEntry) {
+                nf.a = a.chain_b + chain_bias_stride(ARITH, NACC); nf.na = chain_bias_stride(ARITH, kHead2) / 4;
+                next_w = a.chain_w + chain_layer_size(ARITH, 8, NACC);
+            } else if constexpr (FOLD) {
+                next_w = nullptr;
+            } else if constexpr (CHAIN == kTailEntry) {
+                nf.a = a.entry_b; nf.na = chain_bias_stride(ARITH, 5) / 4;
+            } else if constexpr (CHAIN != 0) {
+                nf.a = a.chain_b; nf.na = chain_bias_stride(ARITH, head_first_ntout(CHAIN)) / 4;
+            }
+            chain_layer<ARITH, MT, NO, NW, kChainAccumulate, kNextFirst>(t, y, wlds, wf, ca, p, lane, pre, buf, vs, nf, next_w, kVecFin);
+        }
+    }
+    if constexpr (FOLD) {
+        float gmax = 0.0f;
+#pragma unroll
+        for (int n = 0; n < NACC; ++n) {
+            const int og = n * 4 + g;
+            const f32x4 bz = vfin[n * 4 + g];
+            f32x4 ri{1.f, 1.f, 1.f, 1.f};
+            if constexpr (ARITH == OJF_ARITH_F16X3) ri = vfin[(NACC + n) * 4 + g];
+#pragma unroll
+            for (int m = 0; m < MT; ++m) {
+                const f32x4 lin4 = ARITH == OJF_ARITH_F16X3 ? fma4(y[m][n], ri, bz) : y[m][n] + bz;
+                if constexpr (CHAIN == kTailEntry) {
+                    f32x4 v = lin4;
+#pragma unroll
+                    for (int j = 0; j < 4; ++j) v[j] = (og * 4 + j < a.entry_act_n && !(v[j] > 0.0f)) ? (v[j] != v[j] ? v[j] : 0.0f) : v[j];
+                    if (p[m] < a.npix && og < a.entry_og) {
+                        a.entry_out[(size_t)og * a.npix + p[m]] = og < a.entry_split ? split_pack4(v) : v;
+                        if constexpr (ARITH == OJF_ARITH_F16X3) gmax = guard_max(gmax, lin4);
+                    }
+                } else {
+                    if constexpr (ARITH == OJF_ARITH_F16X3) gmax = guard_max(gmax, lin4);
+                    y[m][n] = leaky_max4(lin4, 0.01f);
+                }
+            }
+        }
+        if constexpr (ARITH == OJF_ARITH_F16X3)
+            if (gmax > 65504.0f && a.ovf) guard_raise(a.ovf, 1);
+        if constexpr (CHAIN != kTailEntry) {
+            ca.out_rows = a.out_rows; ca.rows_stride = a.rows_stride; ca.rows_n = a.rows_n; ca.scale = a.scale;
+            head_run_from2<ARITH, MT, CHAIN>(y, t, wlds, a.chain_w + chain_layer_size(ARITH, 8, NACC), a.chain_b + chain_bias_stride(ARITH, NACC),
+                                             ca, p, lane, pre, buf, vs);
+        }
+    } else {
+        float gmax = 0.0f;
+#pragma unroll
+        for (int n = 0; n < NO; ++n) {
+            const int og = n * 4 + g;
+            const f32x4 bf = vfin[n * 4 + g];
+#pragma unroll
+            for (int m = 0; m < MT; ++m) {
+                f32x4 v = y[m][n] + bf;
+                if constexpr (ARITH == OJF_ARITH_F16X3) v = fma4(y[m][n], vfin[NO * 4 + n * 4 + g], bf);
+                if constexpr (ARITH == OJF_ARITH_F16X3) gmax = guard_max(gmax, v);
+                if constexpr (CHAIN) y[m][n] = v;
+                else if (p[m] < a.npix && og < a.og_store) a.out[(size_t)(a.out_g0 + og) * a.npix + p[m]] = v;
+            }
+        }
+        if constexpr (ARITH == OJF_ARITH_F16X3)
+            if (gmax > 65504.0f && a.ovf) guard_raise(a.ovf, 1);
+        if constexpr (CHAIN == kTailEntry) {
+            block_colsum<MT, NO>(y, p, a.npix, red, a.colsum, lane, wave, a.colsum_off);
+            ca.out_planes = a.entry_out; ca.out_g0 = 0; ca.og_store = a.entry_og; ca.act_n = a.entry_act_n; ca.split_groups = a.entry_split;
+            chain_layer<ARITH, MT, 8, 5, kChainEntry, 0>(y, t, wlds, a.entry_w, ca, p, lane, pre, buf, vs);
+        } else if constexpr (CHAIN) {
+            ca.out_rows = a.out_rows; ca.rows_stride = a.rows_stride; ca.rows_n = a.rows_n; ca.scale = a.scale;
+            head_run<ARITH, MT, CHAIN>(y, t, wlds, a.chain_w, a.chain_b, ca, p, lane, pre, buf, vs);
+        }
     }
 }
 
@@ -1131,6 +1190,10 @@
     int c_out;
     float *bias_out;
     int bias_len;
+    const float *foldT = nullptr, *fold_add = nullptr;
+    float *fold_out = nullptr;
+    int fold_n = 0;
+    const float *WtT = nullptr, *prev_bias = nullptr;
 };
 
 struct PyramidArgs {
@@ -1207,12 +1270,12 @@
 
 __device__ __forceinline__ void gave_bias_block(const GaveArgs &a, float *mean, float *gv);
 
-__global__ __launch_bounds__(256) void pool_pyramid_kernel(const PyramidArgs a)
+__global__ __launch_bounds__(256) __attribute__((amdgpu_waves_per_eu(8))) void pool_pyramid_kernel(const PyramidArgs a)
 {
     __shared__ f32x4 buf[2][kPoolStride * (kPoolTH + 6)];
     if (banded_block_x() >= a.tiles) {
         if (blockIdx.y == 0 && banded_block_x() == a.tiles && a.fold_gave)
-            gave_bias_block(a.gave, reinterpret_cast<float *>(buf), reinterpret_cast<float *>(buf) + 256);
+            gave_bias_block(a.gave, reinterpret_cast<float *>(buf), reinterpret_cast<float *>(buf) + kColMax);
         return;
     }
     const int yg = blockIdx.y / a.c4, cg = blockIdx.y - yg * a.c4;
@@ -1263,17 +1326,36 @@
 {
     const int t = threadIdx.x;
     if (a.fixed) {
-        if (t < kColMax) {
+        const int ncol = a.WtT ? 4 * 128 : a.cphys;
+#pragma unroll 1
+        for (int ch = t; ch < kColMax; ch += 256) {
             long long q = 0;
 #pragma unroll
             for (int sh = 0; sh < kColShards; ++sh) {
-                q += a.fixed->fix[sh][t];
-                a.fixed->fix[sh][t] = 0;
+                q += a.fixed->fix[sh][ch];
+                a.fixed->fix[sh][ch] = 0;
             }
-            const bool bad = a.fixed->bad[t] != 0;
-            a.fixed->bad[t] = 0;
+            const bool bad = a.fixed->bad[ch] != 0;
+            a.fixed->bad[ch] = 0;
             const float sum = (float)((double)q * (1.0 / (double)kColScale));
-            mean[t] = t < a.cphys ? (bad ? __builtin_nanf("") : sum / (float)a.npix) : 0.0f;
+            mean[ch] = ch < ncol ? (bad ? __builtin_nanf("") : sum / (float)a.npix) : 0.0f;
+        }
+        if (a.WtT) {
+            __syncthreads();
+            const int o = t & 127, hb = t >> 7;
+            float s = 0.0f;
+            if (o < a.c_out)
+#pragma unroll 1
+                for (int b = 2 * hb; b < 2 * hb + 2; ++b) {
+                    const float *wt = a.WtT + (size_t)b * a.c_out * a.c_out;
+#pragma unroll 8
+                    for (int k = 0; k < a.c_out; ++k) s = __builtin_fmaf(wt[(size_t)k * a.c_out + o], mean[b * 128 + k], s);
+                }
+            gv[t] = s;
+            __syncthreads();
+            const float my = t < a.cphys && t < a.c_out ? a.prev_bias[t] + (gv[t] + gv[128 + t]) : 0.0f;
+            __syncthreads();
+            mean[t] = my;
         }
     } else if (a.cphys <= 128) {
         const int ch = t & 127, half = t >> 7;
@@ -1312,12 +1394,18 @@
             for (int j = 0; j < a.c_out; ++j) s = __builtin_fmaf(a.WfgT[(size_t)j * a.c_out + t], gv[j], s);
         }
         a.bias_out[t] = s;
+    } else if (t - a.bias_len < a.fold_n) {
+        const int o = t - a.bias_len;
+        float z = a.fold_add[o];
+#pragma unroll 8
+        for (int j = 0; j < a.c_out; ++j) z = __builtin_fmaf(a.foldT[(size_t)j * a.fold_n + o], gv[j], z);
+        a.fold_out[o] = z;
     }
 }
 
 __global__ __launch_bounds__(256) void gave_bias_kernel(const GaveArgs a)
 {
-    __shared__ float mean[256];
+    __shared__ float mean[kColMax];
     __shared__ float gv[256];
     gave_bias_block(a, mean, gv);
 }
@@ -2240,6 +2328,13 @@
     float *entry_w = nullptr, *entry_b = nullptr;
     int entry_ntin = 8;
     float *entry_wh[2] = {nullptr, nullptr}, *entry_bh[2] = {nullptr, nullptr}, *bias0 = nullptr;
+    std::vector<float> entry_host_w, entry_host_b;
+    int fold_into = 0, fold_nacc = 0;
+    float *fold_w = nullptr;
+    float *fold_b = nullptr;
+    float *fold_MT = nullptr, *fold_add = nullptr;
+    float *WtT = nullptr;
+    const Vortex *fold_next = nullptr;
     PackedBranches branches;
 };
 
@@ -2310,6 +2405,22 @@
     return *p ? 0 : alloc_planes(p, npix, ch);
 }
 
+template <class F>
+static void pack_tail(std::vector<float> &tw, std::vector<float> &tb, std::vector<float> &rf, const ojf_net *net, const ojf_conv_layer *L,
+                      int nt, F fb)
+{
+    const int NV = 2, NO = 8, c = net->c, out = net->pool_in;
+    rf = chain_row_scales(net->arith, nt, 4 * out, [&](int oc, int k) { return fb(k / out, oc, k % out); });
+    for (int br = 0; br < 4; ++br) {
+        const ojf_conv_layer &l1 = L[4 + 4 * br];
+        auto w1 = [&](int oc, int k) { return oc < out && k < c ? l1.weight_host[(size_t)oc * c + k] : 0.0f; };
+        const std::vector<float> r1 = chain_row_scales(net->arith, NO, c, w1);
+        pack_chain_layer(tw, net->arith, NO, NV, r1, w1);
+        pack_chain_layer(tw, net->arith, nt, NO, rf, [&](int oc, int k) { return fb(br, oc, k); });
+        append_chain_bias(tb, net->arith, NO, out, l1.bias_host, r1);
+    }
+}
+
 static int build_vortex(ojf_net *net, Vortex &v, const ojf_conv_layer *L, int c_in, const std::vector<int> &in_map,
                         int c_in_phys)
 {
@@ -2344,6 +2455,8 @@
             pack_chain_layer(ew, net->arith, 5, v.entry_ntin, re, we);
             append_chain_bias(eb, net->arith, 5, 4 * cs, b.B.data(), re);
             if (upload(ew, &v.entry_w) || upload(eb, &v.entry_b)) return -2;
+            v.entry_host_w = b.W;
+            v.entry_host_b = b.B;
             static const bool no_half = getenv("OJF_NO_HALF_ENTRY") != nullptr;
             if (v.entry_ntin == 16 && c_in_phys == 2 * net->os && !no_half) {
                 const std::vector<float> zero_bias(4 * cs, 0.0f);
@@ -2395,27 +2508,59 @@
         if (upload(zero, &v.bias_final)) return -2;
     }
     if ((cs + 15) / 16 == 2 && (os + 15) / 16 == 8) {
-        const int NV = 2, NO = 8;
-        std::vector<float> tw, tb;
         const ojf_conv_layer &lf = L[17];
-        const std::vector<float> rf = chain_row_scales(net->arith, NO, 4 * out, [&](int oc, int k) {
-            return oc < out ? lf.weight_host[(size_t)oc * 5 * out + out + k] : 0.0f;
+        std::vector<float> tw, tb, rf;
+        pack_tail(tw, tb, rf, net, L, 8, [&](int br, int oc, int k) {
+            return oc < out && k < out ? lf.weight_host[(size_t)oc * 5 * out + out * (br + 1) + k] : 0.0f;
         });
-        for (int br = 0; br < 4; ++br) {
-            const ojf_conv_layer &l1 = L[4 + 4 * br];
-            auto w1 = [&](int oc, int k) { return oc < out && k < c ? l1.weight_host[(size_t)oc * c + k] : 0.0f; };
-            const std::vector<float> r1 = chain_row_scales(net->arith, NO, c, w1);
-            pack_chain_layer(tw, net->arith, NO, NV, r1, w1);
-            pack_chain_layer(tw, net->arith, NO, NO, rf, [&](int oc, int k) {
-                return oc < out && k < out ? lf.weight_host[(size_t)oc * 5 * out + out * (br + 1) + k] : 0.0f;
-            });
-            append_chain_bias(tb, net->arith, NO, out, l1.bias_host, r1);
-        }
         std::vector<float> rfi(rf.size());
         for (size_t i = 0; i < rf.size(); ++i) rfi[i] = 1.0f / rf[i];
         if (upload(rfi, &v.tail_rinv)) return -2;
         if (upload(tw, &v.tail_w) || upload(tb, &v.tail_b1)) return -2;
     }
+    return 0;
+}
+
+template <class F>
+static int build_tail_fold(ojf_net *net, Vortex &v, const ojf_conv_layer *L, int into, int nacc, int rows, F m, const float *madd)
+{
+    const int out = net->pool_in, n = nacc * 16;
+    const ojf_conv_layer &lf = L[17];
+    std::vector<float> C((size_t)4 * n * out, 0.0f);
+    for (int br = 0; br < 4; ++br)
+        for (int oc = 0; oc < rows; ++oc)
+            for (int k = 0; k < out; ++k) {
+                double acc = 0.0;
+                for (int j = 0; j < out; ++j)
+                    acc += (double)m(oc, j) * (double)lf.weight_host[(size_t)j * 5 * out + out * (br + 1) + k];
+                C[((size_t)br * n + oc) * out + k] = (float)acc;
+            }
+    std::vector<float> tw, tb, rc;
+    pack_tail(tw, tb, rc, net, L, nacc, [&](int br, int oc, int k) { return oc < n && k < out ? C[((size_t)br * n + oc) * out + k] : 0.0f; });
+    std::vector<float> fb, MT((size_t)out * n, 0.0f), add(n, 0.0f);
+    const std::vector<float> zero(n, 0.0f);
+    append_chain_bias(fb, net->arith, nacc, n, zero.data(), rc);
+    for (int oc = 0; oc < rows; ++oc) {
+        double a0 = madd[oc];
+        for (int o = 0; o < out; ++o) a0 += (double)m(oc, o) * (double)lf.bias_host[o];
+        add[oc] = (float)a0;
+        for (int j = 0; j < out; ++j) {
+            double acc = 0.0;
+            for (int o = 0; o < out; ++o) acc += (double)m(oc, o) * (double)lf.weight_host[(size_t)o * 5 * out + j];
+            MT[(size_t)j * n + oc] = (float)acc;
+        }
+    }
+    if (upload(tw, &v.fold_w) || upload(fb, &v.fold_b) || upload(MT, &v.fold_MT) || upload(add, &v.fold_add)) return -2;
+    if (into == kTailEntry) {
+        std::vector<float> wt((size_t)4 * out * out);
+        for (int br = 0; br < 4; ++br)
+            for (int k = 0; k < out; ++k)
+                for (int o = 0; o < out; ++o)
+                    wt[((size_t)br * out + k) * out + o] = lf.weight_host[(size_t)o * 5 * out + out * (br + 1) + k];
+        if (upload(wt, &v.WtT)) return -2;
+    }
+    v.fold_into = into;
+    v.fold_nacc = nacc;
     return 0;
 }
 
@@ -2431,7 +2576,8 @@
     }
     release(v.branches);
     float *ptrs[] = {v.Wg, v.bg, v.Wfg, v.bf, v.bias_final, v.tail_w, v.tail_b1, v.tail_rinv, v.entry_w, v.entry_b,
-                     v.entry_wh[0], v.entry_wh[1], v.entry_bh[0], v.entry_bh[1], v.bias0};
+                     v.entry_wh[0], v.entry_wh[1], v.entry_bh[0], v.entry_bh[1], v.bias0,
+                     v.fold_w, v.fold_b, v.fold_MT, v.fold_add, v.WtT};
     for (float *p : ptrs)
         if (p) (void)hipFree(p);
 }
@@ -2447,10 +2593,21 @@
 
 static int chain_blocks(const ojf_net *net) { return ((net->npix + 15) / 16 + ojf::kChainWaves - 1) / ojf::kChainWaves; }
 
+static bool tail_fold_off()
+{
+    static const bool off = getenv("OJF_NO_TAIL_FOLD") != nullptr;
+    return off;
+}
+static bool folds_entry(const Vortex &v)
+{
+    static const bool on = getenv("OJF_TAIL_FOLD_ENTRY") != nullptr && atoi(getenv("OJF_TAIL_FOLD_ENTRY")) != 0;
+    return v.fold_into == kTailEntry && on && !tail_fold_off();
+}
+
 static int run_vortex(ojf_net *net, Vortex &v, const float *in, int in_g0, float *out, int out_g0, hipStream_t st,
                       ojf_net::Scratch &sc, const ChainArgs *head = nullptr, bool *head_done = nullptr,
                       bool entry_done = false, const Vortex *next = nullptr, bool *next_done = nullptr, bool in_split = false,
-                      int half = -1, ColSums *next_colsum = nullptr, const float *z2 = nullptr)
+                      int half = -1, ColSums *next_colsum = nullptr, const float *z2 = nullptr, const Vortex *prev_fold = nullptr)
 {
     const int h = net->h, w = net->w, c4 = net->cs / 4, o4 = net->os / 4;
     const bool h16 = net->arith == OJF_ARITH_F16X3;
@@ -2459,6 +2616,19 @@
     static const bool no_split = getenv("OJF_CONV_SPLIT") && atoi(getenv("OJF_CONV_SPLIT")) == 0;
     const bool split = h16 && chain_flow && !no_split;
     if (in_split && (!chain_flow || entry_done)) return fail("run_vortex: internal error (split-plane input without the entry kernel)");
+    if (prev_fold && (!chain_flow || !entry_done || z2 || !prev_fold->WtT))
+        return fail("run_vortex: internal error (branch sums of a folded tail without its entry planes)");
+    static const bool unfused = getenv("OJF_NO_TAIL") != nullptr;
+    const bool fused = v.tail_w && !unfused;
+    static const bool no_head_fusion = getenv("OJF_NO_HEAD_FUSION") != nullptr;
+    static const bool no_entry_fusion = getenv("OJF_NO_ENTRY_FUSION") != nullptr;
+    const bool head_tail = fused && head && net->chain_kind && !no_head_fusion;
+    const bool half_tail = fused && !head_tail && chain_flow && next && half >= 0 && half < 2 && next->entry_wh[half] && next->tail_w &&
+                           next_colsum && !no_entry_fusion;
+    const bool entry_tail = fused && !head_tail && !half_tail && chain_flow && next && next->entry_w && next->tail_w &&
+                            next->c_in_phys == net->os && !no_entry_fusion;
+    const bool fold = chain_flow && v.fold_w && ((head_tail && v.fold_into == net->chain_kind && !tail_fold_off()) ||
+                                                 (entry_tail && folds_entry(v) && next == v.fold_next));
     if (!chain_flow) {
         if (entry_done) return fail("run_vortex: internal error (entry planes without the chain flow)");
         OJF_HIP(hipEventRecord(sc.ev_fork, st));
@@ -2496,6 +2666,10 @@
         pa.h = h; pa.w = w; pa.c4 = c4;
         pa.tiles = ((w + kPoolTW - 1) / kPoolTW) * ((h + kPoolTH - 1) / kPoolTH);
         pa.gave = gave_args(net, v, nullptr, 0, 0, (z2 && net->colsum3) ? net->colsum3 : sc.colsum);
+        if (fold) {
+            pa.gave.foldT = v.fold_MT; pa.gave.fold_add = v.fold_add; pa.gave.fold_out = v.fold_b; pa.gave.fold_n = v.fold_nacc * 16;
+        }
+        if (prev_fold) { pa.gave.WtT = prev_fold->WtT; pa.gave.prev_bias = prev_fold->bias_final; }
         pa.fold_gave = chain_flow ? 1 : 0;
         pa.split_out = split ? 1 : 0;
         if (z2) {
@@ -2507,8 +2681,6 @@
         OJF_HIP(hipGetLastError());
     }
     const float *bin[4] = {z2 ? sc.Q0 : sc.Z, sc.Q1, sc.Q2, sc.Q3};
-    static const bool unfused = getenv("OJF_NO_TAIL") != nullptr;
-    const bool fused = v.tail_w && !unfused;
     static const bool branch_kernel = getenv("OJF_BRANCH_KERNEL") != nullptr && atoi(getenv("OJF_BRANCH_KERNEL")) != 0;
     static const bool subconv = getenv("OJF_SUBCONV") != nullptr && atoi(getenv("OJF_SUBCONV")) != 0;
     if (split && v.branches.n_items && branch_kernel) {
@@ -2561,18 +2733,22 @@
     ta.chain_w = nullptr; ta.chain_b = nullptr; ta.out_rows = nullptr; ta.rows_stride = 0; ta.rows_n = 0; ta.scale = 1.0f;
     ta.entry_w = nullptr; ta.entry_b = nullptr; ta.entry_out = nullptr; ta.entry_og = 0; ta.entry_act_n = 0; ta.colsum = nullptr; ta.entry_split = 0;
     const dim3 grid(chain_blocks(net)), block(ojf::kChainThreads);
-    static const bool no_head_fusion = getenv("OJF_NO_HEAD_FUSION") != nullptr;
-    static const bool no_entry_fusion = getenv("OJF_NO_ENTRY_FUSION") != nullptr;
-    if (head && net->chain_kind && !no_head_fusion) {
+    if (fold) { ta.w = planes(v.fold_w); ta.fold_b = v.fold_b; }
+    if (head_tail) {
         ta.chain_w = head->w; ta.chain_b = head->bias; ta.out_rows = head->out_rows;
         ta.rows_stride = head->rows_stride; ta.rows_n = head->rows_n; ta.scale = head->scale;
-        if (net->chain_kind == 19 && h16) hipLaunchKernelGGL((vortex_tail_kernel<OJF_ARITH_F16X3, 1, 2, 8, 19>), grid, block, 0, st, ta);
+        if (fold) {
+            if (net->chain_kind == 19 && h16) hipLaunchKernelGGL((vortex_tail_kernel<OJF_ARITH_F16X3, 1, 2, 8, 19, 6>), grid, block, 0, st, ta);
+            else if (net->chain_kind == 19) hipLaunchKernelGGL((vortex_tail_kernel<OJF_ARITH_F32, 1, 2, 8, 19, 6>), grid, block, 0, st, ta);
+            else if (h16) hipLaunchKernelGGL((vortex_tail_kernel<OJF_ARITH_F16X3, 1, 2, 8, 20, 7>), grid, block, 0, st, ta);
+            else hipLaunchKernelGGL((vortex_tail_kernel<OJF_ARITH_F32, 1, 2, 8, 20, 7>), grid, block, 0, st, ta);
+        } else if (net->chain_kind == 19 && h16) hipLaunchKernelGGL((vortex_tail_kernel<OJF_ARITH_F16X3, 1, 2, 8, 19>), grid, block, 0, st, ta);
         else if (net->chain_kind == 19) hipLaunchKernelGGL((vortex_tail_kernel<OJF_ARITH_F32, 1, 2, 8, 19>), grid, block, 0, st, ta);
         else if (h16) hipLaunchKernelGGL((vortex_tail_kernel<OJF_ARITH_F16X3, 1, 2, 8, 20>), grid, block, 0, st, ta);
         else hipLaunchKernelGGL((vortex_tail_kernel<OJF_ARITH_F32, 1, 2, 8, 20>), grid, block, 0, st, ta);
         mark_launch("vortex_tail_kernel (+ prediction head)", st);
         if (head_done) *head_done = true;
-    } else if (chain_flow && next && half >= 0 && half < 2 && next->entry_wh[half] && next->tail_w && next_colsum && !legacy_env && !no_entry_fusion) {
+    } else if (half_tail) {
         ta.entry_w = planes(next->entry_wh[half]); ta.entry_b = next->entry_bh[half]; ta.entry_out = planes(sc.Z);
         ta.entry_og = 4 * c4; ta.entry_act_n = 0; ta.colsum = next_colsum; ta.colsum_off = half * net->os;
         ta.entry_split = 0;
@@ -2580,11 +2756,13 @@
         else hipLaunchKernelGGL((vortex_tail_kernel<OJF_ARITH_F32, 1, 2, 8, kTailEntry>), grid, block, 0, st, ta);
         mark_launch("vortex_tail_kernel (+ half of the next entry GEMM)", st);
         if (next_done) *next_done = true;
-    } else if (chain_flow && next && next->entry_w && next->tail_w && next->c_in_phys == net->os && !legacy_env && !no_entry_fusion) {
+    } else if (entry_tail) {
         ta.entry_w = planes(next->entry_w); ta.entry_b = next->entry_b; ta.entry_out = planes(sc.Z);
         ta.entry_og = 4 * c4; ta.entry_act_n = net->cs; ta.colsum = sc.colsum;
         ta.entry_split = (h16 && !no_split) ? c4 : 0;
-        if (h16) hipLaunchKernelGGL((vortex_tail_kernel<OJF_ARITH_F16X3, 1, 2, 8, kTailEntry>), grid, block, 0, st, ta);
+        if (fold && h16) hipLaunchKernelGGL((vortex_tail_kernel<OJF_ARITH_F16X3, 1, 2, 8, kTailEntry, 5>), grid, block, 0, st, ta);
+        else if (fold) hipLaunchKernelGGL((vortex_tail_kernel<OJF_ARITH_F32, 1, 2, 8, kTailEntry, 5>), grid, block, 0, st, ta);
+        else if (h16) hipLaunchKernelGGL((vortex_tail_kernel<OJF_ARITH_F16X3, 1, 2, 8, kTailEntry>), grid, block, 0, st, ta);
         else hipLaunchKernelGGL((vortex_tail_kernel<OJF_ARITH_F32, 1, 2, 8, kTailEntry>), grid, block, 0, st, ta);
         mark_launch("vortex_tail_kernel (+ next entry GEMM)", st);
         if (next_done) *next_done = true;
@@ -2733,21 +2911,26 @@
     };
     const std::vector<int> dense_map = slot_map(net->pool_in, c, cs);
     const std::vector<int> flat_map = slot_map(net->pool_in, net->pool_in, os);
+    int li_first = 0, li_last = 0;
     if (version == 3) {
         rc = build_dense(0);
+        li_first = li;
         if (!rc) { rc = build_vortex(net, net->vortex[0], L + li, net->pool_in, dense_map, (gf + 1) * cs); li += 18; }
         if (!rc && sem) {
             rc = build_dense(1);
             if (!rc) { rc = build_vortex(net, net->vortex[1], L + li, net->pool_in, dense_map, (gf + 1) * cs); li += 18; }
         }
         if (!rc) {
+            li_last = li;
             rc = build_vortex(net, net->vortex[2], L + li, net->heads * net->pool_in,
                               slot_map(net->heads * net->pool_in, net->pool_in, os), net->heads * os);
             li += 18;
         }
     } else {
         rc = build_dense(0);
+        li_first = li;
         if (!rc) { rc = build_vortex(net, net->vortex[0], L + li, net->pool_in, dense_map, (gf + 1) * cs); li += 18; }
+        li_last = li;
         if (!rc) { rc = build_vortex(net, net->vortex[2], L + li, net->pool_in, flat_map, os); li += 18; }
     }
     if (!rc) {
@@ -2779,6 +2962,20 @@
         }
         if (upload(cw, &net->chain_w) || upload(cb, &net->chain_b)) rc = -2;
         else net->chain_kind = c;
+    }
+    if (!rc && net->chain_kind && net->vortex[2].tail_w) {
+        const ojf_conv_layer &p1 = L[n_layers - (2 * (gf - 1) + 3)];
+        if (p1.c_in != net->pool_in) rc = fail("ojf_net_create: prediction head shapes do not chain");
+        else
+            rc = build_tail_fold(net, net->vortex[2], L + li_last, net->chain_kind, head_first_ntout(net->chain_kind), p1.c_out,
+                                 [&](int oc, int j) { return p1.weight_host[(size_t)oc * p1.c_in + j]; }, p1.bias_host);
+    }
+    if (!rc && net->heads == 1 && net->vortex[0].tail_w && net->vortex[2].entry_w && net->vortex[2].entry_ntin == 8 &&
+        net->vortex[2].c_in_phys == os && net->vortex[2].entry_host_w.size() == (size_t)4 * cs * os) {
+        const Vortex &nx = net->vortex[2];
+        rc = build_tail_fold(net, net->vortex[0], L + li_first, kTailEntry, 5, 4 * cs,
+                             [&](int oc, int j) { return nx.entry_host_w[(size_t)oc * os + j]; }, nx.entry_host_b.data());
+        net->vortex[0].fold_next = &net->vortex[2];
     }
     if (!rc) {
         int idx = 0;
@@ -3001,14 +3198,17 @@
             OJF_HIP(hipStreamWaitEvent(st, net->ev_head_join, 0));
         }
         if (halves && entry_done != done1) return fail("ojf_net_forward: internal error (one head ran its half of the entry GEMM, the other did not)");
+        const Vortex *prev_fold = (!two && entry_done && folds_entry(net->vortex[0])) ? &net->vortex[0] : nullptr;
         if (run_vortex(net, net->vortex[2], net->YY, 0, net->Y3, 0, st, net->sc[0], head, &head_done, entry_done, nullptr, nullptr, false, -1,
-                       nullptr, (halves && entry_done) ? net->sc[1].Z : nullptr)) return -2;
+                       nullptr, (halves && entry_done) ? net->sc[1].Z : nullptr, prev_fold)) return -2;
     } else {
         if (run_dense(net, 0, st)) return -2;
         bool entry_done = false;
         if (run_vortex(net, net->vortex[0], net->X[0], 0, net->YY, 0, st, net->sc[0], nullptr, nullptr, false, &net->vortex[2],
                        &entry_done, net->chain_dense)) return -2;
-        if (run_vortex(net, net->vortex[2], net->YY, 0, net->Y3, 0, st, net->sc[0], head, &head_done, entry_done)) return -2;
+        const Vortex *prev_fold = (entry_done && folds_entry(net->vortex[0])) ? &net->vortex[0] : nullptr;
+        if (run_vortex(net, net->vortex[2], net->YY, 0, net->Y3, 0, st, net->sc[0], head, &head_done, entry_done, nullptr, nullptr, false, -1,
+                       nullptr, nullptr, prev_fold)) return -2;
     }
     if (head_done) return 0;
     if (net->chain_kind && !unfused) {
```

After: 2638 frames/sec, median of 6. 1.01x the previous value.
